# jopohl/urh

Measured on AMD Instinct MI355X. Metric: Msamples/s IQ->bits (1 GiB complex64 2-FSK per GPU, qad materialised, compact outputs copied to the host), higher is better.
Workload: dtype f32

## Files before the change

### include/urhgpu.h

```cpp
#ifndef URHGPU_H
#define URHGPU_H

#include <stdint.h>

#ifdef __cplusplus
extern "C" {
#endif

#define URHGPU_VERSION 100

#define URHGPU_OK 0
#define URHGPU_ERR_HIP (-1)
#define URHGPU_ERR_DTYPE (-2)
#define URHGPU_ERR_ARG (-3)
#define URHGPU_ERR_CAPACITY (-4)
#define URHGPU_ERR_UNSUPPORTED (-5)
#define URHGPU_ERR_NO_DEVICE (-6)

#define URHGPU_DT_I8 0
#define URHGPU_DT_U8 1
#define URHGPU_DT_I16 2
#define URHGPU_DT_U16 3
#define URHGPU_DT_F32 4

// ... 53 lines not shown
                                float *d_out, int64_t chunk, int64_t n_chunks, double *d_sum, double *d_max);

int urhgpu_bandpass(urhgpu_ctx *ctx, const float *x, int64_t n, const double *taps, int64_t m, int64_t shift,
                    int64_t n_out, double *out);

int urhgpu_bandpass_dev(urhgpu_ctx *ctx, const float *d_x, int64_t n, const double *d_taps, int64_t m, int64_t shift,
                        int64_t n_out, const float *d_left, int64_t n_left, const float *d_right, int64_t n_right,
                        void *d_out, int out_c64);

int urhgpu_iir_filter(urhgpu_ctx *ctx, const double *a, int64_t na, const double *b, int64_t nb,
                      const float *x, int64_t n, float *out);


typedef struct urhgpu_params {
    int dtype;
    int mod;
    int bits_per_symbol;
    float noise_threshold;
    float center;
    float center_spacing;
    int tolerance;
    uint32_t samples_per_symbol;
    float costas_loop_bandwidth;
    int64_t pause_threshold;
    int write_bit_sample_pos;
    float noise_other;
    int mod_order;
} urhgpu_params;

typedef struct urhgpu_outputs {
    float *qad;
    int64_t *rows;
    int64_t cap_rows;
    uint8_t *bits;
    int64_t cap_bits;
    int64_t *msg_off;
    int64_t *pauses;
    int64_t cap_msg;
    int64_t *pos;
    int64_t cap_pos;
    int64_t *pos_off;
    int64_t *counts;
    void *blob;
    int64_t cap_blob;
    int64_t *h_counts;
} urhgpu_outputs;

#define URHGPU_BLOB_MAGIC INT64_C(0x55524842424C4F42)
#define URHGPU_BLOB_HEADER_BYTES 128
#define URHGPU_BLOB_LEN16 2
#define URHGPU_BLOB_ROW16 4
int64_t urhgpu_blob_capacity(int64_t cap_rows, int64_t cap_bits, int64_t cap_msg, int64_t cap_pos, int has_pos);

int urhgpu_outputs_to_host(urhgpu_ctx *ctx, const urhgpu_outputs *out, int write_pos, void *host_dst, int64_t cap_dst, int64_t *total_bytes);

int urhgpu_afp_demod_dev(urhgpu_ctx *ctx, const void *d_iq, int64_t n, const urhgpu_params *p, float *d_qad);

int urhgpu_grab_pulse_lens_dev(urhgpu_ctx *ctx, const float *d_qad, int64_t n, const urhgpu_params *p,
                               int64_t *d_rows, int64_t cap_rows, int64_t *d_n_rows);

int urhgpu_ppseq_to_bits_dev(urhgpu_ctx *ctx, const int64_t *d_rows, const int64_t *d_n_rows, int64_t cap_rows_hint,
                             const urhgpu_params *p, const urhgpu_outputs *out);

int urhgpu_iq_to_bits_dev(urhgpu_ctx *ctx, const void *d_iq, int64_t n, const urhgpu_params *p,
                          const urhgpu_outputs *out);

typedef struct urhgpu_center_result {
    double center;
    int64_t flag;
    int64_t n_bins;
    double e0, delta;
    int64_t kept, trimmed;
    int64_t n_counts;
} urhgpu_center_result;
int urhgpu_detect_center_dev(urhgpu_ctx *ctx, const float *d_qad, int64_t n, int64_t max_size, void *d_result, int64_t hist_cap);
int urhgpu_iq_to_bits_auto_center_dev(urhgpu_ctx *ctx, const void *d_iq, int64_t n, const urhgpu_params *p, int64_t max_size,
                                      const urhgpu_outputs *out, void *d_result, void *h_result, int64_t hist_cap);
int64_t urhgpu_center_hist_cap(urhgpu_ctx *ctx);

typedef struct urhgpu_stream urhgpu_stream;
typedef struct urhgpu_host_result {
    int64_t seq;
    int64_t n_samples;
    int64_t n_rows, n_msg, n_bits, n_pos, rows_needed;
    int64_t blob_bytes;
    int truncated;
    const int32_t *row_len;
    const uint16_t *row_len16;
    const void *esc;
    int64_t n_esc;
    const int8_t *row_state;
    const uint8_t *bits_packed;
    const int64_t *msg_off, *pauses, *pos_off;
    const uint32_t *pos32;
    const void *blob;
    const float *d_qad;
    const uint16_t *row16;
} urhgpu_host_result;
int urhgpu_stream_capacities(int64_t n_max, const urhgpu_params *p, int64_t *cap_rows, int64_t *cap_bits, int64_t *cap_msg, int64_t *cap_pos);
int urhgpu_stream_create(urhgpu_ctx *ctx, int64_t n_max, const urhgpu_params *p, int want_qad, int want_pos, int64_t cap_rows, urhgpu_stream **out);
int urhgpu_stream_destroy(urhgpu_stream *st);
int urhgpu_stream_push(urhgpu_stream *st, const void *d_iq, int64_t n, urhgpu_host_result *ready);
int urhgpu_stream_push_upload(urhgpu_stream *st, const void *h_iq, void *d_iq, int64_t n, urhgpu_host_result *ready);
int urhgpu_stream_flush(urhgpu_stream *st, urhgpu_host_result *out3, int *n_out);
int urhgpu_stream_set_auto_center(urhgpu_stream *st, int enable, int64_t max_size);
int urhgpu_stream_center(urhgpu_stream *st, int64_t seq, double *center, int64_t *flag, const uint32_t **hist, int64_t *n_bins, double *e0,
                         double *delta);
int urhgpu_stream_stats(urhgpu_stream *st, int64_t *out4);
int urhgpu_stream_costas_stats(urhgpu_stream *st, int64_t *out5);
int urhgpu_stream_wide_passes(urhgpu_stream *st, int64_t *n_passes);

#define URHGPU_ROW_ABSORBED (-(INT64_C(1) << 62))
#define URHGPU_SHARD_SUMMARY_BYTES 72
int urhgpu_shard_runs_dev(urhgpu_ctx *ctx, const void *d_iq, int64_t n_local, int64_t pos_base, int64_t n_total,
                          int rank, int world, const void *d_left_halo, const urhgpu_params *p,
                          const urhgpu_outputs *out, void *d_summary);
int urhgpu_shard_prelaunch_dev(urhgpu_ctx *ctx, const void *d_iq, int64_t n_local, int64_t pos_base, int64_t n_total,
                               int rank, int world, const urhgpu_params *p, const urhgpu_outputs *out);
int urhgpu_shard_launch_dev(urhgpu_ctx *ctx, const void *d_iq, int64_t n_local, int64_t pos_base, int64_t n_total,
                            int rank, int world, const void *d_left_halo, const urhgpu_params *p, const urhgpu_outputs *out);
int urhgpu_shard_rows_dev(urhgpu_ctx *ctx, const void *d_summaries, int64_t *d_merge);
int urhgpu_shard_bits_prepare_dev(urhgpu_ctx *ctx, const int64_t *d_merge_all, int64_t *d_flags);
int urhgpu_shard_bits_finish_dev(urhgpu_ctx *ctx, const int64_t *d_flags_all);

#define URHGPU_COSTAS_SUMMARY_BYTES 160
int64_t urhgpu_costas_halo_samples(const urhgpu_params *p);
int urhgpu_shard_costas_spec_dev(urhgpu_ctx *ctx, const void *d_iq, int64_t n_local, int64_t pos_base, int64_t n_total, int rank, int world,
                                 const void *d_halo, int64_t n_halo, const urhgpu_params *p, const urhgpu_outputs *out, void *d_summary);
int urhgpu_shard_costas_resolve_dev(urhgpu_ctx *ctx, const uint32_t *start_state, uint32_t *d_end_state);

int urhgpu_shard_demod_dev(urhgpu_ctx *ctx, const void *d_iq, int64_t n_local, int64_t pos_base, int64_t n_total, int rank, int world,
                           const void *d_left_halo, const urhgpu_params *p, const urhgpu_outputs *out);
int urhgpu_shard_seam_value(urhgpu_ctx *ctx, float *seam);

int urhgpu_magnitude_chunk_stats_dev(urhgpu_ctx *ctx, const void *d_iq, int dtype, int64_t n, int64_t chunk,
                                     int64_t n_chunks, double *d_sum, double *d_max);


int urhgpu_segment_runs_dev(urhgpu_ctx *ctx, const void *d_iq, int dtype, int64_t n, float noise_threshold,
                            int64_t *d_rows, int64_t cap_rows, int64_t *d_n_rows);
int urhgpu_message_ranges_dev(urhgpu_ctx *ctx, const void *d_iq, int dtype, int64_t n, float noise_threshold, int64_t *seg_out, int64_t cap_seg_out,
                              int64_t *n_seg_out, int64_t *merged_out, int64_t cap_merged_out, int64_t *n_merged_out, int *merge_ambiguous);
int urhgpu_message_ranges_demod_dev(urhgpu_ctx *ctx, const void *d_iq, int dtype, int64_t n, float noise_threshold, int64_t *seg_out,
                                    int64_t cap_seg_out, int64_t *n_seg_out, int64_t *merged_out, int64_t cap_merged_out,
                                    int64_t *n_merged_out, int *merge_ambiguous, float *d_qad_ask);
int urhgpu_compact_gt_dev(urhgpu_ctx *ctx, const float *d_x, int64_t n, float thr, float *d_out, int64_t *d_count);
int urhgpu_edges_le_dev(urhgpu_ctx *ctx, const float *d_x, int64_t n, float center, int64_t *d_idx, int64_t cap, int64_t *d_count);
int urhgpu_minmax_f32_dev(urhgpu_ctx *ctx, const float *d_x, int64_t n, float *d_out2);
int urhgpu_pairwise_sum_f32_dev(urhgpu_ctx *ctx, const float *d_x, int64_t n, int mode, float mean, float *sum_out);
int urhgpu_histogram_f32_dev(urhgpu_ctx *ctx, const float *d_x, int64_t n, const double *d_edges, int64_t n_edges, int64_t *d_counts);

int urhgpu_msg_center_stats(urhgpu_ctx *ctx, const float *d_x, int64_t n, const int64_t *ranges, int n_msgs, int64_t max_bins,
                            double *out_stats, int64_t *out_hist, double *out_center, int32_t *out_flag);
int urhgpu_msg_plateaus(urhgpu_ctx *ctx, const float *d_x, int64_t n, const int64_t *ranges, const double *centers, int n_msgs,
                        int percentage, int64_t extra_window, int64_t *out_off, uint64_t *out_len, int64_t cap_total);

int urhgpu_merge_plateaus(const uint64_t *plateaus, int64_t n, uint64_t tolerance, uint64_t max_count, uint64_t *out, int64_t *n_out);

int urhgpu_detect_modulation_dev(urhgpu_ctx *ctx, const float *d_iq, int64_t n, const int64_t *ranges, int n_msgs, int wavelet_scale,
                                 int median_filter_order, int *labels_out, double *vars_out);

int urhgpu_msg_bit_lengths(const uint64_t *lens, const int64_t *off, int n_msgs, int64_t *tol_out, int64_t *bitlen_out);
int urhgpu_msg_plateau_decisions(urhgpu_ctx *ctx, const float *d_x, int64_t n, const int64_t *ranges, const double *centers, int n_msgs,
                                 int percentage, int64_t extra_window, int64_t *tol_out, int64_t *bitlen_out);
int urhgpu_msg_estimate(urhgpu_ctx *ctx, const float *d_x, int64_t n, const int64_t *ranges, int n_msgs, int64_t max_bins, int percentage,
                        int64_t extra_window, double *out_stats, double *out_center, int32_t *out_flag, int64_t *tol_out, int64_t *bitlen_out);
int urhgpu_test_bit_length_from_counts(const uint64_t *lens, int64_t n, int64_t *tol_out, int64_t *bitlen_out);
int urhgpu_msg_divisor_histogram(const uint64_t *lens, int64_t n, uint64_t *hist_out, int64_t cap, int64_t *hist_len, int64_t *tol_out);
int urhgpu_bit_length_from_order(const uint64_t *hist, const int64_t *order_desc, int64_t len, int64_t *bitlen_out);

int urhgpu_minmax(urhgpu_ctx *ctx, const void *arr, int dtype, int64_t n, void *out2);
int urhgpu_segment_messages(urhgpu_ctx *ctx, const void *magnitudes, int is_f64, int64_t n, float noise_threshold, int64_t *seg_out,
                            int64_t cap_seg, int64_t *n_seg);
int urhgpu_get_plateau_lengths(urhgpu_ctx *ctx, const float *rect_data, int64_t n, float center, int percentage, uint64_t *out, int64_t cap,
                               int64_t *n_out);
int urhgpu_threshold_divisor_histogram(const uint64_t *lens, int64_t n, float threshold, uint64_t *hist_out, int64_t cap, int64_t *hist_len);
int urhgpu_median_filter(urhgpu_ctx *ctx, const double *data, int64_t n, unsigned int k, float *out);

int urhgpu_test_fast_division_dev(urhgpu_ctx *ctx, uint64_t seed, int reps, uint64_t *n_mismatch);
int urhgpu_test_sincosf_fast_dev(urhgpu_ctx *ctx, uint64_t *n_mismatch);
int urhgpu_test_force_merge_ambiguous(int on);

int urhgpu_modulate_dev(urhgpu_ctx *ctx, const uint8_t *bits, const int64_t *bit_off, const uint32_t *pause, const uint32_t *start,
                        int n_msgs, uint32_t samples_per_symbol, int mod, const float *parameters, int bits_per_symbol,
                        float carrier_amplitude, float carrier_frequency, float carrier_phase, float sample_rate, int dtype,
                        void *d_out, int64_t cap_samples, int64_t *total_samples);
int urhgpu_modulate(urhgpu_ctx *ctx, const uint8_t *bits, int64_t num_bits, uint32_t samples_per_symbol, int mod,
                    const float *parameters, int bits_per_symbol, float carrier_amplitude, float carrier_frequency,
                    float carrier_phase, float sample_rate, uint32_t pause, uint32_t start, int dtype, void *out);

int urhgpu_modulate_gfsk_dev(urhgpu_ctx *ctx, const uint8_t *bits, const int64_t *bit_off, const uint32_t *pause, const uint32_t *start,
                             int n_msgs, uint32_t samples_per_symbol, const float *parameters, int bits_per_symbol,
                             float carrier_amplitude, float carrier_phase, float sample_rate, int dtype, const float *gauss_fir,
                             int n_taps, const float *frequencies, void *d_out, int64_t cap_samples, int64_t *total_samples);
int urhgpu_modulate_gfsk(urhgpu_ctx *ctx, const uint8_t *bits, int64_t num_bits, uint32_t samples_per_symbol, const float *parameters,
                         int bits_per_symbol, float carrier_amplitude, float carrier_phase, float sample_rate, uint32_t pause,
                         uint32_t start, int dtype, const float *gauss_fir, int n_taps, const float *frequencies, void *out);

int urhgpu_convert_dev(urhgpu_ctx *ctx, const void *d_src, int src_dtype, void *d_dst, int dst_dtype, int64_t n);
int urhgpu_pcm_to_iq_dev(urhgpu_ctx *ctx, const void *d_raw, int64_t n_frames, int channels, int sample_width, float *d_out);
int urhgpu_fft_peak_dev(urhgpu_ctx *ctx, const float *d_x, int64_t n, int64_t *peak_index);
int urhgpu_sub_encode_runs(const uint8_t *values, int64_t n, int64_t stride, int64_t *runs_out, int64_t cap, int64_t *n_runs);
int urhgpu_astype_dev(urhgpu_ctx *ctx, const void *d_src, int src_dtype, void *d_dst, int dst_dtype, int64_t n);

int urhgpu_path_minmax_dev(urhgpu_ctx *ctx, const void *d_samples, int dtype, int64_t start, int64_t end,
                           int64_t samples_per_pixel, void *d_values);
int urhgpu_path_minmax(urhgpu_ctx *ctx, const void *samples, int dtype, int64_t n, int64_t start, int64_t end,
                       int64_t samples_per_pixel, void *values);

int urhgpu_spectrogram_dev(urhgpu_ctx *ctx, const float *d_x, int64_t n, int window_size, int64_t hop, int64_t frames,
                           const double *d_window, const double *d_twiddles, double *d_stft, float *d_db);
int urhgpu_bgra_lookup_dev(urhgpu_ctx *ctx, const float *d_db, int64_t frames, int window_size, const uint32_t *d_colormap,
                           int n_colors, float data_min, float data_max, uint32_t *d_image);

int urhgpu_bench_copy_ceiling_dev(urhgpu_ctx *ctx, const float *d_in, float *d_out, int64_t n_samples, int shape, int reps, float *ms_per_copy);
int urhgpu_test_hot_probe(urhgpu_ctx *ctx, const void *d_iq, int64_t n, const urhgpu_params *p, float *d_qad, int stream_kind, int event_mode,
                          int graded, int launches, int keep, void *d_chunks_out, int64_t *n_chunks_out, float *dur_ms, float *gap_ms, int bubble_us,
                          int load_kind);
int urhgpu_test_hot_stamps(int on);
int urhgpu_test_tail_skip(int mask);
int urhgpu_test_fetch_chunk_tables(urhgpu_ctx *ctx, void *host_dst, int64_t n_chunks);
int urhgpu_memcpy_to_host(urhgpu_ctx *ctx, const void *d_src, void *host_dst, int64_t bytes);
int urhgpu_memcpy_dtod(urhgpu_ctx *ctx, void *d_dst, const void *d_src, int64_t bytes);

int urhgpu_test_force_state_bytes(int on);

int urhgpu_test_force_generic_tail(int on);

int urhgpu_test_force_tiles_per_chunk(int tiles);

int64_t urhgpu_test_wide_int_launches(void);

int64_t urhgpu_test_costas_host_syncs(void);
int64_t urhgpu_test_center_host_syncs(void);
int urhgpu_test_costas_scratch(int64_t n, int loop_order, int64_t *out3);

int urhgpu_test_atan2f_dev(urhgpu_ctx *ctx, const float *d_y, const float *d_x, int64_t n, float *d_out);

int urhgpu_chunk_power_stats_dev(urhgpu_ctx *ctx, const void *d_src, int dtype, int64_t n_rows, void *d_dst, int64_t n_store, double *sum_out,
                                 double *max_out);
int urhgpu_chunk_stats_launches(urhgpu_ctx *ctx, int64_t *n_launches);

int urhgpu_magnitude_chunk_partials_dev(urhgpu_ctx *ctx, const void *d_iq, int dtype, int64_t n_local, int64_t pos_base, int64_t n_total,
                                        int64_t chunk, int64_t n_chunks, double *d_sum, double *d_max);
#define URHGPU_PW_REC_HEAD 8
#define URHGPU_PW_REC_FIRST 136
#define URHGPU_PW_REC_LAST 264
#define URHGPU_PW_REC_TAIL 392
#define URHGPU_PW_REC_PIECES 520
int urhgpu_pairwise_partial_f32_dev(urhgpu_ctx *ctx, const float *d_x, int64_t m_local, int64_t g_off, int64_t m_total, int mode, float mean,
                                    float *d_out, int64_t cap, int64_t *n_out);

typedef struct urhgpu_noise_result {
    double noise;
    float noise_f32;
    float noise_sqrd;
    int64_t flag;
    int64_t chunk, n_chunks;
    int64_t n_candidates;
    double min_mean, max_mean;
} urhgpu_noise_result;
double urhgpu_noise_max_magnitude(int dtype);
int urhgpu_detect_noise_level_dev(urhgpu_ctx *ctx, const void *d_iq, int dtype, int64_t n, void *d_result);
int urhgpu_iq_to_bits_auto_dev(urhgpu_ctx *ctx, const void *d_iq, int64_t n, const urhgpu_params *p, int auto_noise, int auto_center,
                               int64_t center_max_size, const urhgpu_outputs *out, void *d_noise_result, void *h_noise_result,
                               void *d_center_result, void *h_center_result, int64_t hist_cap);
int urhgpu_stream_set_auto_noise(urhgpu_stream *st, int enable);
int urhgpu_stream_noise(urhgpu_stream *st, int64_t seq, double *noise, int64_t *flag);
int64_t urhgpu_test_noise_host_syncs(void);

typedef struct urhgpu_msg_record {
    double rssi;
    int64_t first_pos;
    int64_t mid_pos;
    int32_t n_pad;
    int32_t flag;
} urhgpu_msg_record;
int urhgpu_msg_records_dev(urhgpu_ctx *ctx, const void *d_iq, int64_t n, const urhgpu_params *p, const urhgpu_outputs *out,
                           int64_t message_length_divisor, void *d_rec, int64_t cap_msg, void *h_rec);
int urhgpu_stream_set_msg_records(urhgpu_stream *st, int enable, int64_t message_length_divisor);
int urhgpu_stream_msg_records(urhgpu_stream *st, int64_t seq, const urhgpu_msg_record **rec, int64_t *n_msg);
int64_t urhgpu_test_records_host_syncs(void);

int urhgpu_dc_correct_dev(urhgpu_ctx *ctx, const void *d_in, int64_t n, int dtype, void *d_out, void *d_mean);
int urhgpu_dc_correct(urhgpu_ctx *ctx, const void *h_in, int64_t n, int dtype, void *h_out, void *h_mean);
int64_t urhgpu_test_dc_host_syncs(void);
int urhgpu_test_dc_stats(urhgpu_ctx *ctx, int64_t *stats);

int urhgpu_shard_dc_sums_dev(urhgpu_ctx *ctx, const void *d_in, int64_t n, int dtype, void *d_words);
#define URHGPU_DC_RECORD_BYTES 64
int urhgpu_shard_dc_spec_dev(urhgpu_ctx *ctx, const void *d_in, int64_t n, const double *base, void *d_records);
int urhgpu_shard_dc_resolve_dev(urhgpu_ctx *ctx, const void *d_in, int64_t n, const uint32_t *entry, void *d_exit);
int urhgpu_shard_dc_apply_dev(urhgpu_ctx *ctx, const void *d_in, int64_t n, int dtype, const void *mean, void *d_out);
int urhgpu_shard_dc_stats(urhgpu_ctx *ctx, int64_t *stats);

#define URHGPU_SHARD_REC_SUMMARY_WORDS 10
#define URHGPU_SHARD_REC_FIRST_WORDS 8
int urhgpu_shard_records_summary_dev(urhgpu_ctx *ctx, int64_t n_local, int64_t pos_base, const urhgpu_outputs *out, void *d_words);
int urhgpu_shard_records_lookup_dev(urhgpu_ctx *ctx, const urhgpu_outputs *out, const void *d_index, int64_t n, void *d_values);
int urhgpu_shard_msg_records_dev(urhgpu_ctx *ctx, const void *d_iq, int64_t n_local, int64_t pos_base, int64_t n_total, const urhgpu_params *p,
                                 const urhgpu_outputs *out, int64_t message_length_divisor, const int64_t *first, const void *d_window,
                                 int64_t window_len, void *d_rec, int64_t cap_msg, void *h_rec);

#ifdef __cplusplus
}
#endif
#endif
```

### urh_amd/_lib.py

```python
import ctypes as C
import os
import threading

HERE = os.path.dirname(os.path.abspath(__file__))
LIB_PATH = os.path.join(HERE, "liburhgpu.so")

OK = 0
ERR_HIP, ERR_DTYPE, ERR_ARG, ERR_CAPACITY, ERR_UNSUPPORTED, ERR_NO_DEVICE = -1, -2, -3, -4, -5, -6
BLOB_LEN16 = 2
BLOB_ROW16 = 4

DT_I8, DT_U8, DT_I16, DT_U16, DT_F32 = 0, 1, 2, 3, 4
MOD_ASK, MOD_FSK, MOD_PSK, MOD_OTHER = 0, 1, 2, 3
ROW_ABSORBED = -(1 << 62)
BLOB_MAGIC = 0x55524842424C4F42
BLOB_HEADER_BYTES = 128


class UrhGpuError(RuntimeError):
    def __init__(self, status, msg):
        super().__init__(msg)
        self.status = status


class Params(C.Structure):
    _fields_ = [
        ("dtype", C.c_int), ("mod", C.c_int), ("bits_per_symbol", C.c_int),
        ("noise_threshold", C.c_float), ("center", C.c_float), ("center_spacing", C.c_float),
        ("tolerance", C.c_int), ("samples_per_symbol", C.c_uint32), ("costas_loop_bandwidth", C.c_float),
        ("pause_threshold", C.c_int64), ("write_bit_sample_pos", C.c_int), ("noise_other", C.c_float),
        ("mod_order", C.c_int),
    ]


class Outputs(C.Structure):
    _fields_ = [
        ("qad", C.c_void_p), ("rows", C.c_void_p), ("cap_rows", C.c_int64),
        ("bits", C.c_void_p), ("cap_bits", C.c_int64),
        ("msg_off", C.c_void_p), ("pauses", C.c_void_p), ("cap_msg", C.c_int64),
        ("pos", C.c_void_p), ("cap_pos", C.c_int64), ("pos_off", C.c_void_p),
        ("counts", C.c_void_p),
        ("blob", C.c_void_p), ("cap_blob", C.c_int64), ("h_counts", C.c_void_p),
    ]


class CenterResult(C.Structure):
    _fields_ = [("center", C.c_double), ("flag", C.c_int64), ("n_bins", C.c_int64), ("e0", C.c_double), ("delta", C.c_double),
                ("kept", C.c_int64), ("trimmed", C.c_int64), ("n_counts", C.c_int64)]


class NoiseResult(C.Structure):
    _fields_ = [("noise", C.c_double), ("noise_f32", C.c_float), ("noise_sqrd", C.c_float), ("flag", C.c_int64), ("chunk", C.c_int64),
                ("n_chunks", C.c_int64), ("n_candidates", C.c_int64), ("min_mean", C.c_double), ("max_mean", C.c_double)]


class MsgRecord(C.Structure):
    _fields_ = [("rssi", C.c_double), ("first_pos", C.c_int64), ("mid_pos", C.c_int64), ("n_pad", C.c_int32), ("flag", C.c_int32)]


class HostResult(C.Structure):
    _fields_ = [
        ("seq", C.c_int64), ("n_samples", C.c_int64),
        ("n_rows", C.c_int64), ("n_msg", C.c_int64), ("n_bits", C.c_int64), ("n_pos", C.c_int64), ("rows_needed", C.c_int64),
        ("blob_bytes", C.c_int64), ("truncated", C.c_int),
        ("row_len", C.c_void_p), ("row_len16", C.c_void_p), ("esc", C.c_void_p), ("n_esc", C.c_int64),
        ("row_state", C.c_void_p), ("bits_packed", C.c_void_p),
        ("msg_off", C.c_void_p), ("pauses", C.c_void_p), ("pos_off", C.c_void_p), ("pos32", C.c_void_p),
        ("blob", C.c_void_p), ("d_qad", C.c_void_p), ("row16", C.c_void_p),
    ]


_vp, _i64, _i, _f = C.c_void_p, C.c_int64, C.c_int, C.c_float
PROTOTYPES = {
    "urhgpu_version": (_i, []),
    "urhgpu_strerror": (C.c_char_p, [_i]),
    "urhgpu_last_hip_error": (C.c_char_p, []),
    "urhgpu_device_count": (_i, [C.POINTER(_i)]),
    "urhgpu_ctx_create": (_i, [_i, C.POINTER(_vp)]),
    "urhgpu_ctx_destroy": (_i, [_vp]),
    "urhgpu_ctx_set_stream": (_i, [_vp, _vp]),
    "urhgpu_ctx_use_private_stream": (_i, [_vp]),
    "urhgpu_ctx_sync": (_i, [_vp]),
    "urhgpu_ctx_set_pipelined": (_i, [_vp, _i, _vp]),
    "urhgpu_ctx_set_tuning": (_i, [_vp, C.c_char_p, _i]),
    "urhgpu_ctx_join": (_i, [_vp]),
    "urhgpu_ctx_reserve": (_i, [_vp, _i64, _i]),
    "urhgpu_ctx_info": (_i, [_vp, C.POINTER(_i), C.POINTER(_i), C.POINTER(_i64), C.c_char_p, _i]),
    "urhgpu_ctx_costas_stats": (_i, [_vp, C.POINTER(C.c_int32)]),
    "urhgpu_ctx_costas_stats5": (_i, [_vp, C.POINTER(C.c_int32)]),
    "urhgpu_ctx_profile_begin": (_i, [_vp, _i]),
    "urhgpu_ctx_profile_end": (_i, [_vp, C.POINTER(C.c_float), _i, C.POINTER(_i)]),
    "urhgpu_get_magnitudes": (_i, [_vp, _vp, _i, _i64, _vp]),
    "urhgpu_afp_demod": (_i, [_vp, _vp, _i, _i64, _f, _i, _i, _f, _f, _vp]),
    "urhgpu_get_center_thresholds": (_i, [_f, _f, _i, _vp]),
    "urhgpu_grab_pulse_lens": (_i, [_vp, _vp, _i64, _f, C.c_uint16, _i, C.c_uint32, C.c_uint8, _f, _f, _vp, _i64,
                                    C.POINTER(_i64)]),
    "urhgpu_ppseq_to_bits": (_i, [_vp, _vp, _i64, _i64, _i, _i, _i64, _vp, _i64, _vp, _vp, _i64, _vp, _i64, _vp, _vp]),
    "urhgpu_fir_filter": (_i, [_vp, _vp, _i64, _vp, _i64, _vp]),
    "urhgpu_fir_filter_dev": (_i, [_vp, _vp, _i64, _vp, _i64, _vp, _vp]),
    "urhgpu_fir_filter_stats_dev": (_i, [_vp, _vp, _i64, _vp, _i64, _vp, _vp, _i64, _i64, _vp, _vp]),
    "urhgpu_bandpass": (_i, [_vp, _vp, _i64, _vp, _i64, _i64, _i64, _vp]),
    "urhgpu_bandpass_dev": (_i, [_vp, _vp, _i64, _vp, _i64, _i64, _i64, _vp, _i64, _vp, _i64, _vp, _i]),
    "urhgpu_iir_filter": (_i, [_vp, _vp, _i64, _vp, _i64, _vp, _i64, _vp]),
    "urhgpu_afp_demod_dev": (_i, [_vp, _vp, _i64, C.POINTER(Params), _vp]),
    "urhgpu_grab_pulse_lens_dev": (_i, [_vp, _vp, _i64, C.POINTER(Params), _vp, _i64, _vp]),
    "urhgpu_ppseq_to_bits_dev": (_i, [_vp, _vp, _vp, _i64, C.POINTER(Params), C.POINTER(Outputs)]),
    "urhgpu_iq_to_bits_dev": (_i, [_vp, _vp, _i64, C.POINTER(Params), C.POINTER(Outputs)]),
    "urhgpu_detect_center_dev": (_i, [_vp, _vp, _i64, _i64, _vp, _i64]),
    "urhgpu_iq_to_bits_auto_center_dev": (_i, [_vp, _vp, _i64, C.POINTER(Params), _i64, C.POINTER(Outputs), _vp, _vp, _i64]),
    "urhgpu_center_hist_cap": (_i64, [_vp]),
    "urhgpu_stream_set_auto_center": (_i, [_vp, _i, _i64]),
    "urhgpu_stream_center": (_i, [_vp, _i64, C.POINTER(C.c_double), C.POINTER(_i64), C.POINTER(_vp), C.POINTER(_i64), C.POINTER(C.c_double),
                                  C.POINTER(C.c_double)]),
    "urhgpu_test_center_host_syncs": (_i64, []),
    "urhgpu_noise_max_magnitude": (C.c_double, [_i]),
    "urhgpu_detect_noise_level_dev": (_i, [_vp, _vp, _i, _i64, _vp]),
    "urhgpu_iq_to_bits_auto_dev": (_i, [_vp, _vp, _i64, C.POINTER(Params), _i, _i, _i64, C.POINTER(Outputs), _vp, _vp, _vp, _vp, _i64]),
    "urhgpu_stream_set_auto_noise": (_i, [_vp, _i]),
    "urhgpu_stream_noise": (_i, [_vp, _i64, C.POINTER(C.c_double), C.POINTER(_i64)]),
    "urhgpu_test_noise_host_syncs": (_i64, []),
    "urhgpu_msg_records_dev": (_i, [_vp, _vp, _i64, C.POINTER(Params), C.POINTER(Outputs), _i64, _vp, _i64, _vp]),
    "urhgpu_stream_set_msg_records": (_i, [_vp, _i, _i64]),
    "urhgpu_stream_msg_records": (_i, [_vp, _i64, C.POINTER(_vp), C.POINTER(_i64)]),
    "urhgpu_test_records_host_syncs": (_i64, []),
    "urhgpu_shard_records_summary_dev": (_i, [_vp, _i64, _i64, C.POINTER(Outputs), _vp]),
    "urhgpu_shard_records_lookup_dev": (_i, [_vp, C.POINTER(Outputs), _vp, _i64, _vp]),
    "urhgpu_shard_msg_records_dev": (_i, [_vp, _vp, _i64, _i64, _i64, C.POINTER(Params), C.POINTER(Outputs), _i64, C.POINTER(_i64), _vp, _i64, _vp, _i64,
                                          _vp]),
    "urhgpu_blob_capacity": (_i64, [_i64, _i64, _i64, _i64, _i]),
    "urhgpu_outputs_to_host": (_i, [_vp, C.POINTER(Outputs), _i, _vp, _i64, C.POINTER(_i64)]),
    "urhgpu_host_libm_check": (_i, [C.POINTER(_i64)]),
    "urhgpu_stream_capacities": (_i, [_i64, C.POINTER(Params), C.POINTER(_i64), C.POINTER(_i64), C.POINTER(_i64), C.POINTER(_i64)]),
    "urhgpu_stream_create": (_i, [_vp, _i64, C.POINTER(Params), _i, _i, _i64, C.POINTER(_vp)]),
    "urhgpu_stream_destroy": (_i, [_vp]),
    "urhgpu_stream_push": (_i, [_vp, _vp, _i64, C.POINTER(HostResult)]),
    "urhgpu_stream_push_upload": (_i, [_vp, _vp, _vp, _i64, C.POINTER(HostResult)]),
    "urhgpu_stream_flush": (_i, [_vp, C.POINTER(HostResult), C.POINTER(_i)]),
    "urhgpu_stream_stats": (_i, [_vp, C.POINTER(_i64)]),
    "urhgpu_stream_wide_passes": (_i, [_vp, C.POINTER(_i64)]),
    "urhgpu_stream_costas_stats": (_i, [_vp, C.POINTER(_i64)]),
    "urhgpu_shard_runs_dev": (_i, [_vp, _vp, _i64, _i64, _i64, _i, _i, _vp, C.POINTER(Params), C.POINTER(Outputs), _vp]),
    "urhgpu_shard_prelaunch_dev": (_i, [_vp, _vp, _i64, _i64, _i64, _i, _i, C.POINTER(Params), C.POINTER(Outputs)]),
    "urhgpu_shard_launch_dev": (_i, [_vp, _vp, _i64, _i64, _i64, _i, _i, _vp, C.POINTER(Params), C.POINTER(Outputs)]),
    "urhgpu_shard_rows_dev": (_i, [_vp, _vp, _vp]),
    "urhgpu_shard_bits_prepare_dev": (_i, [_vp, _vp, _vp]),
    "urhgpu_shard_bits_finish_dev": (_i, [_vp, _vp]),
    "urhgpu_costas_halo_samples": (_i64, [C.POINTER(Params)]),
    "urhgpu_shard_costas_spec_dev": (_i, [_vp, _vp, _i64, _i64, _i64, _i, _i, _vp, _i64, C.POINTER(Params), C.POINTER(Outputs), _vp]),
    "urhgpu_shard_costas_resolve_dev": (_i, [_vp, C.POINTER(C.c_uint32), _vp]),
    "urhgpu_shard_demod_dev": (_i, [_vp, _vp, _i64, _i64, _i64, _i, _i, _vp, C.POINTER(Params), C.POINTER(Outputs)]),
    "urhgpu_shard_seam_value": (_i, [_vp, C.POINTER(C.c_float)]),
    "urhgpu_magnitude_chunk_stats_dev": (_i, [_vp, _vp, _i, _i64, _i64, _i64, _vp, _vp]),
    "urhgpu_segment_runs_dev": (_i, [_vp, _vp, _i, _i64, _f, _vp, _i64, _vp]),
    "urhgpu_message_ranges_dev": (_i, [_vp, _vp, _i, _i64, _f, _vp, _i64, C.POINTER(_i64), _vp, _i64, C.POINTER(_i64), C.POINTER(_i)]),
    "urhgpu_message_ranges_demod_dev": (_i, [_vp, _vp, _i, _i64, _f, _vp, _i64, C.POINTER(_i64), _vp, _i64, C.POINTER(_i64), C.POINTER(_i), _vp]),
    "urhgpu_compact_gt_dev": (_i, [_vp, _vp, _i64, _f, _vp, _vp]),
    "urhgpu_edges_le_dev": (_i, [_vp, _vp, _i64, _f, _vp, _i64, _vp]),
    "urhgpu_minmax_f32_dev": (_i, [_vp, _vp, _i64, _vp]),
    "urhgpu_pairwise_sum_f32_dev": (_i, [_vp, _vp, _i64, _i, _f, C.POINTER(_f)]),
    "urhgpu_histogram_f32_dev": (_i, [_vp, _vp, _i64, _vp, _i64, _vp]),
    "urhgpu_msg_center_stats": (_i, [_vp, _vp, _i64, _vp, _i, _i64, _vp, _vp, _vp, _vp]),
    "urhgpu_msg_plateaus": (_i, [_vp, _vp, _i64, _vp, _vp, _i, _i, _i64, _vp, _vp, _i64]),
    "urhgpu_detect_modulation_dev": (_i, [_vp, _vp, _i64, _vp, _i, _i, _i, _vp, _vp]),
    "urhgpu_msg_bit_lengths": (_i, [_vp, _vp, _i, _vp, _vp]),
    "urhgpu_msg_plateau_decisions": (_i, [_vp, _vp, _i64, _vp, _vp, _i, _i, _i64, _vp, _vp]),
    "urhgpu_msg_estimate": (_i, [_vp, _vp, _i64, _vp, _i, _i64, _i, _i64, _vp, _vp, _vp, _vp, _vp]),
    "urhgpu_test_bit_length_from_counts": (_i, [_vp, _i64, C.POINTER(_i64), C.POINTER(_i64)]),
    "urhgpu_msg_divisor_histogram": (_i, [_vp, _i64, _vp, _i64, C.POINTER(_i64), C.POINTER(_i64)]),
    "urhgpu_bit_length_from_order": (_i, [_vp, _vp, _i64, C.POINTER(_i64)]),
    "urhgpu_merge_plateaus": (_i, [_vp, _i64, C.c_uint64, C.c_uint64, _vp, C.POINTER(_i64)]),
    "urhgpu_minmax": (_i, [_vp, _vp, _i, _i64, _vp]),
    "urhgpu_segment_messages": (_i, [_vp, _vp, _i, _i64, _f, _vp, _i64, C.POINTER(_i64)]),
    "urhgpu_get_plateau_lengths": (_i, [_vp, _vp, _i64, _f, _i, _vp, _i64, C.POINTER(_i64)]),
    "urhgpu_threshold_divisor_histogram": (_i, [_vp, _i64, _f, _vp, _i64, C.POINTER(_i64)]),
    "urhgpu_median_filter": (_i, [_vp, _vp, _i64, C.c_uint, _vp]),
    "urhgpu_test_hot_probe": (_i, [_vp, _vp, _i64, C.POINTER(Params), _vp, _i, _i, _i, _i, _i, _vp, C.POINTER(_i64), _vp, _vp, _i, _i]),
    "urhgpu_test_hot_stamps": (_i, [_i]),
    "urhgpu_test_tail_skip": (_i, [_i]),
    "urhgpu_test_fetch_chunk_tables": (_i, [_vp, _vp, _i64]),
    "urhgpu_test_fast_division_dev": (_i, [_vp, C.c_uint64, _i, C.POINTER(C.c_uint64)]),
    "urhgpu_test_sincosf_fast_dev": (_i, [_vp, C.POINTER(C.c_uint64)]),
    "urhgpu_test_force_merge_ambiguous": (_i, [_i]),
    "urhgpu_modulate_dev": (_i, [_vp, _vp, _vp, _vp, _vp, _i, C.c_uint32, _i, _vp, _i, _f, _f, _f, _f, _i, _vp, _i64, C.POINTER(_i64)]),
    "urhgpu_modulate": (_i, [_vp, _vp, _i64, C.c_uint32, _i, _vp, _i, _f, _f, _f, _f, C.c_uint32, C.c_uint32, _i, _vp]),
    "urhgpu_modulate_gfsk_dev": (_i, [_vp, _vp, _vp, _vp, _vp, _i, C.c_uint32, _vp, _i, _f, _f, _f, _i, _vp, _i, _vp, _vp, _i64, C.POINTER(_i64)]),
    "urhgpu_modulate_gfsk": (_i, [_vp, _vp, _i64, C.c_uint32, _vp, _i, _f, _f, _f, C.c_uint32, C.c_uint32, _i, _vp, _i, _vp, _vp]),
    "urhgpu_spectrogram_dev": (_i, [_vp, _vp, _i64, _i, _i64, _i64, _vp, _vp, _vp, _vp]),
    "urhgpu_bgra_lookup_dev": (_i, [_vp, _vp, _i64, _i, _vp, _i, _f, _f, _vp]),
    "urhgpu_convert_dev": (_i, [_vp, _vp, _i, _vp, _i, _i64]),
    "urhgpu_pcm_to_iq_dev": (_i, [_vp, _vp, _i64, _i, _i, _vp]),
    "urhgpu_sub_encode_runs": (_i, [_vp, _i64, _i64, _vp, _i64, _vp]),
    "urhgpu_fft_peak_dev": (_i, [_vp, _vp, _i64, _vp]),
    "urhgpu_astype_dev": (_i, [_vp, _vp, _i, _vp, _i, _i64]),
    "urhgpu_path_minmax_dev": (_i, [_vp, _vp, _i, _i64, _i64, _i64, _vp]),
    "urhgpu_path_minmax": (_i, [_vp, _vp, _i, _i64, _i64, _i64, _i64, _vp]),
    "urhgpu_bench_copy_ceiling_dev": (_i, [_vp, _vp, _vp, _i64, _i, _i, C.POINTER(_f)]),
    "urhgpu_memcpy_to_host": (_i, [_vp, _vp, _vp, _i64]),
    "urhgpu_memcpy_dtod": (_i, [_vp, _vp, _vp, _i64]),
    "urhgpu_test_force_state_bytes": (_i, [_i]),
    "urhgpu_test_force_tiles_per_chunk": (_i, [_i]),
    "urhgpu_test_wide_int_launches": (_i64, []),
    "urhgpu_test_costas_host_syncs": (_i64, []),
    "urhgpu_test_costas_scratch": (_i, [_i64, _i, C.POINTER(_i64)]),
    "urhgpu_test_force_generic_tail": (_i, [_i]),
    "urhgpu_test_atan2f_dev": (_i, [_vp, _vp, _vp, _i64, _vp]),
    "urhgpu_chunk_power_stats_dev": (_i, [_vp, _vp, _i, _i64, _vp, _i64, C.POINTER(C.c_double), C.POINTER(C.c_double)]),
    "urhgpu_chunk_stats_launches": (_i, [_vp, C.POINTER(_i64)]),
    "urhgpu_magnitude_chunk_partials_dev": (_i, [_vp, _vp, _i, _i64, _i64, _i64, _i64, _i64, _vp, _vp]),
    "urhgpu_pairwise_partial_f32_dev": (_i, [_vp, _vp, _i64, _i64, _i64, _i, _f, _vp, _i64, C.POINTER(_i64)]),
    "urhgpu_dc_correct_dev": (_i, [_vp, _vp, _i64, _i, _vp, _vp]),
    "urhgpu_dc_correct": (_i, [_vp, _vp, _i64, _i, _vp, _vp]),
    "urhgpu_test_dc_host_syncs": (_i64, []),
    "urhgpu_test_dc_stats": (_i, [_vp, C.POINTER(_i64)]),
    "urhgpu_shard_dc_sums_dev": (_i, [_vp, _vp, _i64, _i, _vp]),
    "urhgpu_shard_dc_spec_dev": (_i, [_vp, _vp, _i64, C.POINTER(C.c_double), _vp]),
    "urhgpu_shard_dc_resolve_dev": (_i, [_vp, _vp, _i64, C.POINTER(C.c_uint32), _vp]),
    "urhgpu_shard_dc_apply_dev": (_i, [_vp, _vp, _i64, _i, _vp, _vp]),
    "urhgpu_shard_dc_stats": (_i, [_vp, C.POINTER(_i64)]),
}

_lib = None
_lock = threading.Lock()


def _share_torch_hip_runtime():
    import importlib.util
    try:
        spec = importlib.util.find_spec("torch")
    except (ImportError, ValueError):
        spec = None
    if spec is None or not spec.origin:
        return
    cand = os.path.join(os.path.dirname(spec.origin), "lib", "libamdhip64.so")
    if os.path.exists(cand):
        try:
            C.CDLL(cand, mode=C.RTLD_GLOBAL)
        except OSError:
            pass


def load():
    global _lib
    with _lock:
        if _lib is None:
            path = os.environ.get("URHGPU_LIB", LIB_PATH)
            if not os.path.exists(path):
                raise UrhGpuError(ERR_NO_DEVICE, f"{path} is missing: build it with `python -m urh_amd.build` "
                                                 "(there is no CPU fallback)")
            _share_torch_hip_runtime()
            lib = C.CDLL(path)
            for name, (res, args) in PROTOTYPES.items():
                fn = getattr(lib, name)
                fn.restype = res
                fn.argtypes = args
            _lib = lib
    return _lib


def host_libm_check():
    out = (C.c_int64 * 4)()
    check(load().urhgpu_host_libm_check(out))
    return {"sincosf_compared": int(out[0]), "sincosf_mismatches": int(out[1]), "atan2f_compared": int(out[2]), "atan2f_mismatches": int(out[3])}


_libm_verdict = None


def host_libm_verdict(warn: bool = True):
    global _libm_verdict
    if _libm_verdict is None:
        _libm_verdict = host_libm_check()
        if warn and (_libm_verdict["sincosf_mismatches"] or _libm_verdict["atan2f_mismatches"]):
            import warnings
            warnings.warn("liburhgpu: this host's libm differs from the one the device code restates "
                          f"(sinf/cosf: {_libm_verdict['sincosf_mismatches']} of {_libm_verdict['sincosf_compared']}, atan2f: "
                          f"{_libm_verdict['atan2f_mismatches']} of {_libm_verdict['atan2f_compared']} probes): PSK / FSK results may differ from the "
                          "reference run on THIS host in isolated samples", RuntimeWarning, stacklevel=3)
    return _libm_verdict


def check(status: int):
    if status == OK:
        return
    lib = load()
    msg = lib.urhgpu_strerror(status).decode()
    if status == ERR_HIP:
        msg += ": " + lib.urhgpu_last_hip_error().decode()
    if status == ERR_DTYPE:
        raise ValueError("Unsupported dtype")
    raise UrhGpuError(status, msg)


class Context:

    def __init__(self, device: int = 0):
        lib = load()
        h = C.c_void_p()
        check(lib.urhgpu_ctx_create(int(device), C.byref(h)))
        self._h = h
        self.device = int(device)

    @property
    def handle(self):
        return self._h

    def set_stream(self, stream_ptr):
        check(load().urhgpu_ctx_set_stream(self._h, C.c_void_p(stream_ptr or 0)))

    def use_private_stream(self):
        check(load().urhgpu_ctx_use_private_stream(self._h))

    def sync(self):
        check(load().urhgpu_ctx_sync(self._h))

    def set_pipelined(self, enable: bool, tail_stream_ptr=None):
        check(load().urhgpu_ctx_set_pipelined(self._h, 1 if enable else 0, C.c_void_p(tail_stream_ptr or 0)))

    def set_tuning(self, key: str, value: int):
        check(load().urhgpu_ctx_set_tuning(self._h, key.encode(), int(value)))

    def join(self):
        check(load().urhgpu_ctx_join(self._h))

    def reserve(self, n_samples: int, tolerance: int):
        check(load().urhgpu_ctx_reserve(self._h, int(n_samples), int(tolerance)))

    def info(self):
        cu, wf, mem = C.c_int(), C.c_int(), C.c_int64()
        name = C.create_string_buffer(256)
        check(load().urhgpu_ctx_info(self._h, C.byref(cu), C.byref(wf), C.byref(mem), name, 256))
        return {"compute_units": cu.value, "wavefront": wf.value, "hbm_bytes": mem.value, "name": name.value.decode()}

    def profile_begin(self, max_records: int):
        check(load().urhgpu_ctx_profile_begin(self._h, int(max_records)))

    def profile_end(self, cap: int = 4096):
        ms = (C.c_float * cap)()
        n = C.c_int(0)
        check(load().urhgpu_ctx_profile_end(self._h, ms, cap, C.byref(n)))
        return [float(ms[i]) for i in range(min(n.value, cap))]

    def costas_stats(self):
        out = (C.c_int32 * 4)()
        check(load().urhgpu_ctx_costas_stats(self._h, out))
        return tuple(int(v) for v in out)

    def costas_stats5(self):
        out = (C.c_int32 * 5)()
        check(load().urhgpu_ctx_costas_stats5(self._h, out))
        return tuple(int(v) for v in out)

    def close(self):
        if self._h:
            load().urhgpu_ctx_destroy(self._h)
            self._h = None

    def __del__(self):
        try:
            self.close()
        except Exception:
            pass


_tls = threading.local()


def default_context() -> Context:
    ctx = getattr(_tls, "ctx", None)
    if ctx is None or ctx._h is None:
        ctx = Context(int(os.environ.get("URHGPU_DEVICE", "0")))
        _tls.ctx = ctx
    return ctx
```

### urh_amd/csrc/common.hpp

```cpp
#pragma once
#include <hip/hip_runtime.h>
#include <stdint.h>
#include <stdio.h>
#include <string.h>

#include <atomic>
#include <vector>

#include "../../include/urhgpu.h"

#ifndef URH_TAIL_PRIO_LEVEL
#define URH_TAIL_PRIO_LEVEL 3
#endif
#ifndef URH_TAIL_PAD
#define URH_TAIL_PAD 0
#endif
#if URH_TAIL_PAD
#define URH_TAIL_PRIO() do { __builtin_amdgcn_s_setprio(URH_TAIL_PRIO_LEVEL); __asm__ volatile("v_mov_b32 v95, 0" ::: "v95"); } while (0)
#else
#define URH_TAIL_PRIO() __builtin_amdgcn_s_setprio(URH_TAIL_PRIO_LEVEL)
#endif

namespace urh {

extern thread_local char g_hip_err[256];

inline int hip_fail(hipError_t e, const char *what, const char *file, int line) {
    snprintf(g_hip_err, sizeof(g_hip_err), "%s: %s (%s:%d)", what, hipGetErrorString(e), file, line);
    return URHGPU_ERR_HIP;
}

#define URH_HIP(call)                                                        \
    do {                                                                     \
        hipError_t _e = (call);                                              \
        if (_e != hipSuccess) return urh::hip_fail(_e, #call, __FILE__, __LINE__); \
    } while (0)

#define URH_TRY(call)                 \
    do {                              \
        int _s = (call);              \
        if (_s != URHGPU_OK) return _s; \
    } while (0)

struct Arena {
    void *base = nullptr;
    size_t cap = 0;
    size_t used = 0;
    int reserve(size_t bytes);
    void reset() { used = 0; }
    void *take(size_t bytes) {
        size_t off = (used + 255) & ~size_t(255);
        if (off + bytes > cap) return nullptr;
        used = off + bytes;
        return (char *)base + off;
    }
    void release();
};
inline size_t align256(size_t x) { return (x + 255) & ~size_t(255); }

extern std::atomic<long long> g_center_host_syncs;
extern thread_local int g_center_scope;
extern std::atomic<long long> g_noise_host_syncs;
extern thread_local int g_noise_scope;
extern std::atomic<long long> g_records_host_syncs;
extern thread_local int g_records_scope;
inline void center_note_wait() {
    if (g_center_scope > 0) ++g_center_host_syncs;
    if (g_noise_scope > 0) ++g_noise_host_syncs;
    if (g_records_scope > 0) ++g_records_host_syncs;
}
struct CenterScope { CenterScope() { ++g_center_scope; } ~CenterScope() { --g_center_scope; } };
struct NoiseScope { bool on; explicit NoiseScope(bool enable = true) : on(enable) { if (on) ++g_noise_scope; } ~NoiseScope() { if (on) --g_noise_scope; } };
struct RecordsScope { bool on; explicit RecordsScope(bool enable = true) : on(enable) { if (on) ++g_records_scope; } ~RecordsScope() { if (on) --g_records_scope; } };

}

constexpr size_t kSmallPinned = size_t(1) << 20;
constexpr int kNoiseMaxChunks = 199;
constexpr size_t kNoiseWorkBytes = 128 * 1024;
struct urhgpu_ctx {
    int device = 0;
    hipStream_t own_stream = nullptr;
    hipStream_t stream = nullptr;
    hipDeviceProp_t prop;
    urh::Arena arena;
    urh::Arena staging;
    urh::Arena aux;
    urh::Arena fir_work;
    hipEvent_t ev_fir = nullptr;
    hipStream_t fir_stream = nullptr;
    int64_t *d_counts = nullptr;
    int64_t *h_counts = nullptr;
    bool tune_spin_wait = true;
    bool tune_wide_int = false;
    bool tune_shard_summary_generic = false;
    int tune_costas_dev_rounds = -1;
    int32_t *costas_stats_next = nullptr;
    hipStream_t last_tail = nullptr;
    int wide_int_next = 0;
    char *h_small = nullptr;
    int32_t *d_tickets = nullptr;
    void *d_desc = nullptr;
    size_t desc_cap = 0;
    void *d_rdesc = nullptr;
    size_t rdesc_cap = 0;
    unsigned long long scan_epoch = 0x0ACE0FBA5E000000ull;
    std::vector<hipEvent_t> prof_events;
    std::vector<bool> prof_dispatch;
    int prof_used = 0;
    bool prof_on = false;
    bool prof_bracket = false;
    void *shard = nullptr;
    bool pipelined = false;
    int hot_lds_pad_sharded = 33 * 1024;
    int tune_hot_cus_removed = 4;
    hipStream_t hot_masked = nullptr;
    hipEvent_t ev_in = nullptr;
    int hot_lds_pad = 0;
    hipStream_t tail_stream = nullptr;
    bool own_tail_stream = false;
    urh::Arena arena_alt, arena_alt2;
    hipEvent_t ev_hot = nullptr;
    hipEvent_t ev_tail[3] = {nullptr, nullptr, nullptr};
    int flip = 0;
    bool tail_pending = false;
    int tile_parity = 0;
    void *d_seg = nullptr;
    bool seg_dirty[3] = {false, false, false};
    int tune_stream_segments = 7;
    int tune_stream_policy = 5;
    long long passes_begun = 0;
    bool tune_stream_latency = false;
    bool tune_stream_pos_direct = true;
    int tune_upload_pieces = 4;
    hipEvent_t ev_piece[16] = {};
    hipEvent_t ev_hot_done[3] = {nullptr, nullptr, nullptr};
    hipStream_t bits_stream = nullptr;
    hipEvent_t ev_rows[3][16] = {};
    hipEvent_t ev_bits[3] = {nullptr, nullptr, nullptr};
    urh::Arena chunk_work;
    double *h_chunk = nullptr;
    long long chunk_launches = 0;
    urh::Arena center_work;
    int tune_center_max_bins = 4096;
    hipEvent_t ev_center = nullptr;
    void *d_noise_work = nullptr;
    int wide_int_auto = 0;
    urh::Arena dc_work;
    hipEvent_t ev_dc = nullptr;
    hipStream_t dc_stream = nullptr;
    const void *dc_shard_in = nullptr;
    int64_t dc_shard_n = -1;
};
constexpr size_t kSegBlockBytes = 4096;

namespace urh {
int iq_to_bits_streamed(urhgpu_ctx *ctx, const void *d_iq, int64_t n, const urhgpu_params *p, const urhgpu_outputs *out, void *host_blob,
                        int64_t cap_host, hipEvent_t ev_ready, bool *streamed, const void *h_iq, void *stage_blob = nullptr, bool *staged = nullptr,
                        hipEvent_t ev_rows = nullptr, int len16 = 0);
hipError_t wait_stream(const urhgpu_ctx *ctx, hipStream_t s);
int reserve_psk_pass(urhgpu_ctx *ctx, int64_t n_max, int tolerance, bool want_qad);
int join_tail(urhgpu_ctx *ctx);
inline int stage_in(urhgpu_ctx *ctx, const void *host, size_t bytes, void **dev) {
    void *d = ctx->staging.take(bytes ? bytes : 16);
    if (!d) return URHGPU_ERR_ARG;
    if (bytes) URH_HIP(hipMemcpyAsync(d, host, bytes, hipMemcpyHostToDevice, ctx->stream));
    *dev = d;
    return URHGPU_OK;
}
inline int fetch_out(urhgpu_ctx *ctx, void *host, const void *dev, size_t bytes) {
    URH_HIP(hipMemcpyAsync(host, dev, bytes, hipMemcpyDeviceToHost, ctx->stream));
    URH_HIP(hipStreamSynchronize(ctx->stream));
    return URHGPU_OK;
}
}
```

### urh_amd/csrc/compact.hip

```cpp
#include <hip/hip_runtime.h>

#include "common.hpp"
#include "compact.hpp"
#include "launchers.hpp"

namespace urh {

struct PackArgs {
    const int64_t *rows; const uint8_t *bits; const int64_t *msg_off, *pauses, *pos_off, *pos; const int64_t *counts;
    int64_t cap_rows, cap_bits, cap_msg, cap_pos;
    int has_pos;
    char *blob; int64_t cap_blob;
};

__global__ __launch_bounds__(256) void k_pack_blob(const PackArgs a) {
    URH_TAIL_PRIO();
    const BlobLayout L = blob_layout(a.counts, a.cap_rows, a.cap_bits, a.cap_msg, a.cap_pos, a.has_pos);
    const int64_t gtid = blockIdx.x * 256ll + threadIdx.x, stride = (int64_t)gridDim.x * 256;
    int64_t *hdr = (int64_t *)a.blob;
    const bool fits = L.total <= a.cap_blob;
    if (gtid == 0) {
        hdr[0] = URHGPU_BLOB_MAGIC; hdr[1] = L.n_rows; hdr[2] = L.n_msg; hdr[3] = L.n_bits; hdr[4] = L.n_pos; hdr[5] = a.counts[4];
        hdr[6] = fits ? L.total : -L.total; hdr[7] = a.has_pos;
        hdr[8] = L.off_pauses; hdr[9] = L.off_msg_off; hdr[10] = L.off_pos_off; hdr[11] = L.off_row_state; hdr[12] = L.off_bits;
        hdr[13] = L.off_row_len; hdr[14] = L.off_pos32;
        if (a.counts[1] > a.cap_msg || a.counts[2] > a.cap_bits || (a.has_pos && a.counts[3] > a.cap_pos) || a.counts[4] > a.cap_rows)
            atomicOr((unsigned long long *)&hdr[15], 1ull);
    }
    bool narrow_fail = false;
    if (!fits) return;
    {
        const int64_t nb = (L.n_bits + 7) / 8;
        uint8_t *out = (uint8_t *)(a.blob + L.off_bits);
        const unsigned long long *in = (const unsigned long long *)a.bits;
        for (int64_t j = gtid; j < nb; j += stride) {
            unsigned long long w;
            if (8 * j + 8 <= L.n_bits) w = in[j];
            else { w = 0; for (int k = 0; k < 8 && 8 * j + k < L.n_bits; ++k) w |= (unsigned long long)a.bits[8 * j + k] << (8 * k); }
            out[j] = (uint8_t)(((w & 0x0101010101010101ull) * 0x8040201008040201ull) >> 56);
        }
    }
    {
        int32_t *len = (int32_t *)(a.blob + L.off_row_len);
        int8_t *st = (int8_t *)(a.blob + L.off_row_state);
        for (int64_t i = gtid; i < L.n_rows; i += stride) {
            const longlong2 r = *(const longlong2 *)(a.rows + 2 * i);
            const bool absorbed = (r.x == kRowAbsorbed);
            st[i] = absorbed ? (int8_t)-128 : (int8_t)r.x; len[i] = (int32_t)r.y;
            narrow_fail |= ((!absorbed && (r.x < -127 || r.x > 127)) || r.y < -0x80000000ll || r.y > 0x7fffffffll);
        }
    }
    if (a.has_pos) {
        uint32_t *p32 = (uint32_t *)(a.blob + L.off_pos32);
        for (int64_t i = gtid; i < L.n_pos; i += stride) {
            const int64_t v = a.pos[i];
            p32[i] = (uint32_t)v;
            narrow_fail |= (v < 0 || v > 0xffffffffll);
        }
    }
    if (narrow_fail) atomicOr((unsigned long long *)&hdr[15], 4ull);
    {
        int64_t *pa = (int64_t *)(a.blob + L.off_pauses), *mo = (int64_t *)(a.blob + L.off_msg_off), *po = (int64_t *)(a.blob + L.off_pos_off);
        for (int64_t i = gtid; i <= L.n_msg; i += stride) {
            if (i < L.n_msg) pa[i] = a.pauses[i];
            mo[i] = a.msg_off[i]; po[i] = a.pos_off[i];
        }
    }
}

int launch_pack_blob(const urhgpu_outputs *o, int write_pos, hipStream_t s) {
    if (!o->blob) return URHGPU_OK;
    if (!o->rows || !o->bits || !o->msg_off || !o->pauses || !o->pos_off || !o->counts) return URHGPU_ERR_ARG;
    if (((uintptr_t)o->bits & 7) || ((uintptr_t)o->blob & 15) || ((uintptr_t)o->rows & 15)) return URHGPU_ERR_ARG;
    const int has_pos = (write_pos && o->pos) ? 1 : 0;
    if (o->cap_blob < blob_capacity(o->cap_rows, o->cap_bits, o->cap_msg, o->cap_pos, has_pos)) return URHGPU_ERR_CAPACITY;
    PackArgs a{o->rows, o->bits, o->msg_off, o->pauses, o->pos_off, o->pos, o->counts, o->cap_rows, o->cap_bits, o->cap_msg, o->cap_pos, has_pos,
               (char *)o->blob, o->cap_blob};
#ifndef URH_PACK_BLOCKS
#define URH_PACK_BLOCKS 512
#endif
    if (hipMemsetAsync((char *)o->blob + 15 * 8, 0, 8, s) != hipSuccess) return URHGPU_ERR_HIP;
    hipLaunchKernelGGL(k_pack_blob, dim3(URH_PACK_BLOCKS), dim3(256), 0, s, a);
    return URHGPU_OK;
}

typedef float cp_v4 __attribute__((ext_vector_type(4)));
typedef float cp_v2 __attribute__((ext_vector_type(2)));
__global__ __launch_bounds__(256) void k_copy_shape(const float *in, float *out) {
    const int lane = threadIdx.x & 63;
    const int64_t wave = (int64_t)blockIdx.x * 4 + (threadIdx.x >> 6);
    const float *src = in + wave * 16 * 256 + lane * 4;
    float *dst = out + wave * 16 * 128 + lane * 2;
    cp_v4 cur[2], nxt[2];
    cur[0] = __builtin_nontemporal_load((const cp_v4 *)src);
    cur[1] = __builtin_nontemporal_load((const cp_v4 *)(src + 256));
#pragma unroll 1
    for (int r = 0; r < 16; r += 2) {
        if (r + 2 < 16) {
            nxt[0] = __builtin_nontemporal_load((const cp_v4 *)(src + (int64_t)(r + 2) * 256));
            nxt[1] = __builtin_nontemporal_load((const cp_v4 *)(src + (int64_t)(r + 3) * 256));
        }
#pragma unroll
        for (int j = 0; j < 2; ++j) {
            const cp_v2 t = {cur[j].x + cur[j].y, cur[j].z + cur[j].w};
            __builtin_nontemporal_store(t, (cp_v2 *)(dst + (int64_t)(r + j) * 128));
        }
        cur[0] = nxt[0]; cur[1] = nxt[1];
    }
}
__global__ __launch_bounds__(256) void k_copy_plain(const cp_v4 *in, cp_v4 *out, int64_t n4) {
    for (int64_t i = blockIdx.x * 256ll + threadIdx.x; i < n4; i += (int64_t)gridDim.x * 256) out[i] = in[i];
}
void launch_copy_shape(const float *in, float *out, int64_t n_samples, int shape, hipStream_t s) {
    if (shape == 0) hipLaunchKernelGGL(k_copy_shape, dim3((unsigned)(n_samples / 8192)), dim3(256), 0, s, in, out);
    else hipLaunchKernelGGL(k_copy_plain, dim3(256 * 20), dim3(256), 0, s, (const cp_v4 *)in, (cp_v4 *)out, n_samples / 4);
}

}
```

### urh_amd/csrc/compact.hpp

```cpp
#pragma once
#include <stdint.h>

#include "../../include/urhgpu.h"

namespace urh {

struct BlobLayout {
    int64_t n_rows, n_msg, n_bits, n_pos;
    int64_t off_pauses, off_msg_off, off_pos_off, off_row_state, off_bits, off_row_len, off_pos32, total;
};

__host__ __device__ inline BlobLayout blob_layout(const int64_t *counts5, int64_t cap_rows, int64_t cap_bits, int64_t cap_msg, int64_t cap_pos,
                                                  int has_pos) {
    BlobLayout L;
    L.n_rows = counts5[0] < cap_rows ? counts5[0] : cap_rows;
    L.n_msg = counts5[1] < cap_msg ? counts5[1] : cap_msg;
    L.n_bits = counts5[2] < cap_bits ? counts5[2] : cap_bits;
    L.n_pos = has_pos ? (counts5[3] < cap_pos ? counts5[3] : cap_pos) : 0;
    if (L.n_rows < 0) L.n_rows = 0;
    if (L.n_msg < 0) L.n_msg = 0;
    if (L.n_bits < 0) L.n_bits = 0;
    if (L.n_pos < 0) L.n_pos = 0;
    auto up = [](int64_t x) { return (x + 15) & ~int64_t(15); };
    int64_t o = URHGPU_BLOB_HEADER_BYTES;
    L.off_pauses = o; o = up(o + L.n_msg * 8);
    L.off_msg_off = o; o = up(o + (L.n_msg + 1) * 8);
    L.off_pos_off = o; o = up(o + (L.n_msg + 1) * 8);
    L.off_row_state = o; o = up(o + L.n_rows);
    L.off_bits = o; o = up(o + (L.n_bits + 7) / 8);
    L.off_row_len = o; o = up(o + L.n_rows * 4);
    L.off_pos32 = o; o = up(o + L.n_pos * 4);
    L.total = o;
    return L;
}

struct StagedLayout { int64_t head_cap, off_row_state, off_row_len, off_pos32, total; };
__host__ __device__ inline StagedLayout staged_layout(int64_t cap_rows, int64_t cap_bits, int64_t cap_msg, int64_t cap_pos, int has_pos) {
    const int64_t c[5] = {0, cap_msg, cap_bits, 0, 0};
    auto up = [](int64_t x) { return (x + 15) & ~int64_t(15); };
    StagedLayout S;
    S.head_cap = blob_layout(c, cap_rows, cap_bits, cap_msg, cap_pos, 0).total;
    S.off_row_state = S.head_cap;
    S.off_row_len = up(S.off_row_state + cap_rows);
    S.off_pos32 = up(S.off_row_len + 4 * cap_rows);
    S.total = up(S.off_pos32 + (has_pos ? 4 * cap_pos : 0));
    return S;
}

inline int64_t blob_capacity(int64_t cap_rows, int64_t cap_bits, int64_t cap_msg, int64_t cap_pos, int has_pos) {
    const int64_t c[5] = {cap_rows, cap_msg, cap_bits, cap_pos, cap_rows};
    return blob_layout(c, cap_rows, cap_bits, cap_msg, cap_pos, has_pos).total;
}

}
```

### urh_amd/csrc/launchers.hpp

```cpp
#pragma once
#include <atomic>
#include <hip/hip_runtime.h>
#include <stdint.h>

#include "common.hpp"
#include "runs.hpp"

namespace urh {

struct RunArgs {
    const void *in;
    float *qad;
    const void *left_halo;
    int64_t n;
    int64_t range_begin;
    int64_t range_end;
    int64_t chunk_base;
    int64_t pos_base;
    int64_t chunk_len;
    uint64_t *slab;
    int64_t slab_stride;
    ChunkInfo *chunks;
    float noise_sqrd;
    float noise_val;
    float max_magnitude;
    int order;
    int tol;
    int launch_part;
    int seg_mode;
    float dm_noise_sqrd, dm_max_magnitude, dm_noise_val;
    int lds_pad;
    uint32_t *progress;
    int32_t n_seg;
    int32_t seg_end[kMaxSegments];
    int64_t launch_lo, launch_hi;
    int64_t graded_from, graded_len;
    int wide_int;
    int stamp_probe;
    float thr[kMaxOrder - 1];
    const float *d_thr;
    const float *d_noise;
};
extern bool g_force_state_bytes;
extern std::atomic<long long> g_wide_int_launches;
extern bool g_stamp_probe;
extern int g_tail_skip;
struct HotEvents { hipEvent_t start = nullptr, stop = nullptr; bool used = false; };
int launch_wide_probe(const void *d_iq, int dtype, int64_t n, float noise_sqrd, int32_t *h_out, hipStream_t s, const float *d_noise = nullptr);
int launch_demod_runs_iq(const RunArgs &a, int dtype, int mod, bool write_qad, hipStream_t s, HotEvents *ev = nullptr);
int launch_runs_qad(const RunArgs &a, hipStream_t s, HotEvents *ev = nullptr);
bool runs_streamable(const RunArgs &a);
int launch_afp_demod(const RunArgs &a, int dtype, int mod, int grid, hipStream_t s);
int launch_afp_seam(const RunArgs &a, int dtype, int mod, float *d_out, hipStream_t s);
void launch_test_div(uint64_t seed, int reps, unsigned long long *d_mismatches, hipStream_t s);
void launch_test_sincosf_fast(unsigned long long *d_mismatches, hipStream_t s);
void launch_test_atan2f(const float *y, const float *x, int64_t n, float *out, hipStream_t s);

struct ModMsg {
    int64_t bit_off;
    int64_t n_sym;
    int64_t sym_off;
    int64_t out_off;
    uint32_t pause;
    uint32_t start;
};
constexpr int kModGfsk = 5;
struct ModArgs {
    const uint8_t *bits;
    const ModMsg *msgs;
    const float *params;
    float *phase;
    void *out;
    int n_msgs, mod, dtype, bps;
    int oqpsk;
    const float *taps;
    int n_taps;
    int freq_given;
    float *gf_freq, *gf_phase;
    uint32_t sps;
    float carrier_amplitude, carrier_frequency, carrier_phase, sample_rate;
};
int launch_modulate(const ModArgs &a, int64_t max_samples, hipStream_t s);

int launch_stft(const float2 *x, int64_t n, int ws, int64_t hop, int64_t frames, const double *window, const double2 *tw,
                double2 *out_c128, float *out_db, hipStream_t s);
int launch_bgra_lookup(const float *data, int64_t frames, int ws, const uint32_t *colormap, int n_colors, float dmin, float dmax,
                       uint32_t *image, hipStream_t s);

int launch_convert(const void *src, int src_dtype, void *dst, int dst_dtype, int64_t n, hipStream_t s);
int launch_astype(const void *src, int src_dtype, void *dst, int dst_dtype, int64_t n, hipStream_t s);
int launch_pcm_to_iq(const void *raw, int64_t n_frames, int channels, int width, float *out, hipStream_t s);
size_t fft_peak_scratch_bytes(int64_t n);
int launch_fft_peak(const float2 *x, int log2n, void *scratch, int64_t *d_peak, hipStream_t s);

int launch_path_minmax(const void *samples, int dtype, int64_t start, int64_t end, int64_t spp, void *values, hipStream_t s);

int launch_bandpass(const float2 *x, int64_t n, const float2 *left, int64_t n_left, const float2 *right, int64_t n_right,
                    const double2 *taps, int m, int64_t shift, int64_t n_out, double2 *out128, float2 *out64, hipStream_t s,
                    void *work = nullptr);
size_t bandpass_fft_work_bytes();

struct ResolveScratch {
    int32_t *has_stable;
    int32_t *prev_stable;
    int32_t *has_acc;
    int32_t *prev_acc;
    int64_t *out_cnt;
    int64_t *out_off;
    int32_t *blk_stable;
    int32_t *blk_acc;
    int64_t *blk_cnt;
};
size_t resolve_scratch_bytes(int64_t n_chunks);
ResolveScratch resolve_scratch_carve(void *mem, int64_t n_chunks);

struct ResolveAux {
    int32_t first_nonlead;
    int32_t open_chunk;
    int32_t first_stable;
    int32_t last_stable;
};
constexpr int32_t kAuxNone = 0x7F7F7F7F;

struct ResolveArgs {
    ChunkInfo *chunks;
    int64_t n_chunks;
    int64_t n_total;
    int tol;
    int local_pass;
    ResolveAux *aux;
    ChunkInfo *summary_out;
    int64_t chunk_first;
    int64_t n_local;
    int64_t *d_ts_carry;
    int64_t *rows;
    int64_t cap_rows;
    int64_t *d_n_acc;
    int64_t *d_n_rows;
    int64_t *d_n_rows_needed;
    int write_last_row;
    ResolveScratch sc;
};
struct EmitArgs {
    const ChunkInfo *chunks;
    int64_t chunk_first;
    const uint64_t *slab;
    int64_t slab_stride;
    int64_t *rows;
    int64_t cap_rows;
    int64_t *d_ts_carry;
    int is_ask;
    int64_t sps;
    ResolveScratch sc;
};
struct BitsParams {
    int64_t sps;
    int64_t bps;
    int64_t pause_threshold;
    int64_t samples_per_bit;
    int write_pos;
    const int64_t *d_row_base;
    const int64_t *d_ts_carry;
    const int64_t *d_absorbed;
    const int32_t *d_extra;
    int is_last_rank;
    const int64_t *d_rows_needed;
};
constexpr int64_t kRowAbsorbed = -(int64_t(1) << 62);
struct BitsOut {
    uint8_t *bits; int64_t cap_bits;
    int64_t *msg_off; int64_t *pauses; int64_t cap_msg;
    int64_t *pos; int64_t cap_pos; int64_t *pos_off;
    int64_t *counts;
    int64_t *h_counts = nullptr;
};
int launch_resolve(const ResolveArgs &a, int32_t *tickets, hipStream_t s);
int launch_shard_summary(const ResolveArgs &a, int32_t *ticket, hipStream_t s);
int launch_resolve_emit_single(const ResolveArgs &r, const EmitArgs &e, hipStream_t s);
int launch_emit_rows(const EmitArgs &a, int64_t n_local_chunks, hipStream_t s);
size_t merge_scratch_bytes(int64_t cap);
int launch_merge_rows_ask(const int64_t *rows_in, const int64_t *d_n_in, int64_t cap, int64_t *rows_out,
                          int64_t cap_out, int64_t *d_n_out, void *scratch, int32_t *tickets, hipStream_t s);
size_t bits_scratch_bytes(int64_t cap_rows);
struct ScanState {
    int32_t *tickets;
    void *desc;
    size_t desc_bytes;
    unsigned long long *epoch;
};
size_t bits_desc_bytes(int64_t cap_rows);
int launch_ppseq_to_bits(const int64_t *rows, const int64_t *d_n_rows, int64_t cap_rows, const BitsParams &bp,
                         const BitsOut &o, void *scratch, const ScanState &ss, hipStream_t s);
int launch_bits_prepare(const int64_t *rows, const int64_t *d_n_rows, int64_t cap_rows, const BitsParams &bp,
                        void *scratch, int64_t *d_flags, const ScanState &ss, hipStream_t s);
int launch_bits_finish(const int64_t *rows, const int64_t *d_n_rows, int64_t cap_rows, const BitsParams &bp,
                       const BitsOut &o, void *scratch, const ScanState &ss, hipStream_t s);
struct SegState {
    int64_t rows_at[kMaxSegments];
    int64_t rows_needed;
    int64_t n_acc;
    int64_t n_groups;
    int64_t n_groups_local;
    int64_t end_bits, end_pos, end_msgs;
    int64_t err;
    struct In {
        int64_t g0;
        int64_t carry[3];
        int64_t ship_bits, ship_pos, ship_msgs, pad;
    } in[2];
};
static_assert(sizeof(SegState) == 128 + 64 + 128, "SegState");
constexpr int64_t kSegAlign = 256;
struct SegGate {
    const uint32_t *progress;
    int k;
    uint32_t target;
    int init;
    SegState *seg;
    long long max_ticks;
    int fused;
};
struct RowsSegment {
    int index;
    int final;
    int64_t c0, c1;
    SegGate gate;
    int8_t *h_state;
    int32_t *h_len;
    int fuse_gate;
    int len16;
    int64_t *esc;
    int64_t esc_cap;
};
struct BitsSegment {
    int index;
    int final;
    int64_t c0, c1;
    int rows_index;
    SegState *state;
};
struct SegPackDst {
    void *host;
    int64_t cap_host;
    uint32_t *progress_reset;
    int blocks;
    int pos_direct;
    int split;
    void *host_head;
    const int64_t *esc;
    int64_t esc_cap;
    int64_t row16_esc_off;
};

struct TileTailMem {
    void *mem;
    int64_t n_chunks;
    int32_t *huge_count;
    int parity;
    void *rdesc;
    unsigned long long epoch;
    int64_t *d_row_base = nullptr;
};
size_t tile_rdesc_bytes(int64_t n_chunks);
size_t tile_tail_bytes(int64_t n_chunks);
int64_t tile_desc_cap(int64_t cap_rows, int64_t n_chunks);
int launch_tile_rows(const ResolveArgs &r, const EmitArgs &e, const TileTailMem &m, const BitsParams *bp, hipStream_t s);
int launch_tile_bits(const TileTailMem &m, const int64_t *rows, const int64_t *d_n_rows, int64_t cap_rows, const BitsParams &bp,
                     const BitsOut &o, void *scratch, const ScanState &ss, hipStream_t s);
int launch_tile_bits_prepare(const TileTailMem &m, const int64_t *rows, const int64_t *d_n_rows, int64_t cap_rows, const BitsParams &bp,
                             void *scratch, int64_t *d_flags, const ScanState &ss, hipStream_t s);
int launch_tile_bits_finish(const TileTailMem &m, const int64_t *rows, const int64_t *d_n_rows, int64_t cap_rows, const BitsParams &bp,
                            const BitsOut &o, void *scratch, const ScanState &ss, hipStream_t s);
int launch_rows_segment(const ResolveArgs &r, const EmitArgs &e, const TileTailMem &m, const BitsParams &bp, SegState *state, const RowsSegment &sg,
                        hipStream_t s);
int launch_bits_segment(const TileTailMem &m, const BitsParams &bp, const BitsOut &o, void *scratch, const ScanState &ss, int64_t *rows,
                        int64_t cap_rows, const BitsSegment &sg, const SegPackDst *dst, hipStream_t s);
void launch_merge_summary(const int64_t *rows, const int64_t *d_n_rows, int64_t *d_out5, hipStream_t s);
void launch_merge_fix(int64_t *rows, const int64_t *d_n_rows, const int64_t *d_all, int rank, int world,
                      int64_t *d_absorbed, hipStream_t s);
void launch_bits_extra(const int64_t *d_all, int rank, int world, int32_t *d_extra, hipStream_t s);

size_t fir_stats_scratch_bytes(int64_t n);
size_t fir_work_bytes(int64_t n, int m);
int launch_fir(const float2 *x, int64_t n, const float2 *taps, int m, const float2 *halo, float2 *out, hipStream_t s, void *work = nullptr,
               int64_t chunk = 0, int64_t n_chunks = 0, double *d_sum = nullptr, double *d_max = nullptr, void *tile_scratch = nullptr);
int launch_iir(const double *a, int64_t M, const double *b, int64_t N, const float2 *x, int64_t n, float2 *y, hipStream_t s);
int launch_magnitudes(const void *iq, int dtype, int64_t n, double *out, hipStream_t s);
size_t mag_chunk_scratch_bytes(int64_t n_chunks);
int launch_mag_chunk_stats(const void *iq, int dtype, int64_t n, int64_t chunk, int64_t n_chunks, double *d_sum, double *d_max,
                           void *scratch, hipStream_t s);
int launch_noise_chain(const void *iq, int dtype, int64_t n, double max_mag, float cfg_noise, int use_cfg, void *work, void *d_result, void *h_result,
                       hipStream_t s);
size_t compact_scratch_bytes(int64_t n);
int launch_compact_gt(const float *x, int64_t n, const int64_t *d_n, float thr, float *out, int64_t *d_count, void *scratch,
                      int32_t *tickets, hipStream_t s);
int launch_compact_edges(const float *x, int64_t n, const int64_t *d_n, float center, int64_t *out, int64_t cap, int64_t *d_count,
                         void *scratch, int32_t *tickets, hipStream_t s);
size_t minmax_scratch_bytes();
int launch_minmax(const float *x, int64_t n, float *d_out2, void *scratch, hipStream_t s);
int launch_minmax_any(const void *x, int dtype, int64_t n, void *d_out2, void *scratch, hipStream_t s);
int launch_above_flags(const void *mag, int is_f64, int64_t n, float thr, float *flags, hipStream_t s);
int launch_median_filter(const double *data, int64_t n, int k, float *out, hipStream_t s);
constexpr int kDtAboveFlags = 100;
int pairwise_sum_f32(urhgpu_ctx *ctx, const float *d_x, int64_t n, int mode, float mean, float *out);
int launch_hist_edges(const float *x, int64_t n, const double *d_edges, int n_edges, int64_t *d_counts, hipStream_t s);
size_t sp_mag_scratch_bytes(int64_t n_chunks);
int launch_mag_chunk_partials(const void *iq, int dtype, int64_t n_local, int64_t pos_base, int64_t n_total, int64_t chunk, int64_t n_chunks,
                              double *d_sum, double *d_max, void *scratch, hipStream_t s);
int64_t pairwise_partial_words(int64_t m_local, int64_t g_off, int64_t m_total);
size_t pairwise_partial_scratch_bytes(int64_t m_local);
int launch_pairwise_partial(const float *x, int64_t m_local, int64_t g_off, int64_t m_total, int mode, float mean, float *rec, void *scratch,
                            hipStream_t s);
size_t chunk_stats_scratch_bytes(int dtype, int64_t n_rows);
int launch_chunk_stats(const void *d_src, int dtype, int64_t n_rows, void *d_dst, int64_t store_rows, void *scratch, double *h_out, hipStream_t s);
struct SegCtl;
extern bool g_force_merge_ambiguous;
int launch_message_ranges(const int64_t *d_rows, const int64_t *d_n_rows, int64_t cap_rows, const void *d_iq, int dtype, int64_t n, float thr,
                          int ook_merge, int64_t *d_seg, int64_t *d_msgs, int64_t cap, SegCtl *d_ctl, void *scratch, hipStream_t s);
size_t seg_scratch_bytes(int64_t cap_rows, int64_t cap);
size_t seg_ctl_bytes();
void seg_ctl_read(const void *host_copy, int64_t *n_seg, int64_t *n_msgs, int *ambiguous);
int launch_pack_blob(const urhgpu_outputs *o, int write_pos, hipStream_t s);
void launch_copy_shape(const float *in, float *out, int64_t n_samples, int shape, hipStream_t s);
int launch_msg_records(const void *d_iq, int64_t n, const urhgpu_params *p, const urhgpu_outputs *out, int64_t divisor, void *d_rec, int64_t cap_rec,
                       void *h_rec, hipStream_t s);
size_t costas_scratch_bytes(int64_t n);
int launch_costas(urhgpu_ctx *ctx, const void *d_iq, int64_t n, const urhgpu_params *p, float *d_qad, void *scratch, const float *d_noise = nullptr);
extern std::atomic<long long> g_costas_host_syncs;
void costas_scratch_layout(int64_t n, int K, int64_t out3[3]);
constexpr int kCostasSummaryBytes = 160;
struct CostasShard {
    const void *iq;
    const void *halo_end;
    float *out;
    int64_t n, origin, lo, start1;
    urhgpu_params p;
    void *scratch;
};
int64_t costas_halo_samples(const urhgpu_params *p);
int launch_costas_shard_spec(urhgpu_ctx *ctx, const CostasShard &cs, void *d_summary);
int launch_costas_shard_resolve(urhgpu_ctx *ctx, const CostasShard &cs, uint32_t freq_bits, uint32_t phase_bits, void *d_end);

}
```

### urh_amd/csrc/pulse_table.hip

```cpp
#include <hip/hip_runtime.h>

#include <algorithm>

#include "common.hpp"
#include "compact.hpp"
#include "launchers.hpp"
#include "runs.hpp"
#include "scan.hpp"

namespace urh {

#ifndef URH_RESOLVE_BLOCK
#define URH_RESOLVE_BLOCK 256
#endif
#ifndef URH_RESOLVE_ITEMS
#define URH_RESOLVE_ITEMS 4
#endif
constexpr int kResolveBlock = URH_RESOLVE_BLOCK;

__host__ __device__ static inline int64_t resolve_blocks(int64_t n_chunks) { return (n_chunks + kResolveBlock - 1) / kResolveBlock; }

size_t resolve_scratch_bytes(int64_t n_chunks) {
    return (size_t)n_chunks * (4 * 4 + 2 * 8) + (size_t)(resolve_blocks(n_chunks) + 1) * (4 + 4 + 8) + 10 * 256;
}
// ... 1307 lines not shown
            int64_t type = 0;
#if URH_EXPAND_PREFETCH
            longlong2 row_pf = longlong2{0, 0};
            if (i + 64 < end) row_pf = *(const longlong2 *)(a.rows + 2 * (i + 64));
            if (i < end) {
                type = row_cur.x;
                v = row_value(type, row_cur.y, i == 0 && row0g, a.bp);
            }
            row_cur = row_pf;
#else
            if (i < end) {
                const longlong2 row = (i0 == off) ? row0 : *(const longlong2 *)(a.rows + 2 * i);
                type = row.x;
                v = row_value(type, row.y, i == 0 && row0g, a.bp);
            }
#endif
            int64_t in_bits = v.v[0], in_ts = v.v[2];
            int in_l = (int)v.v[1];
#if URH_DPP_SCAN
            in_bits = wave_incl_sum_dpp(in_bits); in_ts = wave_incl_sum_dpp(in_ts); in_l = wave_incl_sum_dpp(in_l);
#else
#pragma unroll
            for (int o = 1; o < 64; o <<= 1) {
                const int64_t ub = __shfl_up(in_bits, o), ut = __shfl_up(in_ts, o);
                const int ul = __shfl_up(in_l, o);
                if (lane >= o) { in_bits += ub; in_ts += ut; in_l += ul; }
            }
#endif
            int64_t kb = 0, ob = 0, op = 0, ts = 0;
            if (i < end && v.v[0] > 0 && v.v[0] <= own_limit) {
                const int64_t grp = run.v[1] + in_l - v.v[1];
                if (grp < n_groups) {
                    GroupOut go = go0;
                    if (grp != g0) go = a.gout[grp];
                    if (go.is_msg) {
                        const int64_t bit_prefix = run.v[0] + in_bits - v.v[0];
                        kb = v.v[0];
                        ob = go.out_bits + (bit_prefix - go.bits_start);
                        op = go.out_pos + (bit_prefix - go.bits_start);
                        ts = run.v[2] + in_ts - v.v[2];
                    }
                }
            }
            constexpr int kShort = 16;
#if URH_EXPAND_EARLY_EXIT
            {
                const int kbs = (kb > 0 && kb <= kShort) ? (int)kb : 0;
                const int nb = (ob + kbs <= a.cap_bits) ? kbs : (int)((a.cap_bits > ob) ? a.cap_bits - ob : 0);
                const int np = !a.bp.write_pos ? 0 : ((op + kbs <= a.cap_pos) ? kbs : (int)((a.cap_pos > op) ? a.cap_pos - op : 0));
                uint8_t *bp8 = a.bits + ob;
                int64_t *pp = a.pos + op;
                uint32_t *hp = a.h_pos ? a.h_pos + op : nullptr;
                int64_t tsk = ts;
                int sh = bps - 1;
#pragma unroll 1
                for (int k = 0; k < kShort; ++k) {
                    if (__ballot(k < kbs) == 0ull) break;
                    const uint8_t b = (type < 0) ? 0 : (uint8_t)((type >> sh) & 1);
                    sh = (sh == 0) ? bps - 1 : sh - 1;
                    if (k < nb) bp8[k] = b;
                    if (k < np) { pp[k] = tsk; if (hp) hp[k] = (uint32_t)tsk; }
                    tsk += a.bp.samples_per_bit;
                }
            }
#else
            if (kb > 0 && kb <= kShort) {
                const int nb = (ob + kb <= a.cap_bits) ? (int)kb : (int)((a.cap_bits > ob) ? a.cap_bits - ob : 0);
                const int np = !a.bp.write_pos ? 0 : ((op + kb <= a.cap_pos) ? (int)kb : (int)((a.cap_pos > op) ? a.cap_pos - op : 0));
                uint8_t *bp8 = a.bits + ob;
                int64_t *pp = a.pos + op;
                uint32_t *hp = a.h_pos ? a.h_pos + op : nullptr;
                int64_t tsk = ts;
                int sh = bps - 1;
                for (int k = 0; k < (int)kb; ++k) {
                    const uint8_t b = (type < 0) ? 0 : (uint8_t)((type >> sh) & 1);
                    sh = (sh == 0) ? bps - 1 : sh - 1;
                    if (k < nb) bp8[k] = b;
                    if (k < np) { pp[k] = tsk; if (hp) hp[k] = (uint32_t)tsk; }
                    tsk += a.bp.samples_per_bit;
                }
            }
#endif
            unsigned long long big = __ballot(kb > kShort);
            while (big) {
                const int src = __builtin_ctzll(big);
                big &= big - 1;
                const int64_t kb_s = __shfl(kb, src), ob_s = __shfl(ob, src), op_s = __shfl(op, src), ts_s = __shfl(ts, src),
                              ty_s = __shfl(type, src);
                for (int64_t k = lane; k < kb_s; k += 64) {
                    const uint8_t b = symbol_bit(ty_s, k, bps);
                    if (ob_s + k < a.cap_bits) a.bits[ob_s + k] = b;
                    if (a.bp.write_pos && op_s + k < a.cap_pos) {
                        a.pos[op_s + k] = ts_s + k * a.bp.samples_per_bit;
                        if (a.h_pos) a.h_pos[op_s + k] = (uint32_t)(ts_s + k * a.bp.samples_per_bit);
                    }
                }
            }
            run.v[0] += lane_bcast(in_bits, 63); run.v[1] += lane_bcast(in_l, 63); run.v[2] += lane_bcast(in_ts, 63);
        }
        row0 = row_next;
    }
}

int launch_resolve(const ResolveArgs &a, int32_t *tickets, hipStream_t s) {
    if (a.n_chunks <= 0) return URHGPU_ERR_ARG;
    const unsigned g = (unsigned)((a.n_chunks + kResolveBlock - 1) / kResolveBlock);
    (void)tickets;
    hipLaunchKernelGGL(k_resolve_a, dim3(g), dim3(kResolveBlock), 0, s, a);
    hipLaunchKernelGGL(k_resolve_b, dim3(g), dim3(kResolveBlock), 0, s, a);
    hipLaunchKernelGGL(k_resolve_c, dim3(g), dim3(kResolveBlock), 0, s, a);
    return URHGPU_OK;
}

int launch_shard_summary(const ResolveArgs &a, int32_t *ticket, hipStream_t s) {
    if (a.n_chunks <= 0 || !a.local_pass || !a.summary_out || a.n_chunks >= kAuxNone) return URHGPU_ERR_ARG;
    static_assert(sizeof(ShardPart) <= 256 && sizeof(ShardPart) <= (size_t)kResolveBlock * 8, "one partial per kResolveBlock chunks fits the out_cnt section (8 bytes per chunk, 256-byte granules)");
    const unsigned g = (unsigned)resolve_blocks(a.n_chunks);
    hipLaunchKernelGGL(k_shard_summary, dim3(g), dim3(kResolveBlock), 0, s, a, (ShardPart *)a.sc.out_cnt, ticket);
    return URHGPU_OK;
}

int launch_resolve_emit_single(const ResolveArgs &r, const EmitArgs &e, hipStream_t s) {
    if (r.n_chunks <= 0 || r.local_pass || r.chunk_first != 0 || r.n_local != r.n_chunks || e.chunk_first != 0) return URHGPU_ERR_ARG;
    const unsigned g = (unsigned)((r.n_chunks + kResolveBlock - 1) / kResolveBlock);
    hipLaunchKernelGGL(k_resolve_a, dim3(g), dim3(kResolveBlock), 0, s, r);
    hipLaunchKernelGGL(k_resolve_b, dim3(g), dim3(kResolveBlock), 0, s, r);
    hipLaunchKernelGGL(k_emit_rows_fused, dim3((unsigned)r.n_chunks), dim3(64), 0, s, e, r);
    return URHGPU_OK;
}

int launch_emit_rows(const EmitArgs &a, int64_t n_local_chunks, hipStream_t s) {
    if (n_local_chunks > 0) hipLaunchKernelGGL(k_emit_rows, dim3((unsigned)n_local_chunks), dim3(64), 0, s, a);
    return URHGPU_OK;
}

static inline int64_t scan_blocks(int64_t cap) { return (cap + kScanTile - 1) / kScanTile; }
constexpr int kGroupItems = 1;
static inline int64_t group_scan_blocks(int64_t cap) { return (cap + kScanBlock * kGroupItems - 1) / (kScanBlock * kGroupItems); }

size_t merge_scratch_bytes(int64_t cap) {
    return (size_t)(scan_blocks(cap) + 1) * sizeof(VecK<2>) + 256 + (size_t)cap * 16 + 512;
}

int launch_merge_rows_ask(const int64_t *rows_in, const int64_t *d_n_in, int64_t cap, int64_t *rows_out,
                          int64_t cap_out, int64_t *d_n_out, void *scratch, int32_t *tickets, hipStream_t s) {
    if (cap <= 0) return URHGPU_OK;
    const int64_t nb = scan_blocks(cap);
    char *p = (char *)scratch;
    VecK<2> *partials = (VecK<2> *)p; p += ((size_t)(nb + 1) * sizeof(VecK<2>) + 255) & ~size_t(255);
    int64_t *grp_state = (int64_t *)p; p += (size_t)cap * 8;
    int64_t *grp_end = (int64_t *)p;
    MergeLoad ld{rows_in};
    MergeStore st{rows_in, d_n_in, grp_state, grp_end};
    (void)tickets;
    hipLaunchKernelGGL((k_scan_reduce<2, MergeLoad>), dim3(scan_grid(nb)), dim3(kScanBlock), 0, s, d_n_in, ld, partials, nb);
    hipLaunchKernelGGL((k_scan_apply<2, MergeLoad, MergeStore>), dim3(scan_grid(nb)), dim3(kScanBlock), 0, s, d_n_in, ld, partials, nb, st,
                       kScanAlwaysDirect);
    hipLaunchKernelGGL((k_scan_finish<2, NoFinal>), dim3(1), dim3(kScanBlock), 0, s, d_n_in, partials, nb, NoFinal(), kScanAlwaysDirect);
    int64_t fin_blocks = (cap + 255) / 256; if (fin_blocks > 4096) fin_blocks = 4096;
    hipLaunchKernelGGL(k_merge_finish, dim3((unsigned)fin_blocks), dim3(256), 0, s, partials + nb, grp_state, grp_end,
                       rows_out, cap_out, d_n_out);
    return URHGPU_OK;
}

size_t bits_scratch_bytes(int64_t cap_rows) {
    const int64_t nb = scan_blocks(cap_rows);
    const int64_t cap_groups = cap_rows + 1;
    const int64_t nbg = group_scan_blocks(cap_groups);
    return (size_t)(nb + 1) * sizeof(VecK<4>) + (size_t)(nbg + 1) * sizeof(VecK<3>) + (size_t)cap_rows * sizeof(RowInfo) +
           (size_t)cap_groups * (sizeof(GroupInfo) + sizeof(GroupOut)) + 64 + 8 * 256 + 64 + 256 +
           (size_t)kHugeCap * sizeof(HugeRow) + 256;
}

namespace {
struct BitsScratch {
    VecK<4> *part4; VecK<3> *part3; RowInfo *info; GroupInfo *groups; GroupOut *gout; int64_t *d_n_groups;
    HugeRow *huge; int32_t *huge_count;
    int64_t nb, nbg;
};
BitsScratch carve_bits(void *scratch, int64_t cap_rows) {
    BitsScratch b;
    b.nb = scan_blocks(cap_rows);
    const int64_t cap_groups = cap_rows + 1;
    b.nbg = group_scan_blocks(cap_groups);
    char *p = (char *)scratch;
    auto take = [&](size_t bytes) { char *r = p; p += (bytes + 255) & ~size_t(255); return r; };
    b.part4 = (VecK<4> *)take((size_t)(b.nb + 1) * sizeof(VecK<4>));
    b.part3 = (VecK<3> *)take((size_t)(b.nbg + 1) * sizeof(VecK<3>));
    b.info = (RowInfo *)take((size_t)cap_rows * sizeof(RowInfo));
    b.groups = (GroupInfo *)take((size_t)cap_groups * sizeof(GroupInfo));
    b.gout = (GroupOut *)take((size_t)cap_groups * sizeof(GroupOut));
    b.d_n_groups = (int64_t *)take(64);
    b.huge_count = (int32_t *)take(64);
    b.huge = (HugeRow *)take((size_t)kHugeCap * sizeof(HugeRow));
    return b;
}
}

struct GroupCountFinal {
    const int64_t *d_n_rows;
    const GroupInfo *groups;
    int64_t *d_n_groups;
    int64_t *d_flags;
    __device__ void operator()(const VecK<4> &grand) const {
        const int64_t n = *d_n_rows;
        const int64_t n_l = (n > 0) ? grand.v[1] : 0;
        *d_n_groups = (n > 0) ? n_l + 1 : 0;
        if (d_flags) {
            d_flags[0] = n_l > 0;
            d_flags[1] = (n > 0) && groups[0].data_end > 0;
            d_flags[2] = (n > 0) && (groups[n_l].data_end - (n_l ? groups[n_l - 1].data_end : 0) > 0);
        }
    }
};

size_t bits_desc_bytes(int64_t cap_rows) {
    if (cap_rows <= 0) cap_rows = 1;
    return (((size_t)(scan_blocks(cap_rows) + 1) * sizeof(ScanDesc<4>) + 255) & ~size_t(255)) + (size_t)(group_scan_blocks(cap_rows + 1) + 1) * sizeof(ScanDesc<3>) + 512;
}

int launch_bits_prepare(const int64_t *rows, const int64_t *d_n_rows, int64_t cap_rows, const BitsParams &bp,
                        void *scratch, int64_t *d_flags, const ScanState &ss, hipStream_t s) {
    if (cap_rows <= 0) cap_rows = 1;
    if (ss.desc_bytes < bits_desc_bytes(cap_rows)) return URHGPU_ERR_ARG;
    const BitsScratch b = carve_bits(scratch, cap_rows);
    const bool single = (d_flags == nullptr);
    BitsLoad ld{rows, d_n_rows, bp, single ? b.d_n_groups : nullptr};
    BitsStore st{rows, d_n_rows, b.info, b.groups, bp.d_ts_carry, bp.d_absorbed, single ? b.d_n_groups : nullptr};
    GroupCountFinal fin{d_n_rows, b.groups, b.d_n_groups, d_flags};
    hipLaunchKernelGGL((k_scan_reduce<4, BitsLoad>), dim3(scan_grid(b.nb)), dim3(kScanBlock), 0, s, d_n_rows, ld, b.part4, b.nb);
    hipLaunchKernelGGL((k_scan_apply<4, BitsLoad, BitsStore>), dim3(scan_grid(b.nb)), dim3(kScanBlock), 0, s, d_n_rows, ld, b.part4, b.nb, st,
                       kScanAlwaysDirect);
    if (!single)
        hipLaunchKernelGGL((k_scan_finish<4, GroupCountFinal>), dim3(1), dim3(kScanBlock), 0, s, d_n_rows, b.part4, b.nb, fin, kScanAlwaysDirect);
    return URHGPU_OK;
}

int launch_bits_finish(const int64_t *rows, const int64_t *d_n_rows, int64_t cap_rows, const BitsParams &bp,
                       const BitsOut &o, void *scratch, const ScanState &ss, hipStream_t s) {
    if (cap_rows <= 0) cap_rows = 1;
    if (ss.desc_bytes < bits_desc_bytes(cap_rows)) return URHGPU_ERR_ARG;
    const BitsScratch b = carve_bits(scratch, cap_rows);
    ScanDesc<3> *desc3 = (ScanDesc<3> *)((char *)ss.desc + (((size_t)(b.nb + 1) * sizeof(ScanDesc<4>) + 255) & ~size_t(255)));
    GroupLoad gl{b.groups, b.d_n_groups, bp.d_extra, bp.is_last_rank, bp.write_pos};
    GroupStore gs{gl, b.gout, o.msg_off, o.pauses, o.pos_off, o.pos, o.cap_msg, o.cap_pos};
    BitsCountsFinal fin{d_n_rows, o.msg_off, o.pos_off, o.counts, b.huge_count, bp.d_rows_needed, o.h_counts};
    if (!(g_tail_skip & 8))
        hipLaunchKernelGGL((k_scan_lookback<3, GroupLoad, GroupStore, BitsCountsFinal, kGroupItems>), dim3(scan_grid(b.nbg)), dim3(kScanBlock), 0, s,
                           b.d_n_groups, gl, desc3, b.nbg, gs, fin, ++*ss.epoch, ss.tickets + 2, 0);
    ExpandArgs ea{rows, d_n_rows, b.info, b.gout, o.bits, o.cap_bits, o.pos, o.cap_pos, bp, b.huge, b.huge_count, kHugeCap};
    const int64_t eb = std::min<int64_t>((cap_rows + 255) / 256, kExpandMaxBlocks);
    hipLaunchKernelGGL(k_expand_bits, dim3((unsigned)eb), dim3(256), 0, s, ea);
    hipLaunchKernelGGL(k_expand_huge, dim3(kHugeGridX, kHugeGridY), dim3(256), 0, s, ea);
    return URHGPU_OK;
}

int launch_ppseq_to_bits(const int64_t *rows, const int64_t *d_n_rows, int64_t cap_rows, const BitsParams &bp,
                         const BitsOut &o, void *scratch, const ScanState &ss, hipStream_t s) {
    URH_TRY(launch_bits_prepare(rows, d_n_rows, cap_rows, bp, scratch, nullptr, ss, s));
    return launch_bits_finish(rows, d_n_rows, cap_rows, bp, o, scratch, ss, s);
}


int g_tail_skip = 0;
namespace {
constexpr int kTileHugeCap = 8192;
struct TileCarve { TileTail ft; HugeRef *huge; };
TileCarve carve_tile(const TileTailMem &m) {
    TileCarve tc;
    char *p = (char *)m.mem;
    auto take = [&](size_t bytes) { char *r = p; p += (bytes + 255) & ~size_t(255); return r; };
    const int64_t nt = m.n_chunks + 1;
    tc.ft.ploc = (ResElem *)take((size_t)m.n_chunks * sizeof(ResElem));
    tc.ft.btot = (ResElem *)take((size_t)(resolve_blocks(m.n_chunks) + 1) * sizeof(ResElem));
    tc.ft.agg = (VecK<4> *)take((size_t)nt * sizeof(VecK<4>));
    tc.ft.excl = (VecK<4> *)take((size_t)nt * sizeof(VecK<4>));
    tc.ft.tile_off = (int64_t *)take((size_t)nt * 8);
    tc.ft.tile_cnt = (int32_t *)take((size_t)nt * 4);
    tc.ft.d_n_tiles = (int64_t *)take(64);
    tc.huge = (HugeRef *)take((size_t)kTileHugeCap * sizeof(HugeRef));
    tc.ft.huge_count = m.huge_count;
    tc.ft.parity = m.parity;
    tc.ft.want_bits = 0;
    tc.ft.rdesc = (GranDesc *)m.rdesc;
    tc.ft.epoch = m.epoch;
    tc.ft.d_row_base = m.d_row_base;
    tc.ft.esc = nullptr;
    return tc;
}
}

int64_t tile_desc_cap(int64_t cap_rows, int64_t n_chunks) { return std::max<int64_t>(cap_rows, 8 * (n_chunks + 2) + kScanTile); }

size_t tile_rdesc_bytes(int64_t n_chunks) {
    return (size_t)(resolve_blocks(n_chunks) + 2 + (n_chunks + 1 + kScanBlock - 1) / kScanBlock + 2) * sizeof(GranDesc);
}

size_t tile_tail_bytes(int64_t n_chunks) {
    const int64_t nt = n_chunks + 1;
    return (size_t)n_chunks * sizeof(ResElem) + (size_t)(resolve_blocks(n_chunks) + 1) * sizeof(ResElem) + (size_t)nt * (2 * sizeof(VecK<4>) + 12) +
           64 + (size_t)kTileHugeCap * sizeof(HugeRef) + 10 * 256;
}

int launch_tile_rows(const ResolveArgs &r, const EmitArgs &e, const TileTailMem &m, const BitsParams *bp, hipStream_t s) {
    if (r.n_chunks <= 0 || r.local_pass || r.chunk_first != e.chunk_first || r.chunk_first < 0 || r.chunk_first + r.n_local > r.n_chunks ||
        m.n_chunks != r.n_chunks || e.is_ask)
        return URHGPU_ERR_ARG;
    if ((r.n_local != r.n_chunks) != (m.d_row_base != nullptr)) return URHGPU_ERR_ARG;
    TileCarve tc = carve_tile(m);
    EmitTileArgs g;
    g.e = e; g.r = r; g.ft = tc.ft; g.huge = tc.huge; g.huge_cap = kTileHugeCap;
    memset(&g.bp, 0, sizeof(g.bp));
    if (bp) { g.bp = *bp; g.ft.want_bits = 1; }
    const unsigned gb = (unsigned)resolve_blocks(r.n_chunks);
    g.w0 = 0; g.w_end = tail_waves(r.n_chunks); g.final_seg = 1; g.seg = nullptr; g.seg_k = 0; g.h_state = nullptr; g.h_len = nullptr; g.len16 = 0; g.esc = nullptr; g.esc_cap = 0; g.ft.esc = nullptr;
    SegGate no_gate;
    memset(&no_gate, 0, sizeof(no_gate));
    if (!(g_tail_skip & 1)) hipLaunchKernelGGL(k_resolve_one, dim3(gb), dim3(kResolveBlock), 0, s, r, g.ft, (int64_t)0, no_gate);
    if (!(g_tail_skip & 2)) hipLaunchKernelGGL(k_emit_rows_tiles, dim3((unsigned)((tail_waves(r.n_chunks) + 1 + kEmitWaves - 1) / kEmitWaves)), dim3(64 * kEmitWaves), 0, s, g);
    return URHGPU_OK;
}

namespace {
__global__ void k_tile_flags(const int64_t *d_n_rows, const GroupInfo *groups, const int64_t *d_n_groups, int64_t *d_flags) {
    const int64_t n = *d_n_rows, ng = *d_n_groups;
    const int64_t n_l = (n > 0 && ng > 0) ? ng - 1 : 0;
    d_flags[0] = n_l > 0;
    d_flags[1] = (n > 0) && groups[0].data_end > 0;
    d_flags[2] = (n > 0) && (groups[n_l].data_end - (n_l ? groups[n_l - 1].data_end : 0) > 0);
}
}

int launch_tile_bits_prepare(const TileTailMem &m, const int64_t *rows, const int64_t *d_n_rows, int64_t cap_rows, const BitsParams &bp,
                             void *scratch, int64_t *d_flags, const ScanState &ss, hipStream_t s) {
    if (cap_rows <= 0) cap_rows = 1;
    const int64_t nt = m.n_chunks + 1;
    const int64_t cap_desc = tile_desc_cap(cap_rows, m.n_chunks);
    if (ss.desc_bytes < bits_desc_bytes(cap_desc)) return URHGPU_ERR_ARG;
    const TileCarve tc = carve_tile(m);
    const BitsScratch b = carve_bits(scratch, cap_rows);
    const int64_t cap_groups = cap_rows + 1;
    GranDesc *tdesc = (GranDesc *)m.rdesc + resolve_blocks(m.n_chunks) + 2;
    TileScanArgs ta{rows, d_n_rows, tc.ft.agg, tc.ft.tile_off, tc.ft.tile_cnt, tc.ft.excl, b.groups, cap_groups, b.d_n_groups, nt, bp, tdesc,
                    m.epoch, 0, nullptr, 0};
    const unsigned nb_ts = (unsigned)((nt + kScanBlock - 1) / kScanBlock);
    if (!(g_tail_skip & 4)) hipLaunchKernelGGL(k_tile_scan, dim3(nb_ts), dim3(kScanBlock), 0, s, ta);
    if (d_flags) hipLaunchKernelGGL(k_tile_flags, dim3(1), dim3(1), 0, s, d_n_rows, b.groups, b.d_n_groups, d_flags);
    return URHGPU_OK;
}

int launch_tile_bits_finish(const TileTailMem &m, const int64_t *rows, const int64_t *d_n_rows, int64_t cap_rows, const BitsParams &bp,
                            const BitsOut &o, void *scratch, const ScanState &ss, hipStream_t s) {
    if (cap_rows <= 0) cap_rows = 1;
    const int64_t nt = m.n_chunks + 1;
    const int64_t cap_desc = tile_desc_cap(cap_rows, m.n_chunks);
    if (ss.desc_bytes < bits_desc_bytes(cap_desc)) return URHGPU_ERR_ARG;
    const TileCarve tc = carve_tile(m);
    const BitsScratch b = carve_bits(scratch, cap_rows);
    ScanDesc<3> *desc3 = (ScanDesc<3> *)((char *)ss.desc + (((size_t)(scan_blocks(cap_desc) + 1) * sizeof(ScanDesc<4>) + 255) & ~size_t(255)));
    GroupLoad gl{b.groups, b.d_n_groups, bp.d_extra, bp.is_last_rank, bp.write_pos};
    GroupStore gs{gl, b.gout, o.msg_off, o.pauses, o.pos_off, o.pos, o.cap_msg, o.cap_pos};
    BitsCountsFinal fin{d_n_rows, o.msg_off, o.pos_off, o.counts, b.huge_count, bp.d_rows_needed, o.h_counts};
    if (!(g_tail_skip & 8))
        hipLaunchKernelGGL((k_scan_lookback<3, GroupLoad, GroupStore, BitsCountsFinal, kGroupItems>), dim3(scan_grid(b.nbg)), dim3(kScanBlock), 0, s,
                           b.d_n_groups, gl, desc3, b.nbg, gs, fin, ++*ss.epoch, ss.tickets + 2, 0);
    ExpandTileArgs ea{rows, d_n_rows, tc.ft.excl, tc.ft.tile_off, tc.ft.tile_cnt, b.gout, b.d_n_groups, o.bits, o.cap_bits, o.pos, o.cap_pos,
                      bp, tc.huge, m.huge_count, kTileHugeCap, m.parity, nt, 0, nullptr};
    const unsigned tile_blocks = (unsigned)expand_tile_blocks(nt);
    if (!(g_tail_skip & 16)) hipLaunchKernelGGL(k_expand_tiles, dim3(tile_blocks + kHugeBlocksX * kHugeBlocksY), dim3(64 * kEmitWaves), 0, s, ea);
    return URHGPU_OK;
}

int launch_tile_bits(const TileTailMem &m, const int64_t *rows, const int64_t *d_n_rows, int64_t cap_rows, const BitsParams &bp,
                     const BitsOut &o, void *scratch, const ScanState &ss, hipStream_t s) {
    URH_TRY(launch_tile_bits_prepare(m, rows, d_n_rows, cap_rows, bp, scratch, nullptr, ss, s));
    return launch_tile_bits_finish(m, rows, d_n_rows, cap_rows, bp, o, scratch, ss, s);
}

__global__ void k_seg_gate(const SegGate gate) {
    if (threadIdx.x != 0) return;
    if (gate.init) gate.seg->err = 0;
    if (!gate.progress) return;
    const uint32_t *ctr = gate.progress + gate.k * kProgressStride;
    const long long t0 = (long long)wall_clock64();
    while (__hip_atomic_load(ctr, __ATOMIC_RELAXED, __HIP_MEMORY_SCOPE_AGENT) < gate.target) {
        __builtin_amdgcn_s_sleep(16);
        if ((long long)wall_clock64() - t0 > gate.max_ticks) { gate.seg->err = 1 + gate.k; break; }
    }
}

struct SegGroupLoad {
    GroupLoad ld;
    const SegState *seg;
    int parity;
    __device__ VecK<3> operator()(int64_t i) const { return ld(seg->in[parity].g0 + i); }
};
struct SegGroupStore {
    GroupStore st;
    const SegState *seg;
    int parity;
    __device__ void operator()(int64_t i, const VecK<3> &val, const VecK<3> &ex) const {
        const int64_t g0 = seg->in[parity].g0;
        VecK<3> e = ex;
#pragma unroll
        for (int k = 0; k < 3; ++k) e.v[k] += seg->in[parity].carry[k];
        st(g0 + i, val, e);
    }
};
struct SegFinal {
    SegGroupLoad ld;
    SegState *seg;
    const int64_t *d_n_rows;
    int parity;
    int final;
    BitsCountsFinal counts;
    __device__ void operator()(const VecK<3> &grand) const {
        const SegState::In in = seg->in[parity];
        const int64_t nl = seg->n_groups_local;
        VecK<3> tot;
#pragma unroll
        for (int k = 0; k < 3; ++k) tot.v[k] = in.carry[k] + grand.v[k];
        if (final) {
            counts(tot);
            const bool any = *d_n_rows > 0;
            seg->end_msgs = any ? tot.v[0] : 0; seg->end_bits = any ? tot.v[1] : 0; seg->end_pos = any ? tot.v[2] : 0;
            return;
        }
        SegState::In nx = in;
        if (nl <= 0) {
            seg->end_msgs = 0; seg->end_bits = 0; seg->end_pos = 0;
        } else {
            const int64_t g_open = in.g0 + nl - 1;
            const VecK<3> vo = ld(nl - 1);
            VecK<3> exo;
#pragma unroll
            for (int k = 0; k < 3; ++k) exo.v[k] = tot.v[k] - vo.v[k];
            const int64_t d0 = g_open ? ld.ld.groups[g_open - 1].data_end : 0;
            const bool has_data = ld.ld.groups[g_open].data_end - d0 > 0;
            nx.g0 = g_open;
#pragma unroll
            for (int k = 0; k < 3; ++k) nx.carry[k] = exo.v[k];
            seg->end_msgs = exo.v[0]; seg->end_bits = exo.v[1] + vo.v[1]; seg->end_pos = exo.v[2] + vo.v[2];
            nx.ship_msgs = exo.v[0];
            nx.ship_bits = has_data ? exo.v[1] + vo.v[1] : exo.v[1];
            nx.ship_pos = has_data ? exo.v[2] + vo.v[2] : exo.v[2];
        }
        seg->in[parity ^ 1] = nx;
    }
};

struct SegPack {
    const uint8_t *bits; const int64_t *msg_off, *pauses, *pos_off, *pos; const int64_t *counts;
    int64_t cap_rows, cap_bits, cap_msg, cap_pos;
    int has_pos;
    char *host;
    BlobLayout L;
    const SegState *seg;
    const int64_t *d_n_rows;
    int parity, final;
    uint32_t *progress;
    int pos_shipped;
    int split;
    char *head;
    const int64_t *esc;
    int64_t esc_cap;
    int64_t row16_esc_off;
};
__global__ __launch_bounds__(256) void k_pack_seg(const SegPack a) {
    URH_TAIL_PRIO();
    const int64_t gtid = blockIdx.x * 256ll + threadIdx.x, stride = (int64_t)gridDim.x * 256;
    const SegState::In in = a.seg->in[a.parity];
    auto lim = [](int64_t x, int64_t cap) { return x < cap ? (x < 0 ? 0 : x) : cap; };
    const int64_t nbits = lim(a.seg->end_bits, a.cap_bits);
    const int64_t j0 = lim(in.ship_bits, a.cap_bits) / 8, j1 = a.final ? (nbits + 7) / 8 : nbits / 8;
    const int64_t p0 = a.has_pos ? lim(in.ship_pos, a.cap_pos) : 0, p1 = a.has_pos ? lim(a.seg->end_pos, a.cap_pos) : 0;
    const int64_t m0 = lim(in.ship_msgs, a.cap_msg), m1 = lim(a.seg->end_msgs, a.cap_msg);
    BlobLayout L = a.L;
    if (a.split) {
        const int64_t c5[5] = {0, m1, nbits, 0, 0};
        const BlobLayout T = blob_layout(c5, a.cap_rows, a.cap_bits, a.cap_msg, a.cap_pos, 0);
        L.off_pauses = T.off_pauses; L.off_msg_off = T.off_msg_off; L.off_pos_off = T.off_pos_off; L.off_bits = T.off_bits;
    }
    {
        uint8_t *out = (uint8_t *)(a.head + L.off_bits);
        const unsigned long long *in8 = (const unsigned long long *)a.bits;
        auto pack8 = [&](int64_t j) -> unsigned long long {
            unsigned long long w;
            if (8 * j + 8 <= nbits) w = in8[j];
            else { w = 0; for (int k = 0; k < 8 && 8 * j + k < nbits; ++k) w |= (unsigned long long)a.bits[8 * j + k] << (8 * k); }
            return ((w & 0x0101010101010101ull) * 0x8040201008040201ull) >> 56;
        };
#if URH_PACK_WORDS
        int64_t ja = j0 + (int64_t)((8 - ((uintptr_t)(out + j0) & 7)) & 7);
        if (ja > j1) ja = j1;
        int64_t nw = (j1 - ja) / 8;
        const int64_t full = nbits / 8;
        if (ja + 8 * nw > full) nw = full > ja ? (full - ja) / 8 : 0;
        for (int64_t k = gtid; k < nw; k += stride) {
            const int64_t j = ja + 8 * k;
            unsigned long long r = 0;
#pragma unroll
            for (int b = 0; b < 8; ++b) r |= (((in8[j + b] & 0x0101010101010101ull) * 0x8040201008040201ull) >> 56) << (8 * b);
            *(unsigned long long *)(out + j) = r;
        }
        for (int64_t j = j0 + gtid; j < ja; j += stride) out[j] = (uint8_t)pack8(j);
        for (int64_t j = ja + 8 * nw + gtid; j < j1; j += stride) out[j] = (uint8_t)pack8(j);
#else
        for (int64_t j = j0 + gtid; j < j1; j += stride) out[j] = (uint8_t)pack8(j);
#endif
    }
    if (a.has_pos && !a.pos_shipped) {
        uint32_t *p32 = (uint32_t *)(a.host + L.off_pos32);
        for (int64_t i = p0 + gtid; i < p1; i += stride) p32[i] = (uint32_t)a.pos[i];
    }
    {
        int64_t *pa = (int64_t *)(a.head + L.off_pauses), *mo = (int64_t *)(a.head + L.off_msg_off), *po = (int64_t *)(a.head + L.off_pos_off);
        if (gtid == 0 && m0 == 0) { mo[0] = 0; po[0] = 0; }
        for (int64_t i = m0 + gtid; i < m1; i += stride) { pa[i] = a.pauses[i]; mo[i + 1] = a.msg_off[i + 1]; po[i + 1] = a.pos_off[i + 1]; }
    }
    int64_t n_esc = 0;
    if (a.esc && a.final) {
        n_esc = a.esc[0];
        const bool over = n_esc > a.esc_cap;
        if (over) n_esc = a.esc_cap;
        int64_t *dst = (int64_t *)(a.head + (a.row16_esc_off > 0 ? a.row16_esc_off : ((L.off_bits + (nbits + 7) / 8 + 15) & ~int64_t(15))));
        if (gtid == 0) dst[0] = over ? -n_esc : n_esc;
        for (int64_t i = gtid; i < n_esc; i += stride) dst[1 + i] = a.esc[1 + i];
    }
    if (a.final && gtid == 0) {
        int64_t *hdr = (int64_t *)a.head;
        const int64_t *c = a.counts;
        const int64_t n_rows = lim(*a.d_n_rows, a.cap_rows);
        hdr[1] = n_rows; hdr[2] = m1; hdr[3] = nbits; hdr[4] = p1; hdr[5] = c[4];
        const bool row16 = a.esc && a.row16_esc_off > 0;
        hdr[6] = URHGPU_BLOB_HEADER_BYTES + n_rows * (row16 ? 2 : (a.esc ? 3 : 5)) + (a.esc ? 8 + n_esc * 8 : 0) + (nbits + 7) / 8 + p1 * 4 + m1 * 24 + 16;
        hdr[7] = a.has_pos | (row16 ? URHGPU_BLOB_ROW16 : (a.esc ? URHGPU_BLOB_LEN16 : 0));
        hdr[8] = L.off_pauses; hdr[9] = L.off_msg_off; hdr[10] = L.off_pos_off; hdr[11] = row16 ? a.row16_esc_off : L.off_row_state; hdr[12] = L.off_bits;
        hdr[13] = L.off_row_len; hdr[14] = L.off_pos32;
        hdr[15] = ((c[1] > a.cap_msg || c[2] > a.cap_bits || (a.has_pos && c[3] > a.cap_pos) || c[4] > a.cap_rows) ? 1 : 0) | (a.seg->err ? 2 : 0);
        hdr[0] = URHGPU_BLOB_MAGIC;
    }
    if (a.final && a.progress && gtid < kMaxSegments) a.progress[gtid * kProgressStride] = 0;
}

int launch_rows_segment(const ResolveArgs &r, const EmitArgs &e, const TileTailMem &m, const BitsParams &bp, SegState *state, const RowsSegment &sg,
                        hipStream_t s) {
    if (r.n_chunks <= 0 || r.local_pass || r.chunk_first != 0 || e.chunk_first != 0 || r.n_local != r.n_chunks || m.n_chunks != r.n_chunks ||
        e.is_ask || m.d_row_base != nullptr || !state || sg.index < 0 || sg.index >= kMaxSegments)
        return URHGPU_ERR_ARG;
    if (sg.c0 < 0 || sg.c0 % kSegAlign || sg.c1 <= sg.c0 || sg.c1 > r.n_chunks || (sg.final ? sg.c1 != r.n_chunks : (sg.c1 % kSegAlign != 0 || sg.c1 >= r.n_chunks)))
        return URHGPU_ERR_ARG;
    static_assert(kSegAlign % kResolveBlock == 0 && kSegAlign % kScanBlock == 0 && kSegAlign % (kTailCPW * kEmitWaves) == 0, "segment alignment");
    if (sg.final && (r.d_n_rows != &state->rows_at[sg.index] || r.d_n_rows_needed != &state->rows_needed)) return URHGPU_ERR_ARG;
    if ((sg.h_state == nullptr) != (sg.h_len == nullptr) || sg.gate.seg != state) return URHGPU_ERR_ARG;
    const TileCarve tc = carve_tile(m);
    EmitTileArgs g;
    g.e = e; g.r = r; g.ft = tc.ft; g.huge = tc.huge; g.huge_cap = kTileHugeCap;
    g.bp = bp; g.ft.want_bits = 1;
    g.w0 = sg.c0 / kTailCPW; g.w_end = sg.final ? tail_waves(r.n_chunks) : sg.c1 / kTailCPW; g.final_seg = sg.final; g.seg = state; g.seg_k = sg.index;
    g.h_state = sg.h_state; g.h_len = sg.h_len;
    g.len16 = (sg.len16 && sg.esc && sg.h_len) ? sg.len16 : 0; g.esc = g.len16 ? sg.esc : nullptr; g.esc_cap = sg.esc_cap;
    g.ft.esc = (g.len16 && sg.index == 0) ? sg.esc : nullptr;
    if (g_tail_skip & 64) { g.h_state = nullptr; g.h_len = nullptr; }
    if (g_tail_skip & 128) g.e.rows = nullptr;
    TileTail ft_resolve = g.ft;
    if (sg.index != 0) ft_resolve.want_bits = 0;
    SegGate gate = sg.gate;
    gate.fused = (sg.fuse_gate && gate.progress && !gate.init && resolve_blocks(sg.c1 - sg.c0) == 1) ? 1 : 0;
    if (!gate.fused && gate.progress) hipLaunchKernelGGL(k_seg_gate, dim3(1), dim3(64), 0, s, gate);
    if (!(g_tail_skip & 1)) hipLaunchKernelGGL(k_resolve_one, dim3((unsigned)resolve_blocks(sg.c1 - sg.c0)), dim3(kResolveBlock), 0, s, r, ft_resolve, sg.c0 / kResolveBlock, gate);
    if (!(g_tail_skip & 2)) hipLaunchKernelGGL(k_emit_rows_tiles, dim3((unsigned)((g.w_end - g.w0 + 1 + kEmitWaves - 1) / kEmitWaves)), dim3(64 * kEmitWaves), 0, s, g);
    return URHGPU_OK;
}

int launch_bits_segment(const TileTailMem &m, const BitsParams &bp, const BitsOut &o, void *scratch, const ScanState &ss, int64_t *rows,
                        int64_t cap_rows, const BitsSegment &sg, const SegPackDst *dst, hipStream_t s) {
    if (m.n_chunks <= 0 || m.d_row_base != nullptr || !sg.state || sg.rows_index < 0 || sg.rows_index >= kMaxSegments) return URHGPU_ERR_ARG;
    if (sg.c0 < 0 || sg.c0 % kSegAlign || sg.c1 <= sg.c0 || sg.c1 > m.n_chunks || (sg.final ? sg.c1 != m.n_chunks : (sg.c1 % kSegAlign != 0 || sg.c1 >= m.n_chunks)))
        return URHGPU_ERR_ARG;
    if (cap_rows <= 0) cap_rows = 1;
    const int64_t cap_desc = tile_desc_cap(cap_rows, m.n_chunks);
    if (ss.desc_bytes < bits_desc_bytes(cap_desc)) return URHGPU_ERR_ARG;
    const TileCarve tc = carve_tile(m);
    const BitsScratch b = carve_bits(scratch, cap_rows);
    SegState *st = sg.state;
    const int64_t *d_n_rows = &st->rows_at[sg.rows_index];
    const int parity = sg.index & 1;
    const int64_t t1 = sg.final ? m.n_chunks + 1 : sg.c1;
    const int64_t cap_groups = cap_rows + 1;
    GranDesc *tdesc = (GranDesc *)m.rdesc + resolve_blocks(m.n_chunks) + 2;
    TileScanArgs ta{rows, d_n_rows, tc.ft.agg, tc.ft.tile_off, tc.ft.tile_cnt, tc.ft.excl, b.groups, cap_groups, &st->n_groups, t1, bp, tdesc,
                    m.epoch, sg.c0 / kScanBlock, st, parity};
    if (!(g_tail_skip & 4)) hipLaunchKernelGGL(k_tile_scan, dim3((unsigned)((t1 - sg.c0 + kScanBlock - 1) / kScanBlock)), dim3(kScanBlock), 0, s, ta);
    ScanDesc<3> *desc3 = (ScanDesc<3> *)((char *)ss.desc + (((size_t)(scan_blocks(cap_desc) + 1) * sizeof(ScanDesc<4>) + 255) & ~size_t(255)));
    GroupLoad gl{b.groups, &st->n_groups, nullptr, sg.final ? 1 : 0, bp.write_pos, sg.final ? 0 : 1};
    const int has_pos = (bp.write_pos && o.pos) ? 1 : 0;
    const int64_t caps[5] = {cap_rows, o.cap_msg, o.cap_bits, o.cap_pos, cap_rows};
    BlobLayout L = blob_layout(caps, cap_rows, o.cap_bits, o.cap_msg, o.cap_pos, has_pos);
    const bool split = dst && dst->host && dst->split;
    if (split) {
        if (!sg.final || sg.c0 != 0) return URHGPU_ERR_ARG;
        const StagedLayout SL = staged_layout(cap_rows, o.cap_bits, o.cap_msg, o.cap_pos, has_pos);
        L.off_row_state = SL.off_row_state; L.off_row_len = SL.off_row_len; L.off_pos32 = SL.off_pos32;
    }
    const bool pos_direct = dst && dst->host && has_pos && sg.final && sg.c0 == 0 && dst->pos_direct;
    uint32_t *h_pos = pos_direct ? (uint32_t *)((char *)dst->host + L.off_pos32) : nullptr;
    GroupStore gs{gl, b.gout, o.msg_off, o.pauses, o.pos_off, o.pos, o.cap_msg, o.cap_pos, h_pos};
    SegGroupLoad sl{gl, st, parity};
    SegGroupStore sst{gs, st, parity};
    SegFinal fin{sl, st, d_n_rows, parity, sg.final ? 1 : 0, BitsCountsFinal{d_n_rows, o.msg_off, o.pos_off, o.counts, b.huge_count, &st->rows_needed, o.h_counts}};
    if (!(g_tail_skip & 8))
        hipLaunchKernelGGL((k_scan_lookback<3, SegGroupLoad, SegGroupStore, SegFinal, kGroupItems>), dim3((unsigned)std::min<int64_t>(scan_grid(b.nbg), 32)),
                           dim3(kScanBlock), 0, s, &st->n_groups_local, sl, desc3, b.nbg, sst, fin, ++*ss.epoch, ss.tickets + 2, 0);
    ExpandTileArgs ea{rows, d_n_rows, tc.ft.excl, tc.ft.tile_off, tc.ft.tile_cnt, b.gout, &st->n_groups, o.bits, o.cap_bits, o.pos, o.cap_pos,
                      bp, tc.huge, m.huge_count, kTileHugeCap, m.parity, t1, sg.c0, h_pos};
    const unsigned tile_blocks = (unsigned)expand_tile_blocks(t1 - sg.c0);
    if (g_tail_skip & 2048) ea.cap_bits = 0;
    if (!(g_tail_skip & 16)) hipLaunchKernelGGL(k_expand_tiles, dim3(tile_blocks + kHugeBlocksX * kHugeBlocksY), dim3(64 * kEmitWaves), 0, s, ea);
// ... 73 lines not shown
```

### urh_amd/csrc/shard.hip

```cpp
#include "pass.hpp"

using namespace urh;

namespace {

struct ShardSession {
    int phase = 0;
    bool piped = false;
    RunArgs run;
    int rank = 0, world = 1;
    int64_t n_local = 0, pos_base = 0, n_total = 0;
    urhgpu_params p;
    urhgpu_outputs out;
    Plan pl;
    ChunkInfo *table = nullptr;
    uint64_t *slab = nullptr;
    ResolveAux *aux = nullptr;
    void *rs_mem = nullptr;
    int64_t *rows_stage = nullptr; void *merge_scratch = nullptr; int64_t *d_n_stage = nullptr;
    void *bits_scratch = nullptr;
    int64_t *d_small = nullptr;
    const int64_t *d_row_base = nullptr;
    bool use_tile = false;
    TileTailMem tile;
    CostasShard costas;
    int costas_phase = 0;
    bool demod_done = false;
    const void *demod_iq = nullptr; float *demod_qad = nullptr; int64_t demod_n = 0;
    int demod_mod = 0, demod_dtype = 0; float demod_noise = 0.f;
    float *d_seam = nullptr;
};

ShardSession *session(urhgpu_ctx *ctx) {
    if (!ctx->shard) ctx->shard = new (std::nothrow) ShardSession();
    return (ShardSession *)ctx->shard;
}

}

void urh::free_shard_session(urhgpu_ctx *ctx) {
    ShardSession *ss = (ShardSession *)ctx->shard;
    if (ss && ss->d_seam) (void)hipFree(ss->d_seam);
    delete ss;
    ctx->shard = nullptr;
}

extern "C" {

static int shard_launch(urhgpu_ctx *ctx, const void *d_iq, int64_t n_local, int64_t pos_base, int64_t n_total, int rank, int world,
                        const void *d_left_halo, const urhgpu_params *p, const urhgpu_outputs *out, int part) {
    if (!ctx || !p || !out || !d_iq || !out->rows || !out->counts) return URHGPU_ERR_ARG;
    if (world < 1 || world > kMaxWorld || rank < 0 || rank >= world || n_local < 2 || pos_base < 0 || pos_base + n_local > n_total)
        return URHGPU_ERR_ARG;
    if (rank == 0 && pos_base != 0) return URHGPU_ERR_ARG;
    if (dtype_bytes(p->dtype) == 0) return URHGPU_ERR_DTYPE;
    URH_TRY(check_params(p, true));
    if (((uintptr_t)d_iq & 15) || (out->qad && ((uintptr_t)out->qad & 7))) return URHGPU_ERR_ARG;
    URH_HIP(hipSetDevice(ctx->device));
    ShardSession *ss = session(ctx);
    if (!ss) return URHGPU_ERR_ARG;
    const bool psk = (p->mod == URHGPU_MOD_PSK);
    if (psk && (ctx->pipelined || part != 0)) return URHGPU_ERR_UNSUPPORTED;
    if (psk && (ss->costas_phase != 2 || out->qad != ss->costas.out || n_local != ss->costas.n || d_iq != ss->costas.iq)) return URHGPU_ERR_ARG;
    const bool dem = !psk && part == 0 && !ctx->pipelined && ss->demod_done && out->qad && out->qad == ss->demod_qad && n_local == ss->demod_n &&
                     d_iq == ss->demod_iq && p->mod == ss->demod_mod && p->dtype == ss->demod_dtype && p->noise_threshold == ss->demod_noise;
    ss->demod_done = false;
    const bool from_qad = psk || dem;
    if (dem) d_left_halo = (rank > 0) ? (const void *)ss->d_seam : nullptr;
    ss->piped = ctx->pipelined;
    if (ss->piped) URH_TRY(begin_pipelined_pass(ctx)); else URH_TRY(join_tail(ctx));
    const bool ask = (p->mod == URHGPU_MOD_ASK);
    ss->use_tile = !ask && g_tile_tail;
    hipStream_t s = ctx->stream;
    if (ss->piped && ss->use_tile) URH_TRY(hot_stream_begin(ctx, &s));
    ss->phase = 0; ss->rank = rank; ss->world = world; ss->n_local = n_local; ss->pos_base = pos_base; ss->n_total = n_total;
    ss->p = *p; ss->out = *out;
    const Plan pl = make_plan(ctx, n_local, p->tolerance);
    ss->pl = pl;
    URH_TRY(ctx->arena.reserve(digitize_scratch_bytes(pl, out->cap_rows, ask, true)));
    ctx->arena.reset();
    const int64_t n_table = pl.n_chunks + world - 1;
    ss->table = (ChunkInfo *)ctx->arena.take((size_t)n_table * sizeof(ChunkInfo));
    ss->slab = (uint64_t *)ctx->arena.take((size_t)pl.n_chunks * pl.slab_stride * 8);
    ss->rs_mem = ctx->arena.take(resolve_scratch_bytes(n_table));
    ss->aux = (ResolveAux *)(ctx->d_tickets + 4);
    ss->d_small = (int64_t *)ctx->arena.take(8 * 8);
    ss->bits_scratch = ctx->arena.take(bits_scratch_bytes(std::max<int64_t>(out->cap_rows, 1)));
    ss->rows_stage = out->rows; ss->merge_scratch = nullptr; ss->d_n_stage = ss->d_small + 3;
    if (ask) {
        ss->rows_stage = (int64_t *)ctx->arena.take((size_t)out->cap_rows * 16);
        ss->merge_scratch = ctx->arena.take(merge_scratch_bytes(out->cap_rows));
        ss->d_n_stage = (int64_t *)ctx->arena.take(64);
    }
    if (!ss->table || !ss->slab || !ss->rs_mem || !ss->d_small || !ss->bits_scratch || !ss->rows_stage ||
        !ss->d_n_stage || (ask && !ss->merge_scratch))
        return URHGPU_ERR_ARG;
    if (ss->use_tile) {
        URH_TRY(tile_tail_mem(ctx, n_table, true, &ss->tile));
        if (world > 1) ss->tile.d_row_base = ss->d_small + 4;
    }
    RunArgs &a = ss->run;
    URH_TRY(hot_run_args(ctx, p, pl, n_local, pos_base, !from_qad, &a));
    a.in = from_qad ? (const void *)out->qad : d_iq; a.qad = from_qad ? nullptr : out->qad; a.left_halo = d_left_halo;
    a.lds_pad = !ctx->pipelined ? 0 : (ss->use_tile ? ctx->hot_lds_pad : ctx->hot_lds_pad_sharded);
    a.chunks = ss->table + rank;
    a.slab = ss->slab;
    a.launch_part = part;
    if (part == 1 && rank > 0 && !a.left_halo) a.left_halo = d_iq;
    URH_TRY(hot_launch(ctx, a, p, !from_qad, s, ss->piped && n_local % kTile == 0, ss->piped ? ctx->ev_hot : nullptr,
                       ss->piped ? ctx->tail_stream : nullptr, nullptr));
    ss->costas_phase = 0;
    URH_HIP(hipGetLastError());
    return URHGPU_OK;
}

int urhgpu_shard_prelaunch_dev(urhgpu_ctx *ctx, const void *d_iq, int64_t n_local, int64_t pos_base, int64_t n_total,
                               int rank, int world, const urhgpu_params *p, const urhgpu_outputs *out) {
    if (p && p->mod == URHGPU_MOD_PSK) return URHGPU_ERR_UNSUPPORTED;
    if (ctx && ctx->shard) ((ShardSession *)ctx->shard)->demod_done = false;
    URH_TRY(shard_launch(ctx, d_iq, n_local, pos_base, n_total, rank, world, nullptr, p, out, rank > 0 ? 1 : 0));
    ((ShardSession *)ctx->shard)->phase = -1;
    return URHGPU_OK;
}

int urhgpu_shard_launch_dev(urhgpu_ctx *ctx, const void *d_iq, int64_t n_local, int64_t pos_base, int64_t n_total,
                            int rank, int world, const void *d_left_halo, const urhgpu_params *p, const urhgpu_outputs *out) {
    if ((rank == 0) != (d_left_halo == nullptr)) return URHGPU_ERR_ARG;
    if (p && p->mod == URHGPU_MOD_PSK) return URHGPU_ERR_UNSUPPORTED;
    if (ctx && ctx->shard) ((ShardSession *)ctx->shard)->demod_done = false;
    URH_TRY(shard_launch(ctx, d_iq, n_local, pos_base, n_total, rank, world, d_left_halo, p, out, 0));
    ((ShardSession *)ctx->shard)->phase = -2;
    return URHGPU_OK;
}

int urhgpu_shard_runs_dev(urhgpu_ctx *ctx, const void *d_iq, int64_t n_local, int64_t pos_base, int64_t n_total,
                          int rank, int world, const void *d_left_halo, const urhgpu_params *p,
                          const urhgpu_outputs *out, void *d_summary) {
    if (!ctx || !d_summary) return URHGPU_ERR_ARG;
    if ((rank == 0) != (d_left_halo == nullptr)) return URHGPU_ERR_ARG;
    ShardSession *ss = (ShardSession *)ctx->shard;
    hipStream_t s;
    if (ss && (ss->phase == -1 || ss->phase == -2)) {
        if (ss->rank != rank || ss->world != world || ss->n_local != n_local || ss->run.in != d_iq) return URHGPU_ERR_ARG;
        URH_HIP(hipSetDevice(ctx->device));
        s = ss->piped ? ctx->tail_stream : ctx->stream;
        if (rank > 0 && ss->phase == -1) {
            RunArgs a = ss->run;
            a.left_halo = d_left_halo; a.launch_part = 2;
            URH_TRY(launch_demod_runs_iq(a, p->dtype, p->mod, out->qad != nullptr, s));
        }
    } else {
        URH_TRY(shard_launch(ctx, d_iq, n_local, pos_base, n_total, rank, world, d_left_halo, p, out, 0));
        ss = (ShardSession *)ctx->shard;
        s = ss->piped ? ctx->tail_stream : ctx->stream;
    }
    const Plan &pl = ss->pl;
    const int64_t n_table = pl.n_chunks + world - 1;
    ResolveArgs r;
    memset(&r, 0, sizeof(r));
    r.sc = resolve_scratch_carve(ss->rs_mem, n_table);
    r.chunks = ss->table + rank; r.n_chunks = pl.n_chunks; r.n_total = n_local; r.tol = ss->p.tolerance;
    r.rows = nullptr; r.cap_rows = 0; r.d_n_acc = ctx->d_counts + 9; r.d_n_rows = ctx->d_counts + 10;
    r.d_n_rows_needed = ctx->d_counts + 8; r.write_last_row = 0;
    r.local_pass = 1; r.aux = ss->aux; r.summary_out = (ChunkInfo *)d_summary; r.chunk_first = 0; r.n_local = pl.n_chunks;
    if (ctx->tune_shard_summary_generic) URH_TRY(launch_resolve(r, ctx->d_tickets, s));
    else URH_TRY(launch_shard_summary(r, ctx->d_tickets + 1, s));
    URH_HIP(hipGetLastError());
    ss->phase = 1;
    return URHGPU_OK;
}

int urhgpu_shard_demod_dev(urhgpu_ctx *ctx, const void *d_iq, int64_t n_local, int64_t pos_base, int64_t n_total, int rank, int world,
                           const void *d_left_halo, const urhgpu_params *p, const urhgpu_outputs *out) {
    if (!ctx || !p || !out || !d_iq || !out->qad || !out->rows || !out->counts) return URHGPU_ERR_ARG;
    if (world < 1 || world > kMaxWorld || rank < 0 || rank >= world || n_local < 2 || pos_base < 0 || pos_base + n_local > n_total || n_total <= 2)
        return URHGPU_ERR_ARG;
    if (rank == 0 ? pos_base != 0 : pos_base < 1) return URHGPU_ERR_ARG;
    if ((rank == 0) != (d_left_halo == nullptr)) return URHGPU_ERR_ARG;
    if (dtype_bytes(p->dtype) == 0) return URHGPU_ERR_DTYPE;
    if (p->mod != URHGPU_MOD_ASK && p->mod != URHGPU_MOD_FSK) return URHGPU_ERR_UNSUPPORTED;
    URH_TRY(check_params(p, true));
    if (((uintptr_t)d_iq & 15) || ((uintptr_t)out->qad & 7)) return URHGPU_ERR_ARG;
    if (ctx->pipelined) return URHGPU_ERR_UNSUPPORTED;
    URH_HIP(hipSetDevice(ctx->device));
    URH_TRY(join_tail(ctx));
    ShardSession *ss = session(ctx);
    if (!ss) return URHGPU_ERR_ARG;
    ss->demod_done = false;
    ss->costas_phase = 0;
    ss->phase = 0;
    if (!ss->d_seam) URH_HIP(hipMalloc((void **)&ss->d_seam, 64));
    RunArgs a;
    URH_TRY(hot_run_args(ctx, p, make_plan(ctx, n_local, p->tolerance), n_local, pos_base, true, &a));
    a.in = d_iq; a.qad = out->qad; a.left_halo = d_left_halo;
    const int64_t rows = (n_local + 511) / 512;
    const int grid = (int)std::min<int64_t>(rows, (int64_t)ctx->prop.multiProcessorCount * 16);
    URH_TRY(launch_afp_demod(a, p->dtype, p->mod, grid, ctx->stream));
    if (rank > 0) URH_TRY(launch_afp_seam(a, p->dtype, p->mod, ss->d_seam, ctx->stream));
    URH_HIP(hipGetLastError());
    ss->demod_iq = d_iq; ss->demod_qad = out->qad; ss->demod_n = n_local;
    ss->demod_mod = p->mod; ss->demod_dtype = p->dtype; ss->demod_noise = p->noise_threshold;
    ss->demod_done = true;
    return URHGPU_OK;
}

int urhgpu_shard_seam_value(urhgpu_ctx *ctx, float *seam) {
    if (!ctx || !seam) return URHGPU_ERR_ARG;
    ShardSession *ss = (ShardSession *)ctx->shard;
    if (!ss || !ss->d_seam) return URHGPU_ERR_ARG;
    URH_HIP(hipSetDevice(ctx->device));
    URH_HIP(hipMemcpyAsync(seam, ss->d_seam, sizeof(float), hipMemcpyDeviceToHost, ctx->stream));
    URH_HIP(hipStreamSynchronize(ctx->stream));
    return URHGPU_OK;
}

int urhgpu_shard_rows_dev(urhgpu_ctx *ctx, const void *d_summaries, int64_t *d_merge) {
    if (!ctx || !d_summaries) return URHGPU_ERR_ARG;
    ShardSession *ss = (ShardSession *)ctx->shard;
    if (!ss || ss->phase != 1) return URHGPU_ERR_ARG;
    URH_HIP(hipSetDevice(ctx->device));
    hipStream_t s = ss->piped ? ctx->tail_stream : ctx->stream;
    const int rank = ss->rank, world = ss->world;
    const Plan &pl = ss->pl;
    const bool ask = (ss->p.mod == URHGPU_MOD_ASK);
    if (ask && !d_merge) return URHGPU_ERR_ARG;
    const int64_t n_table = pl.n_chunks + world - 1;
    const ChunkInfo *S = (const ChunkInfo *)d_summaries;
    if (rank > 0) URH_HIP(hipMemcpyAsync(ss->table, S, (size_t)rank * sizeof(ChunkInfo), hipMemcpyDeviceToDevice, s));
    if (rank + 1 < world)
        URH_HIP(hipMemcpyAsync(ss->table + rank + pl.n_chunks, S + rank + 1, (size_t)(world - 1 - rank) * sizeof(ChunkInfo),
                               hipMemcpyDeviceToDevice, s));
    ResolveArgs r;
    memset(&r, 0, sizeof(r));
    r.sc = resolve_scratch_carve(ss->rs_mem, n_table);
    r.chunks = ss->table; r.n_chunks = n_table; r.n_total = ss->n_total; r.tol = ss->p.tolerance;
    r.rows = ss->rows_stage; r.cap_rows = ss->out.cap_rows; r.d_n_acc = ctx->d_counts + 9; r.d_n_rows = ss->d_n_stage;
    r.d_n_rows_needed = ctx->d_counts + 8; r.write_last_row = (rank == world - 1) ? 1 : 0;
    r.local_pass = 0; r.aux = ss->aux; r.summary_out = nullptr; r.chunk_first = rank; r.n_local = pl.n_chunks;
    r.d_ts_carry = ss->d_small;
    URH_HIP(hipMemsetAsync(ss->d_small, 0, 8 * 8, s));
    EmitArgs e;
    e.sc = r.sc;
    e.chunks = ss->table; e.chunk_first = rank; e.slab = ss->slab; e.slab_stride = pl.slab_stride;
    e.rows = ss->rows_stage; e.cap_rows = ss->out.cap_rows; e.d_ts_carry = ss->d_small; e.is_ask = ask ? 1 : 0;
    e.sps = ss->p.samples_per_symbol;
    if (ss->use_tile) {
        BitsParams bp = bits_params(&ss->p);
        bp.d_row_base = ss->tile.d_row_base;
        URH_TRY(launch_tile_rows(r, e, ss->tile, &bp, s));
        ss->d_row_base = ss->tile.d_row_base;
    } else {
        URH_TRY(launch_resolve(r, ctx->d_tickets, s));
        URH_TRY(launch_emit_rows(e, pl.n_chunks, s));
        ss->d_row_base = r.sc.out_off + rank;
    }
    if (ask) {
        URH_TRY(launch_merge_rows_ask(ss->rows_stage, ss->d_n_stage, ss->out.cap_rows, ss->out.rows, ss->out.cap_rows,
                                      ss->d_small + 3, ss->merge_scratch, ctx->d_tickets, s));
        launch_merge_summary(ss->out.rows, ss->d_small + 3, d_merge, s);
    }
    URH_HIP(hipGetLastError());
    ss->phase = 2;
    return URHGPU_OK;
}

int urhgpu_shard_bits_prepare_dev(urhgpu_ctx *ctx, const int64_t *d_merge_all, int64_t *d_flags) {
    if (!ctx || !d_flags) return URHGPU_ERR_ARG;
    ShardSession *ss = (ShardSession *)ctx->shard;
    if (!ss || ss->phase != 2) return URHGPU_ERR_ARG;
    const bool ask = (ss->p.mod == URHGPU_MOD_ASK);
    if (ask && !d_merge_all) return URHGPU_ERR_ARG;
    if (!ss->out.bits || !ss->out.msg_off || !ss->out.pauses || !ss->out.pos_off) return URHGPU_ERR_ARG;
    URH_HIP(hipSetDevice(ctx->device));
    hipStream_t s = ss->piped ? ctx->tail_stream : ctx->stream;
    int64_t *d_n_rows = ss->d_small + 3;
    if (ask) launch_merge_fix(ss->out.rows, d_n_rows, d_merge_all, ss->rank, ss->world, ss->d_small + 1, s);
    BitsParams bp = bits_params(&ss->p);
    bp.d_row_base = ss->d_row_base; bp.d_ts_carry = ss->d_small; bp.d_absorbed = ask ? ss->d_small + 1 : nullptr;
    bp.d_extra = (const int32_t *)(ss->d_small + 2); bp.is_last_rank = (ss->rank == ss->world - 1) ? 1 : 0;
    ScanState sst;
    const int64_t cap = std::max<int64_t>(ss->out.cap_rows, 1);
    if (ss->use_tile) {
        bp.d_ts_carry = nullptr;
        URH_TRY(scan_state(ctx, tile_desc_cap(cap, ss->tile.n_chunks), &sst));
        URH_TRY(launch_tile_bits_prepare(ss->tile, ss->out.rows, d_n_rows, cap, bp, ss->bits_scratch, d_flags, sst, s));
    } else {
        URH_TRY(scan_state(ctx, cap, &sst));
        URH_TRY(launch_bits_prepare(ss->out.rows, d_n_rows, cap, bp, ss->bits_scratch, d_flags, sst, s));
    }
    URH_HIP(hipGetLastError());
    ss->phase = 3;
    return URHGPU_OK;
}

int urhgpu_shard_bits_finish_dev(urhgpu_ctx *ctx, const int64_t *d_flags_all) {
    if (!ctx || !d_flags_all) return URHGPU_ERR_ARG;
    ShardSession *ss = (ShardSession *)ctx->shard;
    if (!ss || ss->phase != 3) return URHGPU_ERR_ARG;
    URH_HIP(hipSetDevice(ctx->device));
    hipStream_t s = ss->piped ? ctx->tail_stream : ctx->stream;
    const bool ask = (ss->p.mod == URHGPU_MOD_ASK);
    launch_bits_extra(d_flags_all, ss->rank, ss->world, (int32_t *)(ss->d_small + 2), s);
    BitsParams bp = bits_params(&ss->p);
    bp.d_row_base = ss->d_row_base; bp.d_ts_carry = ss->d_small; bp.d_absorbed = ask ? ss->d_small + 1 : nullptr;
    bp.d_extra = (const int32_t *)(ss->d_small + 2); bp.is_last_rank = (ss->rank == ss->world - 1) ? 1 : 0;
    bp.d_rows_needed = ctx->d_counts + 8;
    const urhgpu_outputs &o = ss->out;
    BitsOut bo{o.bits, o.cap_bits, o.msg_off, o.pauses, o.cap_msg, o.pos, o.cap_pos, o.pos_off, o.counts};
    ScanState sst;
    const int64_t cap = std::max<int64_t>(o.cap_rows, 1);
    if (ss->use_tile) {
        bp.d_ts_carry = nullptr;
        URH_TRY(scan_state(ctx, tile_desc_cap(cap, ss->tile.n_chunks), &sst));
        URH_TRY(launch_tile_bits_finish(ss->tile, o.rows, ss->d_small + 3, cap, bp, bo, ss->bits_scratch, sst, s));
    } else {
        URH_TRY(scan_state(ctx, cap, &sst));
        URH_TRY(launch_bits_finish(o.rows, ss->d_small + 3, cap, bp, bo, ss->bits_scratch, sst, s));
    }
    if (o.blob) {
        URH_TRY(launch_pack_blob(&o, ss->p.write_bit_sample_pos, s));
    }
    URH_HIP(hipGetLastError());
    ss->phase = 0;
    if (ss->piped) URH_TRY(end_pipelined_pass(ctx));
    return URHGPU_OK;
}

int64_t urhgpu_costas_halo_samples(const urhgpu_params *p) {
    if (!p) return 0;
    return costas_halo_samples(p);
}

int urhgpu_shard_costas_spec_dev(urhgpu_ctx *ctx, const void *d_iq, int64_t n_local, int64_t pos_base, int64_t n_total, int rank, int world,
                                 const void *d_halo, int64_t n_halo, const urhgpu_params *p, const urhgpu_outputs *out, void *d_summary) {
    if (!ctx || !p || !out || !d_iq || !out->qad || !d_summary) return URHGPU_ERR_ARG;
    if (world < 1 || world > kMaxWorld || rank < 0 || rank >= world || n_local < 2 || pos_base < 0 || pos_base + n_local > n_total ||
        n_total <= 2)
        return URHGPU_ERR_ARG;
    if (rank == 0 ? pos_base != 0 : pos_base < 2) return URHGPU_ERR_ARG;
    if (p->mod != URHGPU_MOD_PSK) return URHGPU_ERR_ARG;
    if (dtype_bytes(p->dtype) == 0) return URHGPU_ERR_DTYPE;
    URH_TRY(check_params(p, true));
    if (((uintptr_t)d_iq & 15) || ((uintptr_t)out->qad & 7)) return URHGPU_ERR_ARG;
    if (ctx->pipelined) return URHGPU_ERR_UNSUPPORTED;
    const int64_t need = (rank == 0) ? 0 : std::min<int64_t>(costas_halo_samples(p), pos_base - 1);
    if (rank == 0 ? (d_halo != nullptr || n_halo != 0) : (d_halo == nullptr || n_halo < need || n_halo > pos_base)) return URHGPU_ERR_ARG;
    URH_HIP(hipSetDevice(ctx->device));
    URH_TRY(join_tail(ctx));
    ShardSession *ss = session(ctx);
    if (!ss) return URHGPU_ERR_ARG;
    ss->costas_phase = 0;
    ss->demod_done = false;
    CostasShard &cs = ss->costas;
    cs.iq = d_iq; cs.n = n_local; cs.out = out->qad; cs.p = *p;
    cs.origin = (rank == 0) ? 1 : 0;
    cs.halo_end = (rank == 0) ? nullptr : (const char *)d_halo + (size_t)n_halo * dtype_bytes(p->dtype);
    cs.lo = (rank == 0) ? 1 : std::max<int64_t>(1 - pos_base, -n_halo);
    cs.start1 = 1 - pos_base;
    URH_TRY(ctx->aux.reserve(costas_scratch_bytes(n_local) + 1024));
    ctx->aux.reset();
    cs.scratch = ctx->aux.take(costas_scratch_bytes(n_local));
    if (!cs.scratch) return URHGPU_ERR_ARG;
    URH_TRY(launch_costas_shard_spec(ctx, cs, d_summary));
    ss->costas_phase = 1;
    return URHGPU_OK;
}

int urhgpu_shard_costas_resolve_dev(urhgpu_ctx *ctx, const uint32_t *start_state, uint32_t *d_end_state) {
    if (!ctx || !start_state) return URHGPU_ERR_ARG;
    ShardSession *ss = (ShardSession *)ctx->shard;
    if (!ss || ss->costas_phase != 1) return URHGPU_ERR_ARG;
    URH_HIP(hipSetDevice(ctx->device));
    URH_TRY(launch_costas_shard_resolve(ctx, ss->costas, start_state[0], start_state[1], d_end_state));
    ss->costas_phase = 2;
    return URHGPU_OK;
}

}
```

### urh_amd/shard_engine.py

```python
import ctypes as C

import numpy as np

from . import _lib
from .pipeline import DevicePipeline, _torch_dtype


class ShardResult:

    def __init__(self, qad, rows, bits, msg_off, pauses, pos, pos_off, counts, params, ctx=None):
        self.qad, self.rows_buf, self.bits_buf = qad, rows, bits
        self.msg_off_buf, self.pauses_buf, self.pos_buf, self.pos_off_buf = msg_off, pauses, pos, pos_off
        self.counts, self.params = counts, params
        self._host_counts = None
        self._ctx = ctx
        self._host = None

    def host_counts(self):
        if self._host_counts is None:
            if self._ctx is not None:
                self._ctx.join()
            c = self.counts.cpu().numpy()
            self._host_counts = tuple(int(x) for x in c[:4])
            self._rows_needed = int(c[4])
        return self._host_counts

    def check_capacity(self):
        n_rows, n_msg, n_bits, n_pos = self.host_counts()
        if self._rows_needed > self.rows_buf.shape[0] or n_msg > self.pauses_buf.shape[0] or n_bits > self.bits_buf.shape[0] \
                or (self.pos_buf is not None and n_pos > self.pos_buf.shape[0]):
            raise _lib.UrhGpuError(_lib.ERR_CAPACITY, f"output capacity too small: rows={self._rows_needed} msgs={n_msg} "
                                                      f"bits={n_bits} pos={n_pos}")

    def piece(self):
        self.check_capacity()
        n_rows, n_msg, n_bits, n_pos = self.host_counts()
        rows = self.rows_buf[:n_rows].cpu().numpy()
        if n_rows and rows[0, 0] == _lib.ROW_ABSORBED:
            rows = rows[1:]
        return dict(rows=rows, bits=self.bits_buf[:n_bits].cpu().numpy(),
                    msg_end=self.msg_off_buf[1:n_msg + 1].cpu().numpy(), pauses=self.pauses_buf[:n_msg].cpu().numpy(),
                    pos=self.pos_buf[:n_pos].cpu().numpy() if self.pos_buf is not None else np.zeros(0, np.int64),
                    pos_end=self.pos_off_buf[1:n_msg + 1].cpu().numpy())

    def host(self):
        from .pipeline import HostBits
        if self._host is None:
            raise ValueError("the engine was not asked for host results (host_results=True)")
        if not isinstance(self._host, HostBits):
            eng, slot, copied, pass_no = self._host
            self._host = eng._finish_host_copy(slot, copied, self.params, self.qad, pass_no)
        return self._host

    def __getitem__(self, k):
        if not hasattr(self, "_piece"):
            self._piece = self.piece()
        return self._piece[k]


class GpuShardEngine(DevicePipeline):

    def __init__(self, device: int = 0, pipelined: bool = False, tuning=None, tail_stream_priority: int = 0, host_results: bool = False,
                 worst_case_rows: bool = False):
        super().__init__(device, pipelined=pipelined, tuning=tuning, tail_stream_priority=tail_stream_priority)
        self.worst_case_rows = bool(worst_case_rows)
        self.host_results = bool(host_results)
        self._pass = 0
        self._hslots = None
        self._copy_stream = None
        self._predicted = 0
        self._hqueued = [False, False, False]
        self._slot_pass = [-1, -1, -1]

    def _host_slot(self, cap_rows, cap_bits, cap_msg, cap_pos, has_pos):
        torch = self.torch
        cap = int(_lib.load().urhgpu_blob_capacity(cap_rows, cap_bits, cap_msg, cap_pos, 1 if has_pos else 0))
        if self._hslots is None or self._hslots[0][0].numel() < cap:
            self._hslots = [(torch.empty(cap, dtype=torch.uint8, device=self.device), torch.empty(cap, dtype=torch.uint8).pin_memory(),
                             torch.cuda.Event()) for _ in range(3)]
            self._hevents = [torch.cuda.Event() for _ in range(3)]
            self._copy_stream = torch.cuda.Stream(self.device)
            self._predicted = 0
            self._hqueued = [False, False, False]
            self._slot_pass = [-1, -1, -1]
        k = self._pass % 3
        self._slot_pass[k] = self._pass
        self._pass += 1
        return k, cap

    def _queue_host_copy(self, k):
        torch = self.torch
        dblob, hblob, done = self._hslots[k]
        if self._predicted <= 0:
            for j in range(3):
                if j != k and self._hqueued[j] and self._hslots[j][2].query():
                    hdr = self._hslots[j][1][:128].numpy().view(np.int64)
                    if int(hdr[0]) == _lib.BLOB_MAGIC:
                        self._predicted = max(self._predicted, abs(int(hdr[6])) + abs(int(hdr[6])) // 8 + 65536)
        n = dblob.numel() if self._predicted <= 0 else min(dblob.numel(), self._predicted)
        self._hqueued[k] = True
        ev = self._hevents[k]
        ev.record(torch.cuda.current_stream(self.device))
        self._copy_stream.wait_event(ev)
        with torch.cuda.stream(self._copy_stream):
            hblob[:n].copy_(dblob[:n], non_blocking=True)
            done.record(self._copy_stream)
        return n

    def _finish_host_copy(self, k, copied, params, qad, pass_no):
        from .pipeline import HostBits
        if self._slot_pass[k] != pass_no:
            raise RuntimeError(f"ShardResult.host(): the blob slot of pass {pass_no} has been reused by pass {self._slot_pass[k]} (three blob slots "
                               f"rotate: look at a result before three later passes have been issued) or the slots were reallocated")
        dblob, hblob, done = self._hslots[k]
        done.synchronize()
        hdr = hblob[:128].numpy().view(np.int64)
        total = abs(int(hdr[6]))
        if total > copied:
            with self.torch.cuda.stream(self._copy_stream):
                hblob[copied:total].copy_(dblob[copied:total], non_blocking=False)
        self._predicted = total + total // 8 + 65536
        h = self._host_bits(HostBits, hblob, params, qad)
        h.sharded_piece = True
        return h

    @staticmethod
    def _host_bits(HostBits, hblob, params, qad):
        return HostBits.from_blob(hblob.data_ptr(), params, n_samples=int(qad.shape[0]) if qad is not None else 0,
                                  d_qad=qad.data_ptr() if qad is not None else 0)

    def tail(self, iq_local, p):
        torch = self.torch
        if iq_local.dtype == torch.complex64:
            iq_local = torch.view_as_real(iq_local)
        return iq_local[-2:].contiguous()

    def halo_view(self, left_halo):
        torch = self.torch
        if left_halo.dtype == torch.complex64:
            left_halo = torch.view_as_real(left_halo)
        if tuple(left_halo.shape) != (2, 2):
            raise ValueError("left_halo: the two samples before the shard, shape (2, 2)")
        return left_halo.contiguous()

    def fir_tail(self, iq_local, k):
        torch = self.torch
        if iq_local.dtype == torch.complex64:
            iq_local = torch.view_as_real(iq_local)
        return iq_local[-k:].contiguous()

    def fir(self, iq_local, taps, left):
        torch = self.torch
        x = torch.view_as_real(iq_local) if iq_local.dtype == torch.complex64 else iq_local
        h = torch.view_as_real(taps) if taps.dtype == torch.complex64 else taps
        if x.dtype != torch.float32 or h.dtype != torch.float32 or not x.is_contiguous():
            raise ValueError("FIR needs contiguous float32 / complex64 samples and taps")
        if h.dim() != 2 or h.shape[1] != 2:
            raise ValueError("taps: complex64 (m,) or float32 (m, 2)")
        h = h.contiguous()
        out = torch.empty_like(x)
        self.ctx.set_stream(torch.cuda.current_stream(self.device).cuda_stream)
        _lib.check(_lib.load().urhgpu_fir_filter_dev(self.ctx.handle, C.c_void_p(x.data_ptr()), x.shape[0], C.c_void_p(h.data_ptr()),
                                                     h.shape[0], C.c_void_p(left.data_ptr()) if left is not None else None,
                                                     C.c_void_p(out.data_ptr())))
        self._fir_keep = (x, h, left)
        return out if iq_local.dtype != torch.complex64 else torch.view_as_complex(out)

    def _setup(self, iq, p, want_qad, n_total=0):
        torch = self.torch
        if iq.dtype == torch.complex64:
            iq = torch.view_as_real(iq)
        if iq.dim() != 2 or iq.shape[1] != 2 or not iq.is_contiguous():
            raise ValueError("IQ must be a contiguous (N, 2) tensor")
        npdt = _torch_dtype(iq)
        n = iq.shape[0]
        cp = p.to_c(npdt)
        cap_rows, cap_bits, cap_msg, cap_pos = self.capacities(n, p, (n // (p.tolerance + 1) + 2) if self.worst_case_rows else None)
        extra = (max(int(n_total) - n, 0) // max(int(p.samples_per_symbol), 1) + 1) * int(p.bits_per_symbol)
        cap_bits += extra
        cap_pos += extra
        qad = self._buf("qad", (n,), torch.float32) if want_qad else None
        rows = self._buf("rows", (cap_rows, 2), torch.int64)
        bits = self._buf("bits", (cap_bits,), torch.uint8)
        msg_off = self._buf("msg_off", (cap_msg + 1,), torch.int64)
        pauses = self._buf("pauses", (cap_msg,), torch.int64)
        pos_off = self._buf("pos_off", (cap_msg + 1,), torch.int64)
        pos = self._buf("pos", (cap_pos,), torch.int64) if p.write_bit_sample_pos else None
        counts = self._buf("counts", (5,), torch.int64)
        o = _lib.Outputs()
        o.qad = qad.data_ptr() if qad is not None else None
        o.rows = rows.data_ptr(); o.cap_rows = cap_rows
        o.bits = bits.data_ptr(); o.cap_bits = cap_bits
        o.msg_off = msg_off.data_ptr(); o.pauses = pauses.data_ptr(); o.cap_msg = cap_msg
        o.pos = pos.data_ptr() if pos is not None else None
        o.cap_pos = cap_pos if pos is not None else 0
        o.pos_off = pos_off.data_ptr()
        o.counts = counts.data_ptr()
        self._hslot = None
        if self.host_results:
            k, cap = self._host_slot(cap_rows, cap_bits, cap_msg, cap_pos if pos is not None else 0, pos is not None)
            dblob, _, done = self._hslots[k]
            (self.tail_stream if self.tail_stream is not None else torch.cuda.current_stream(self.device)).wait_event(done)
            o.blob = dblob.data_ptr(); o.cap_blob = cap
            self._hslot = k
        self._res = ShardResult(qad, rows, bits, msg_off, pauses, pos, pos_off, counts, p, self.ctx)
        self._ask = p.modulation_type == "ASK"
        self._keep = (iq,)
        self.ctx.set_stream(torch.cuda.current_stream(self.device).cuda_stream)
        return iq, n, cp, o

    def runs_begin(self, iq, pos_base, n_total, rank, world, p, want_qad):
        iq, n, cp, o = self._setup(iq, p, want_qad, n_total)
        self._pre = (iq, n, cp, o)
        _lib.check(_lib.load().urhgpu_shard_prelaunch_dev(self.ctx.handle, C.c_void_p(iq.data_ptr()), n, int(pos_base), int(n_total),
                                                          int(rank), int(world), C.byref(cp), C.byref(o)))

    def runs_launch(self, iq, left, pos_base, n_total, rank, world, p, want_qad):
        iq, n, cp, o = self._setup(iq, p, want_qad, n_total)
        self._pre = (iq, n, cp, o)
        self._keep += (left,)
        _lib.check(_lib.load().urhgpu_shard_launch_dev(self.ctx.handle, C.c_void_p(iq.data_ptr()), n, int(pos_base), int(n_total),
                                                       int(rank), int(world), C.c_void_p(left.data_ptr()) if left is not None else None,
                                                       C.byref(cp), C.byref(o)))

    def runs(self, iq, left, pos_base, n_total, rank, world, p, want_qad):
        torch = self.torch
        pre = getattr(self, "_pre", None)
        if pre is not None:
            iq, n, cp, o = pre
            self._pre = None
        else:
            iq, n, cp, o = self._setup(iq, p, want_qad, n_total)
        self._keep += (left,)
        if left is not None and getattr(self, "tail_stream", None) is not None:
            left.record_stream(self.tail_stream)
        summary = self._buf("summary", (9,), torch.int64)
        lh = C.c_void_p(left.data_ptr()) if left is not None else None
        _lib.check(_lib.load().urhgpu_shard_runs_dev(self.ctx.handle, C.c_void_p(iq.data_ptr()), n, int(pos_base), int(n_total),
                                                     int(rank), int(world), lh, C.byref(cp), C.byref(o),
                                                     C.c_void_p(summary.data_ptr())))
        return summary

    def costas_spec(self, iq_local, left_raw, pos_base, n_total, rank, world, p):
        from .sharding import COSTAS_SUMMARY_BYTES
        torch = self.torch
        if self.tail_stream is not None:
            raise ValueError("PSK shards run on an engine that is not pipelined: GpuShardEngine(pipelined=False)")
        iq, n, cp, o = self._setup(iq_local, p, True, n_total)
        self._pre = (iq, n, cp, o)
        halo = None
        if left_raw is not None:
            halo = torch.view_as_real(left_raw) if left_raw.dtype == torch.complex64 else left_raw
            if halo.dtype != iq.dtype or halo.dim() != 2 or halo.shape[1] != 2:
                raise ValueError("left_raw: raw samples in the shard's dtype, (m, 2) or complex64 (m,)")
            halo = halo.contiguous()
            self._keep += (halo,)
        summary = self._buf("costas_summary", (COSTAS_SUMMARY_BYTES,), torch.uint8)
        self._costas_end = self._buf("costas_end", (2,), torch.int32)
        self._costas_end.zero_()
        _lib.check(_lib.load().urhgpu_shard_costas_spec_dev(
            self.ctx.handle, C.c_void_p(iq.data_ptr()), n, int(pos_base), int(n_total), int(rank), int(world),
            C.c_void_p(halo.data_ptr()) if halo is not None else None, int(halo.shape[0]) if halo is not None else 0,
            C.byref(cp), C.byref(o), C.c_void_p(summary.data_ptr())))
        return summary

    def costas_resolve(self, start):
        st = (C.c_uint32 * 2)(int(start[0]), int(start[1]))
        _lib.check(_lib.load().urhgpu_shard_costas_resolve_dev(self.ctx.handle, st, C.c_void_p(self._costas_end.data_ptr())))

    def costas_end(self):
        return self._costas_end

    def costas_last(self):
        return self._res.qad[-1:]

    def costas_stats(self):
        return self.ctx.costas_stats()

    def costas_qad(self):
        return self._res.qad

    def set_center(self, center):
        self._pre[2].center = float(center)

    def demod_own(self, iq_local, left_halo=None):
        torch = self.torch
        if self.tail_stream is not None:
            raise ValueError("a pass that demodulates first runs on an engine that is not pipelined: GpuShardEngine(pipelined=False) "
                             "(gathered values are read on the host between its phases)")
        iq = torch.view_as_real(iq_local) if iq_local.dtype == torch.complex64 else iq_local
        if iq.dim() != 2 or iq.shape[1] != 2:
            raise ValueError("IQ must be an (N, 2) tensor or complex64 (N,)")
        _torch_dtype(iq)
        self._own(iq, "iq_to_bits_auto")
        if left_halo is not None:
            halo = self.halo_view(left_halo)
            if halo.dtype != iq.dtype or halo.device != iq.device:
                raise ValueError("left_halo: the two samples before the shard, in the shard's sample type and on its device")

    def demod(self, iq_local, left, pos_base, n_total, rank, world, p):
        iq, n, cp, o = self._setup(iq_local, p, True, n_total)
        self._pre = (iq, n, cp, o)
        self._keep += (left,)
        _lib.check(_lib.load().urhgpu_shard_demod_dev(self.ctx.handle, C.c_void_p(iq.data_ptr()), n, int(pos_base), int(n_total), int(rank), int(world),
                                                      C.c_void_p(left.data_ptr()) if left is not None else None, C.byref(cp), C.byref(o)))

    def demod_qad(self):
        return self._res.qad

    def demod_seam(self):
        v = (C.c_float * 1)()
        _lib.check(_lib.load().urhgpu_shard_seam_value(self.ctx.handle, v))
        return np.frombuffer(v, dtype=np.float32)[0].copy()

    def _own(self, t, what):
        if not t.is_cuda or t.device != self.device:
            raise ValueError(f"{what}: the shard lies on {t.device}, the engine runs on {self.device}")
        if not t.is_contiguous():
            raise ValueError(f"{what}: the shard must be contiguous")
        self.ctx.set_stream(self.torch.cuda.current_stream(self.device).cuda_stream)

    def noise_partials(self, iq_local, pos_base, n_total, chunk, n_chunks):
        from .signal_functions import dtype_code
        torch = self.torch
        iq = torch.view_as_real(iq_local) if iq_local.dtype == torch.complex64 else iq_local
        if iq.dim() != 2 or iq.shape[1] != 2:
            raise ValueError("IQ must be an (N, 2) tensor or complex64 (N,)")
        code = dtype_code(_torch_dtype(iq))
        self._own(iq, "detect_noise_level")
        out = torch.empty((2, int(n_chunks)), dtype=torch.float64, device=self.device)
        if n_chunks:
            _lib.check(_lib.load().urhgpu_magnitude_chunk_partials_dev(
                self.ctx.handle, C.c_void_p(iq.data_ptr()), code, int(iq.shape[0]), int(pos_base), int(n_total), int(chunk), int(n_chunks),
                C.c_void_p(out[0].data_ptr()), C.c_void_p(out[1].data_ptr())))
        out._urh_keep = iq
        return out

    def compact_gt(self, x, thr):
        torch = self.torch
        if x.dtype != torch.float32 or x.dim() != 1:
            raise ValueError("detect_center: a float32 1-D tensor (the shard's demodulated signal)")
        self._own(x, "detect_center")
        n = int(x.shape[0])
        kept = torch.empty(max(n, 1), dtype=torch.float32, device=self.device)
        cnt = torch.zeros(1, dtype=torch.int64, device=self.device)
        _lib.check(_lib.load().urhgpu_compact_gt_dev(self.ctx.handle, C.c_void_p(x.data_ptr()), n, float(thr), C.c_void_p(kept.data_ptr()),
                                                     C.c_void_p(cnt.data_ptr())))
        kept._urh_keep = x
        return kept, cnt

    def pairwise_partial(self, x, g_off, m_total, mode, mean, words):
        torch = self.torch
        self.ctx.set_stream(torch.cuda.current_stream(self.device).cuda_stream)
        rec = torch.zeros(int(words), dtype=torch.float32, device=self.device)
        n_out = C.c_int64(0)
        _lib.check(_lib.load().urhgpu_pairwise_partial_f32_dev(self.ctx.handle, C.c_void_p(x.data_ptr()) if x.numel() else None, int(x.shape[0]),
                                                               int(g_off), int(m_total), int(mode), float(mean), C.c_void_p(rec.data_ptr()),
                                                               int(words), C.byref(n_out)))
        rec._urh_keep = x
        return rec

    def histogram(self, x, edges):
        torch = self.torch
        self.ctx.set_stream(torch.cuda.current_stream(self.device).cuda_stream)
        d_edges = torch.from_numpy(np.ascontiguousarray(edges, dtype=np.float64)).to(self.device)
        counts = torch.empty(len(edges) - 1, dtype=torch.int64, device=self.device)
        _lib.check(_lib.load().urhgpu_histogram_f32_dev(self.ctx.handle, C.c_void_p(x.data_ptr()) if x.numel() else None, int(x.shape[0]),
                                                        C.c_void_p(d_edges.data_ptr()), len(edges), C.c_void_p(counts.data_ptr())))
        counts._urh_keep = (x, d_edges)
        return counts

    def _dc_rows(self, t, what):
        from .filter import _TORCH_CODES
        torch = self.torch
        x = torch.view_as_real(t) if t.dtype == torch.complex64 else t
        code = _TORCH_CODES.get(str(x.dtype))
        if code is None:
            raise ValueError(f"{what}: Unsupported dtype {x.dtype}")
        if x.dim() != 2 or x.shape[1] != 2:
            raise ValueError(f"{what}: an (n, 2) tensor of a sample type or complex64 (n,)")
        return x, code

    def dc_own(self, iq_local, also, out):
        x, code = self._dc_rows(iq_local, "dc_correct")
        self._own(x, "dc_correct")
        if out is not None and out is not iq_local:
            raise ValueError("dc_correct: out is None or the shard itself")
        for t in also:
            a, a_code = self._dc_rows(t, "dc_correct: also")
            if a_code != code:
                raise ValueError("dc_correct: `also` holds tensors of the shard's sample type")
            self._own(a, "dc_correct: also")
        return code == _lib.DT_F32

    def dc_whole(self, iq_local, out):
        from .filter import dc_correct_dev
        res, mean = dc_correct_dev(self, iq_local, out=out, want_mean=True)
        self._dc_single = self._dc_rows(iq_local, "dc_correct")[1] == _lib.DT_F32
        return res, mean.cpu().numpy()

    def dc_sums(self, iq_local):
        x, code = self._dc_rows(iq_local, "dc_correct")
        self.ctx.set_stream(self.torch.cuda.current_stream(self.device).cuda_stream)
        words = self.torch.empty(3, dtype=self.torch.int64, device=self.device)
        _lib.check(_lib.load().urhgpu_shard_dc_sums_dev(self.ctx.handle, C.c_void_p(x.data_ptr()) if x.shape[0] else None, int(x.shape[0]), code,
                                                        C.c_void_p(words.data_ptr())))
        words._urh_keep = x
        self._dc_single = None
        return words

    def dc_spec(self, iq_local, base):
        x, _ = self._dc_rows(iq_local, "dc_correct")
        self.ctx.set_stream(self.torch.cuda.current_stream(self.device).cuda_stream)
        recs = self.torch.empty((2, 2, 4), dtype=self.torch.int32, device=self.device)
        _lib.check(_lib.load().urhgpu_shard_dc_spec_dev(self.ctx.handle, C.c_void_p(x.data_ptr()) if x.shape[0] else None, int(x.shape[0]),
                                                        (C.c_double * 2)(float(base[0]), float(base[1])), C.c_void_p(recs.data_ptr())))
        recs._urh_keep = x
        return recs

    def dc_resolve(self, iq_local, entry):
        out = self.torch.zeros(2, dtype=self.torch.int32, device=self.device)
        if entry is not None:
            x, _ = self._dc_rows(iq_local, "dc_correct")
            self.ctx.set_stream(self.torch.cuda.current_stream(self.device).cuda_stream)
            _lib.check(_lib.load().urhgpu_shard_dc_resolve_dev(self.ctx.handle, C.c_void_p(x.data_ptr()) if x.shape[0] else None, int(x.shape[0]),
                                                               (C.c_uint32 * 2)(int(entry[0]), int(entry[1])), C.c_void_p(out.data_ptr())))
            out._urh_keep = x
        return out

    def dc_apply(self, t, mean, out=None):
        x, code = self._dc_rows(t, "dc_correct")
        res = self.torch.empty_like(t) if out is None else out
        y = self.torch.view_as_real(res) if res.dtype == self.torch.complex64 else res
        m = np.ascontiguousarray(mean, dtype=np.float32 if code == _lib.DT_F32 else np.float64)
        self.ctx.set_stream(self.torch.cuda.current_stream(self.device).cuda_stream)
        _lib.check(_lib.load().urhgpu_shard_dc_apply_dev(self.ctx.handle, C.c_void_p(x.data_ptr()) if x.shape[0] else None, int(x.shape[0]), code,
                                                         C.c_void_p(m.ctypes.data), C.c_void_p(y.data_ptr()) if x.shape[0] else None))
        res._urh_keep = x
        return res

    def dc_stats(self):
        lib, st = _lib.load(), (C.c_int64 * 8)()
        single = getattr(self, "_dc_single", None)
        if single is not None:
            if single:
                _lib.check(lib.urhgpu_test_dc_stats(self.ctx.handle, st))
            return {"chunks": int(st[0]), "derived": int(st[1]), "reevaluated": int(st[2])}
        _lib.check(lib.urhgpu_shard_dc_stats(self.ctx.handle, st))
        return {"chunks": int(st[0]), "derived": int(st[1] + st[5]), "reevaluated": int(st[2] + st[6])}

    def _records_outputs(self, res):
        if res.pos_buf is None:
            raise ValueError("message_records needs the positions of the pass (write_bit_sample_pos)")
        o = _lib.Outputs()
        o.rows = res.rows_buf.data_ptr(); o.cap_rows = int(res.rows_buf.shape[0])
        o.bits = res.bits_buf.data_ptr(); o.cap_bits = int(res.bits_buf.shape[0])
        o.msg_off = res.msg_off_buf.data_ptr(); o.pauses = res.pauses_buf.data_ptr(); o.cap_msg = int(res.pauses_buf.shape[0])
        o.pos = res.pos_buf.data_ptr(); o.cap_pos = int(res.pos_buf.shape[0])
        o.pos_off = res.pos_off_buf.data_ptr()
        o.counts = res.counts.data_ptr()
        return o

    def _records_shard(self, iq_local):
        torch = self.torch
        iq = torch.view_as_real(iq_local) if iq_local.dtype == torch.complex64 else iq_local
        if iq.dim() != 2 or iq.shape[1] != 2:
            raise ValueError("IQ must be an (N, 2) tensor or complex64 (N,)")
        npdt = _torch_dtype(iq)
        self._own(iq, "message_records")
        return iq, npdt

    def records_summary(self, iq_local, res, pos_base):
        from .sharding import REC_SUMMARY_WORDS
        iq, _ = self._records_shard(iq_local)
        o = self._records_outputs(res)
        self.ctx.set_stream(self.torch.cuda.current_stream(self.device).cuda_stream)
        words = self.torch.empty(REC_SUMMARY_WORDS, dtype=self.torch.int64, device=self.device)
        _lib.check(_lib.load().urhgpu_shard_records_summary_dev(self.ctx.handle, int(iq.shape[0]), int(pos_base), C.byref(o), C.c_void_p(words.data_ptr())))
        return words

    def records_lookup(self, res, index):
        torch = self.torch
        self.ctx.set_stream(torch.cuda.current_stream(self.device).cuda_stream)
        o = self._records_outputs(res)
        d_index = torch.from_numpy(np.ascontiguousarray(index, dtype=np.int64)).to(self.device)
        values = torch.empty(len(index), dtype=torch.int64, device=self.device)
        _lib.check(_lib.load().urhgpu_shard_records_lookup_dev(self.ctx.handle, C.byref(o), C.c_void_p(d_index.data_ptr()), len(index),
                                                               C.c_void_p(values.data_ptr())))
        values._urh_keep = d_index
        return values

    def records_window_part(self, iq_local, pos_base, spans, w_max):
        torch = self.torch
        iq, npdt = self._records_shard(iq_local)
        raw = iq.view(torch.uint8).view(int(iq.shape[0]), 2 * npdt.itemsize)
        part = torch.zeros((len(spans), int(w_max), 2 * npdt.itemsize), dtype=torch.uint8, device=self.device)
        a0, b0 = int(pos_base), int(pos_base) + int(iq.shape[0])
        for j, (lo, w) in enumerate(spans):
            a, b = max(lo, a0), min(lo + w, b0)
            if b > a:
                part[j, a - lo:b - lo] = raw[a - a0:b - a0]
        return part

    def records_finish(self, iq_local, res, pos_base, n_total, p, divisor, first, window):
        from .protocol import RECORD_DTYPE
        torch = self.torch
        iq, npdt = self._records_shard(iq_local)
        o, cp = self._records_outputs(res), p.to_c(npdt)
        self.ctx.set_stream(torch.cuda.current_stream(self.device).cuda_stream)
        cap = max(int(o.cap_msg), 1)
        d_rec = self._buf("shard_records", (cap * RECORD_DTYPE.itemsize,), torch.uint8)
        block = self._pinned.get(("records", "shard"))
        if block is None or block.numel() < cap * RECORD_DTYPE.itemsize:
            block = torch.zeros(cap * RECORD_DTYPE.itemsize, dtype=torch.uint8).pin_memory()
            self._pinned[("records", "shard")] = block
        first = np.ascontiguousarray(first, dtype=np.int64)
        if window is not None:
            window = window.contiguous()
        _lib.check(_lib.load().urhgpu_shard_msg_records_dev(
            self.ctx.handle, C.c_void_p(iq.data_ptr()), int(iq.shape[0]), int(pos_base), int(n_total), C.byref(cp), C.byref(o), int(divisor),
            first.ctypes.data_as(C.POINTER(C.c_int64)), C.c_void_p(window.data_ptr()) if window is not None else None,
            int(window.shape[0]) if window is not None else 0, C.c_void_p(d_rec.data_ptr()), cap, C.c_void_p(block.data_ptr())))
        n_msg = min(int(res.counts[1:2].cpu()[0]), cap)
        return block.numpy().view(RECORD_DTYPE)[:n_msg].copy()

    def rows(self, summaries):
        torch = self.torch
        self._keep += (summaries,)
        merge = self._buf("merge", (5,), torch.int64) if self._ask else None
        _lib.check(_lib.load().urhgpu_shard_rows_dev(self.ctx.handle, C.c_void_p(summaries.data_ptr()),
                                                     C.c_void_p(merge.data_ptr()) if merge is not None else None))
        return merge

    def bits_prepare(self, merged_all):
        torch = self.torch
        self._keep += (merged_all,)
        flags = self._buf("flags", (3,), torch.int64)
        _lib.check(_lib.load().urhgpu_shard_bits_prepare_dev(
            self.ctx.handle, C.c_void_p(merged_all.data_ptr()) if merged_all is not None else None, C.c_void_p(flags.data_ptr())))
        return flags

    def bits_finish(self, flags_all):
        self._keep += (flags_all,)
        _lib.check(_lib.load().urhgpu_shard_bits_finish_dev(self.ctx.handle, C.c_void_p(flags_all.data_ptr())))
        if self._hslot is not None:
            self._res._host = (self, self._hslot, self._queue_host_copy(self._hslot), self._slot_pass[self._hslot])
        res, self._res = self._res, None
        res._keep = self._keep
        self._keep = ()
        return res
```

Before: 471,400.

## Move sharded host-result staging into C with early row shipping and packed head

```diff
diff --git a/include/urhgpu.h b/include/urhgpu.h
--- a/include/urhgpu.h
+++ b/include/urhgpu.h
@@ -379,6 +379,13 @@
                                  const urhgpu_outputs *out, int64_t message_length_divisor, const int64_t *first, const void *d_window,
                                  int64_t window_len, void *d_rec, int64_t cap_msg, void *h_rec);
 
+typedef struct urhgpu_shard_host urhgpu_shard_host;
+int urhgpu_shard_host_create(urhgpu_ctx *ctx, void *copy_stream, urhgpu_shard_host **out);
+int urhgpu_shard_host_destroy(urhgpu_shard_host *h);
+int urhgpu_shard_host_begin(urhgpu_shard_host *h, const urhgpu_params *p, int64_t n_local, int64_t n_total, urhgpu_outputs *out, int64_t *ticket);
+int urhgpu_shard_host_result(urhgpu_shard_host *h, int64_t ticket, const void **blob, int64_t *held);
+int urhgpu_shard_host_stats(urhgpu_shard_host *h, int64_t *out4);
+
 #ifdef __cplusplus
 }
 #endif
diff --git a/urh_amd/_lib.py b/urh_amd/_lib.py
--- a/urh_amd/_lib.py
+++ b/urh_amd/_lib.py
@@ -217,6 +217,11 @@
     "urhgpu_shard_dc_resolve_dev": (_i, [_vp, _vp, _i64, C.POINTER(C.c_uint32), _vp]),
     "urhgpu_shard_dc_apply_dev": (_i, [_vp, _vp, _i64, _i, _vp, _vp]),
     "urhgpu_shard_dc_stats": (_i, [_vp, C.POINTER(_i64)]),
+    "urhgpu_shard_host_create": (_i, [_vp, _vp, C.POINTER(_vp)]),
+    "urhgpu_shard_host_destroy": (_i, [_vp]),
+    "urhgpu_shard_host_begin": (_i, [_vp, C.POINTER(Params), _i64, _i64, C.POINTER(Outputs), C.POINTER(_i64)]),
+    "urhgpu_shard_host_result": (_i, [_vp, _i64, C.POINTER(_vp), C.POINTER(_i64)]),
+    "urhgpu_shard_host_stats": (_i, [_vp, C.POINTER(_i64)]),
 }
 
 _lib = None
diff --git a/urh_amd/csrc/common.hpp b/urh_amd/csrc/common.hpp
--- a/urh_amd/csrc/common.hpp
+++ b/urh_amd/csrc/common.hpp
@@ -111,6 +111,7 @@
     bool prof_on = false;
     bool prof_bracket = false;
     void *shard = nullptr;
+    void *shard_host = nullptr;
     bool pipelined = false;
     int hot_lds_pad_sharded = 33 * 1024;
     int tune_hot_cus_removed = 4;
diff --git a/urh_amd/csrc/compact.hip b/urh_amd/csrc/compact.hip
--- a/urh_amd/csrc/compact.hip
+++ b/urh_amd/csrc/compact.hip
@@ -81,6 +81,87 @@
 #endif
     if (hipMemsetAsync((char *)o->blob + 15 * 8, 0, 8, s) != hipSuccess) return URHGPU_ERR_HIP;
     hipLaunchKernelGGL(k_pack_blob, dim3(URH_PACK_BLOCKS), dim3(256), 0, s, a);
+    return URHGPU_OK;
+}
+
+struct HeadArgs {
+    const uint8_t *bits; const int64_t *msg_off, *pauses, *pos_off, *pos; const int64_t *counts;
+    int64_t cap_rows, cap_bits, cap_msg, cap_pos;
+    int has_pos;
+    char *head, *stage;
+    int64_t off_row_state, off_row_len, off_pos32;
+    const int64_t *esc; int64_t esc_cap;
+};
+
+__global__ __launch_bounds__(256) void k_pack_head(const HeadArgs a) {
+    URH_TAIL_PRIO();
+    const int64_t gtid = blockIdx.x * 256ll + threadIdx.x, stride = (int64_t)gridDim.x * 256;
+    const int64_t c5[5] = {0, a.counts[1], a.counts[2], 0, 0};
+    const BlobLayout L = blob_layout(c5, a.cap_rows, a.cap_bits, a.cap_msg, a.cap_pos, 0);
+    const int64_t nbits = L.n_bits, n_msg = L.n_msg;
+    int64_t n_rows = a.counts[0] < a.cap_rows ? a.counts[0] : a.cap_rows;
+    if (n_rows < 0) n_rows = 0;
+    int64_t n_pos = a.has_pos ? (a.counts[3] < a.cap_pos ? a.counts[3] : a.cap_pos) : 0;
+    if (n_pos < 0) n_pos = 0;
+    {
+        uint8_t *out = (uint8_t *)(a.head + L.off_bits);
+        const unsigned long long *in8 = (const unsigned long long *)a.bits;
+        const int64_t nb = (nbits + 7) / 8, nw = nbits / 64;
+        for (int64_t k = gtid; k < nw; k += stride) {
+            unsigned long long r = 0;
+#pragma unroll
+            for (int b = 0; b < 8; ++b) r |= (((in8[8 * k + b] & 0x0101010101010101ull) * 0x8040201008040201ull) >> 56) << (8 * b);
+            *(unsigned long long *)(out + 8 * k) = r;
+        }
+        for (int64_t j = 8 * nw + gtid; j < nb; j += stride) {
+            unsigned long long w;
+            if (8 * j + 8 <= nbits) w = in8[j];
+            else { w = 0; for (int k = 0; k < 8 && 8 * j + k < nbits; ++k) w |= (unsigned long long)a.bits[8 * j + k] << (8 * k); }
+            out[j] = (uint8_t)(((w & 0x0101010101010101ull) * 0x8040201008040201ull) >> 56);
+        }
+    }
+    if (a.has_pos) {
+        uint32_t *p32 = (uint32_t *)(a.stage + a.off_pos32);
+        for (int64_t i = gtid; i < n_pos; i += stride) p32[i] = (uint32_t)a.pos[i];
+    }
+    {
+        int64_t *pa = (int64_t *)(a.head + L.off_pauses), *mo = (int64_t *)(a.head + L.off_msg_off), *po = (int64_t *)(a.head + L.off_pos_off);
+        for (int64_t i = gtid; i <= n_msg; i += stride) {
+            if (i < n_msg) pa[i] = a.pauses[i];
+            mo[i] = a.msg_off[i]; po[i] = a.pos_off[i];
+        }
+    }
+    int64_t n_esc = 0;
+    bool esc_over = false;
+    if (a.esc) {
+        n_esc = a.esc[0];
+        esc_over = n_esc > a.esc_cap;
+        if (esc_over) n_esc = a.esc_cap;
+        int64_t *dst = (int64_t *)(a.head + ((L.off_bits + (nbits + 7) / 8 + 15) & ~int64_t(15)));
+        if (gtid == 0) dst[0] = esc_over ? -n_esc : n_esc;
+        for (int64_t i = gtid; i < n_esc; i += stride) dst[1 + i] = a.esc[1 + i];
+    }
+    if (gtid == 0) {
+        int64_t *hdr = (int64_t *)a.head;
+        const int64_t *c = a.counts;
+        hdr[1] = n_rows; hdr[2] = n_msg; hdr[3] = nbits; hdr[4] = n_pos; hdr[5] = c[4];
+        hdr[6] = URHGPU_BLOB_HEADER_BYTES + n_rows * (a.esc ? 3 : 5) + (a.esc ? 8 + n_esc * 8 : 0) + (nbits + 7) / 8 + n_pos * 4 + n_msg * 24 + 16;
+        hdr[7] = a.has_pos | (a.esc ? URHGPU_BLOB_LEN16 : 0);
+        hdr[8] = L.off_pauses; hdr[9] = L.off_msg_off; hdr[10] = L.off_pos_off; hdr[11] = a.off_row_state; hdr[12] = L.off_bits;
+        hdr[13] = a.off_row_len; hdr[14] = a.off_pos32;
+        hdr[15] = ((c[1] > a.cap_msg || c[2] > a.cap_bits || (a.has_pos && c[3] > a.cap_pos) || c[4] > a.cap_rows) ? 1 : 0) | (esc_over ? 4 : 0);
+        hdr[0] = URHGPU_BLOB_MAGIC;
+    }
+}
+
+int launch_pack_head(const urhgpu_outputs *o, int write_pos, void *head, void *stage, const int64_t *off3, const int64_t *esc, int64_t esc_cap,
+                     hipStream_t s) {
+    if (!o || !head || !stage || !off3 || !o->bits || !o->msg_off || !o->pauses || !o->pos_off || !o->counts) return URHGPU_ERR_ARG;
+    if (((uintptr_t)o->bits & 7) || ((uintptr_t)head & 15) || ((uintptr_t)stage & 15)) return URHGPU_ERR_ARG;
+    const int has_pos = (write_pos && o->pos) ? 1 : 0;
+    HeadArgs a{o->bits, o->msg_off, o->pauses, o->pos_off, o->pos, o->counts, o->cap_rows, o->cap_bits, o->cap_msg, o->cap_pos, has_pos,
+               (char *)head, (char *)stage, off3[0], off3[1], off3[2], esc, esc_cap};
+    hipLaunchKernelGGL(k_pack_head, dim3(has_pos ? 256 : 32), dim3(256), 0, s, a);
     return URHGPU_OK;
 }
 
diff --git a/urh_amd/csrc/compact.hpp b/urh_amd/csrc/compact.hpp
--- a/urh_amd/csrc/compact.hpp
+++ b/urh_amd/csrc/compact.hpp
@@ -35,11 +35,12 @@
 }
 
 struct StagedLayout { int64_t head_cap, off_row_state, off_row_len, off_pos32, total; };
-__host__ __device__ inline StagedLayout staged_layout(int64_t cap_rows, int64_t cap_bits, int64_t cap_msg, int64_t cap_pos, int has_pos) {
+__host__ __device__ inline StagedLayout staged_layout(int64_t cap_rows, int64_t cap_bits, int64_t cap_msg, int64_t cap_pos, int has_pos,
+                                                      int64_t head_extra = 0) {
     const int64_t c[5] = {0, cap_msg, cap_bits, 0, 0};
     auto up = [](int64_t x) { return (x + 15) & ~int64_t(15); };
     StagedLayout S;
-    S.head_cap = blob_layout(c, cap_rows, cap_bits, cap_msg, cap_pos, 0).total;
+    S.head_cap = blob_layout(c, cap_rows, cap_bits, cap_msg, cap_pos, 0).total + up(head_extra);
     S.off_row_state = S.head_cap;
     S.off_row_len = up(S.off_row_state + cap_rows);
     S.off_pos32 = up(S.off_row_len + 4 * cap_rows);
diff --git a/urh_amd/csrc/launchers.hpp b/urh_amd/csrc/launchers.hpp
--- a/urh_amd/csrc/launchers.hpp
+++ b/urh_amd/csrc/launchers.hpp
@@ -264,7 +264,8 @@
 size_t tile_rdesc_bytes(int64_t n_chunks);
 size_t tile_tail_bytes(int64_t n_chunks);
 int64_t tile_desc_cap(int64_t cap_rows, int64_t n_chunks);
-int launch_tile_rows(const ResolveArgs &r, const EmitArgs &e, const TileTailMem &m, const BitsParams *bp, hipStream_t s);
+struct ShipRows { int8_t *state; int32_t *len; int len16; int64_t *esc; int64_t esc_cap; };
+int launch_tile_rows(const ResolveArgs &r, const EmitArgs &e, const TileTailMem &m, const BitsParams *bp, hipStream_t s, const ShipRows *ship = nullptr);
 int launch_tile_bits(const TileTailMem &m, const int64_t *rows, const int64_t *d_n_rows, int64_t cap_rows, const BitsParams &bp,
                      const BitsOut &o, void *scratch, const ScanState &ss, hipStream_t s);
 int launch_tile_bits_prepare(const TileTailMem &m, const int64_t *rows, const int64_t *d_n_rows, int64_t cap_rows, const BitsParams &bp,
@@ -321,6 +322,8 @@
 size_t seg_ctl_bytes();
 void seg_ctl_read(const void *host_copy, int64_t *n_seg, int64_t *n_msgs, int *ambiguous);
 int launch_pack_blob(const urhgpu_outputs *o, int write_pos, hipStream_t s);
+int launch_pack_head(const urhgpu_outputs *o, int write_pos, void *head, void *stage, const int64_t *off3, const int64_t *esc, int64_t esc_cap,
+                     hipStream_t s);
 void launch_copy_shape(const float *in, float *out, int64_t n_samples, int shape, hipStream_t s);
 int launch_msg_records(const void *d_iq, int64_t n, const urhgpu_params *p, const urhgpu_outputs *out, int64_t divisor, void *d_rec, int64_t cap_rec,
                        void *h_rec, hipStream_t s);
diff --git a/urh_amd/csrc/pulse_table.hip b/urh_amd/csrc/pulse_table.hip
--- a/urh_amd/csrc/pulse_table.hip
+++ b/urh_amd/csrc/pulse_table.hip
@@ -1633,11 +1633,12 @@
            64 + (size_t)kTileHugeCap * sizeof(HugeRef) + 10 * 256;
 }
 
-int launch_tile_rows(const ResolveArgs &r, const EmitArgs &e, const TileTailMem &m, const BitsParams *bp, hipStream_t s) {
+int launch_tile_rows(const ResolveArgs &r, const EmitArgs &e, const TileTailMem &m, const BitsParams *bp, hipStream_t s, const ShipRows *ship) {
     if (r.n_chunks <= 0 || r.local_pass || r.chunk_first != e.chunk_first || r.chunk_first < 0 || r.chunk_first + r.n_local > r.n_chunks ||
         m.n_chunks != r.n_chunks || e.is_ask)
         return URHGPU_ERR_ARG;
     if ((r.n_local != r.n_chunks) != (m.d_row_base != nullptr)) return URHGPU_ERR_ARG;
+    if (ship && (!ship->state || !ship->len || (ship->len16 != 0 && ship->len16 != 1) || (ship->len16 && (!ship->esc || ship->esc_cap < 1)))) return URHGPU_ERR_ARG;
     TileCarve tc = carve_tile(m);
     EmitTileArgs g;
     g.e = e; g.r = r; g.ft = tc.ft; g.huge = tc.huge; g.huge_cap = kTileHugeCap;
@@ -1645,6 +1646,10 @@
     if (bp) { g.bp = *bp; g.ft.want_bits = 1; }
     const unsigned gb = (unsigned)resolve_blocks(r.n_chunks);
     g.w0 = 0; g.w_end = tail_waves(r.n_chunks); g.final_seg = 1; g.seg = nullptr; g.seg_k = 0; g.h_state = nullptr; g.h_len = nullptr; g.len16 = 0; g.esc = nullptr; g.esc_cap = 0; g.ft.esc = nullptr;
+    if (ship) {
+        g.h_state = ship->state; g.h_len = ship->len; g.len16 = ship->len16;
+        if (ship->len16) { g.esc = ship->esc; g.esc_cap = ship->esc_cap; g.ft.esc = ship->esc; }
+    }
     SegGate no_gate;
     memset(&no_gate, 0, sizeof(no_gate));
     if (!(g_tail_skip & 1)) hipLaunchKernelGGL(k_resolve_one, dim3(gb), dim3(kResolveBlock), 0, s, r, g.ft, (int64_t)0, no_gate);
diff --git a/urh_amd/csrc/shard.hip b/urh_amd/csrc/shard.hip
--- a/urh_amd/csrc/shard.hip
+++ b/urh_amd/csrc/shard.hip
@@ -1,6 +1,29 @@
 #include "pass.hpp"
 
 using namespace urh;
+
+struct urhgpu_shard_host {
+    urhgpu_ctx *ctx = nullptr;
+    hipStream_t copy_stream = nullptr;
+    int64_t cap_bytes = 0;
+    struct Slot {
+        char *dev = nullptr;
+        char *h_blob2[2] = {nullptr, nullptr};
+        char *h_blob = nullptr;
+        hipEvent_t ev_rows = nullptr, ev_head = nullptr, ev_shipped = nullptr;
+        int64_t pass = -1;
+        int state = 0;
+        bool staged = false, len16 = false;
+        int has_pos = 0;
+        StagedLayout SL;
+        int64_t cap_rows = 0, cap_pos = 0, esc_cap = 0;
+        int64_t copied = 0, copied_rows = 0, copied_pos = 0;
+    } slot[3];
+    Slot *armed = nullptr;
+    int64_t passes = 0;
+    int64_t predicted_bytes = 0, predicted_rows = 0, predicted_pos = 0;
+    int64_t short_copies = 0, staged_passes = 0;
+};
 
 namespace {
 
@@ -29,7 +52,76 @@
     const void *demod_iq = nullptr; float *demod_qad = nullptr; int64_t demod_n = 0;
     int demod_mod = 0, demod_dtype = 0; float demod_noise = 0.f;
     float *d_seam = nullptr;
+    urhgpu_shard_host::Slot *ship = nullptr;
 };
+
+void predict_from_arrived(urhgpu_shard_host *h, const urhgpu_shard_host::Slot *self) {
+    for (auto &s : h->slot) {
+        if (&s == self || s.state != 2 || hipEventQuery(s.ev_head) != hipSuccess || hipEventQuery(s.ev_shipped) != hipSuccess) continue;
+        const int64_t *hdr = (const int64_t *)s.h_blob;
+        if (hdr[0] != URHGPU_BLOB_MAGIC) continue;
+        const int64_t total = hdr[6] < 0 ? -hdr[6] : hdr[6];
+        h->predicted_bytes = std::max(h->predicted_bytes, total + total / 8 + 65536);
+        h->predicted_rows = std::max(h->predicted_rows, hdr[1] + hdr[1] / 8 + 4096);
+        h->predicted_pos = std::max(h->predicted_pos, hdr[4] + hdr[4] / 8 + 4096);
+    }
+    (void)hipGetLastError();
+}
+
+int ship_rows(urhgpu_shard_host *h, urhgpu_shard_host::Slot &k, hipStream_t s) {
+    URH_HIP(hipEventRecord(k.ev_rows, s));
+    if (h->predicted_rows <= 0) predict_from_arrived(h, &k);
+    const int64_t rows = std::min<int64_t>(h->predicted_rows, k.cap_rows);
+    k.copied_rows = 0;
+    if (rows > 0) {
+        URH_HIP(hipStreamWaitEvent(h->copy_stream, k.ev_rows, 0));
+        URH_HIP(hipMemcpyAsync(k.h_blob + k.SL.off_row_state, k.dev + k.SL.off_row_state, (size_t)rows, hipMemcpyDeviceToHost, h->copy_stream));
+        URH_HIP(hipMemcpyAsync(k.h_blob + k.SL.off_row_len, k.dev + k.SL.off_row_len, (size_t)rows * (k.len16 ? 2 : 4), hipMemcpyDeviceToHost, h->copy_stream));
+        k.copied_rows = rows;
+    }
+    return URHGPU_OK;
+}
+
+int ship_end(urhgpu_shard_host *h, urhgpu_shard_host::Slot &k, const urhgpu_outputs &o, int write_pos, hipStream_t s) {
+    if (k.staged) {
+        const int64_t off3[3] = {k.SL.off_row_state, k.SL.off_row_len, k.SL.off_pos32};
+        int64_t *esc = k.len16 ? (int64_t *)(k.dev + URHGPU_BLOB_HEADER_BYTES) : nullptr;
+        URH_TRY(launch_pack_head(&o, write_pos, k.h_blob, k.dev, off3, esc, k.esc_cap, s));
+        URH_HIP(hipGetLastError());
+        URH_HIP(hipEventRecord(k.ev_head, s));
+        k.copied_pos = 0;
+        const int64_t npos = k.has_pos ? std::min<int64_t>(h->predicted_pos, k.cap_pos) : 0;
+        if (npos > 0) {
+            URH_HIP(hipStreamWaitEvent(h->copy_stream, k.ev_head, 0));
+            URH_HIP(hipMemcpyAsync(k.h_blob + k.SL.off_pos32, k.dev + k.SL.off_pos32, (size_t)npos * 4, hipMemcpyDeviceToHost, h->copy_stream));
+            k.copied_pos = npos;
+        }
+        URH_HIP(hipEventRecord(k.ev_shipped, h->copy_stream));
+        h->staged_passes += 1;
+    } else {
+        URH_TRY(launch_pack_blob(&o, write_pos, s));
+        URH_HIP(hipGetLastError());
+        URH_HIP(hipEventRecord(k.ev_head, s));
+        if (h->predicted_bytes <= 0) predict_from_arrived(h, &k);
+        const int64_t n = h->predicted_bytes > 0 ? std::min<int64_t>(h->predicted_bytes, o.cap_blob) : o.cap_blob;
+        URH_HIP(hipStreamWaitEvent(h->copy_stream, k.ev_head, 0));
+        URH_HIP(hipMemcpyAsync(k.h_blob, k.dev, (size_t)n, hipMemcpyDeviceToHost, h->copy_stream));
+        URH_HIP(hipEventRecord(k.ev_shipped, h->copy_stream));
+        k.copied = n;
+    }
+    k.state = 2;
+    return URHGPU_OK;
+}
+
+void free_host_slots(urhgpu_shard_host *h) {
+    for (auto &s : h->slot) {
+        if (s.dev) (void)hipFree(s.dev);
+        for (char *&p : s.h_blob2) { if (p) (void)hipHostFree(p); p = nullptr; }
+        s.dev = nullptr; s.h_blob = nullptr; s.pass = -1; s.state = 0;
+    }
+    h->cap_bytes = 0;
+    h->armed = nullptr;
+}
 
 ShardSession *session(urhgpu_ctx *ctx) {
     if (!ctx->shard) ctx->shard = new (std::nothrow) ShardSession();
@@ -43,6 +135,8 @@
     if (ss && ss->d_seam) (void)hipFree(ss->d_seam);
     delete ss;
     ctx->shard = nullptr;
+    if (ctx->shard_host) ((urhgpu_shard_host *)ctx->shard_host)->ctx = nullptr;
+    ctx->shard_host = nullptr;
 }
 
 extern "C" {
@@ -75,6 +169,14 @@
     if (ss->piped && ss->use_tile) URH_TRY(hot_stream_begin(ctx, &s));
     ss->phase = 0; ss->rank = rank; ss->world = world; ss->n_local = n_local; ss->pos_base = pos_base; ss->n_total = n_total;
     ss->p = *p; ss->out = *out;
+    ss->ship = nullptr;
+    if (urhgpu_shard_host *h = (urhgpu_shard_host *)ctx->shard_host) {
+        if (h->armed && out->blob && out->blob == h->armed->dev) {
+            ss->ship = h->armed;
+            if (!(ss->use_tile && out->bits && n_total <= INT32_MAX)) ss->ship->staged = false;
+        }
+        h->armed = nullptr;
+    }
     const Plan pl = make_plan(ctx, n_local, p->tolerance);
     ss->pl = pl;
     URH_TRY(ctx->arena.reserve(digitize_scratch_bytes(pl, out->cap_rows, ask, true)));
@@ -247,7 +349,16 @@
     if (ss->use_tile) {
         BitsParams bp = bits_params(&ss->p);
         bp.d_row_base = ss->tile.d_row_base;
-        URH_TRY(launch_tile_rows(r, e, ss->tile, &bp, s));
+        if (ss->ship && ss->ship->staged && ctx->shard_host) {
+            urhgpu_shard_host::Slot &k = *ss->ship;
+            const ShipRows ship{(int8_t *)(k.dev + k.SL.off_row_state), (int32_t *)(k.dev + k.SL.off_row_len), k.len16 ? 1 : 0,
+                                k.len16 ? (int64_t *)(k.dev + URHGPU_BLOB_HEADER_BYTES) : nullptr, k.esc_cap};
+            URH_TRY(launch_tile_rows(r, e, ss->tile, &bp, s, &ship));
+            URH_HIP(hipGetLastError());
+            URH_TRY(ship_rows((urhgpu_shard_host *)ctx->shard_host, k, s));
+        } else {
+            URH_TRY(launch_tile_rows(r, e, ss->tile, &bp, s));
+        }
         ss->d_row_base = ss->tile.d_row_base;
     } else {
         URH_TRY(launch_resolve(r, ctx->d_tickets, s));
@@ -317,7 +428,10 @@
         URH_TRY(scan_state(ctx, cap, &sst));
         URH_TRY(launch_bits_finish(o.rows, ss->d_small + 3, cap, bp, bo, ss->bits_scratch, sst, s));
     }
-    if (o.blob) {
+    if (ss->ship && ctx->shard_host) {
+        URH_TRY(ship_end((urhgpu_shard_host *)ctx->shard_host, *ss->ship, o, ss->p.write_bit_sample_pos, s));
+        ss->ship = nullptr;
+    } else if (o.blob) {
         URH_TRY(launch_pack_blob(&o, ss->p.write_bit_sample_pos, s));
     }
     URH_HIP(hipGetLastError());
@@ -376,4 +490,131 @@
     return URHGPU_OK;
 }
 
-}
+int urhgpu_shard_host_create(urhgpu_ctx *ctx, void *copy_stream, urhgpu_shard_host **out) {
+    if (!ctx || !out || ctx->shard_host) return URHGPU_ERR_ARG;
+    URH_HIP(hipSetDevice(ctx->device));
+    urhgpu_shard_host *h = new (std::nothrow) urhgpu_shard_host();
+    if (!h) return URHGPU_ERR_ARG;
+    h->ctx = ctx; h->copy_stream = (hipStream_t)copy_stream;
+    for (auto &s : h->slot) {
+        if (hipEventCreateWithFlags(&s.ev_rows, hipEventDisableTiming) != hipSuccess || hipEventCreateWithFlags(&s.ev_head, hipEventDisableTiming) != hipSuccess ||
+            hipEventCreateWithFlags(&s.ev_shipped, hipEventDisableTiming) != hipSuccess) {
+            urhgpu_shard_host_destroy(h);
+            return URHGPU_ERR_HIP;
+        }
+    }
+    ctx->shard_host = h;
+    *out = h;
+    return URHGPU_OK;
+}
+
+int urhgpu_shard_host_destroy(urhgpu_shard_host *h) {
+    if (!h) return URHGPU_OK;
+    if (h->ctx) {
+        (void)hipSetDevice(h->ctx->device);
+        (void)urhgpu_ctx_sync(h->ctx);
+        if (h->ctx->shard) ((ShardSession *)h->ctx->shard)->ship = nullptr;
+        if (h->ctx->shard_host == h) h->ctx->shard_host = nullptr;
+    }
+    (void)hipStreamSynchronize(h->copy_stream);
+    free_host_slots(h);
+    for (auto &s : h->slot) {
+        if (s.ev_rows) (void)hipEventDestroy(s.ev_rows);
+        if (s.ev_head) (void)hipEventDestroy(s.ev_head);
+        if (s.ev_shipped) (void)hipEventDestroy(s.ev_shipped);
+    }
+    delete h;
+    return URHGPU_OK;
+}
+
+int urhgpu_shard_host_begin(urhgpu_shard_host *h, const urhgpu_params *p, int64_t n_local, int64_t n_total, urhgpu_outputs *out, int64_t *ticket) {
+    if (!h || !h->ctx || !p || !out || !ticket || n_local < 2 || n_total < n_local) return URHGPU_ERR_ARG;
+    if (out->cap_rows < 1 || out->cap_bits < 0 || out->cap_msg < 0) return URHGPU_ERR_ARG;
+    urhgpu_ctx *ctx = h->ctx;
+    URH_HIP(hipSetDevice(ctx->device));
+    const int has_pos = (p->write_bit_sample_pos && out->pos) ? 1 : 0;
+    const int64_t cap_pos = has_pos ? out->cap_pos : 0;
+    const bool staged = p->mod != URHGPU_MOD_ASK && g_tile_tail && out->bits && n_total <= INT32_MAX;
+    const int64_t esc_cap = n_local / 65535 + 3;
+    const StagedLayout SL = staged_layout(out->cap_rows, out->cap_bits, out->cap_msg, cap_pos, has_pos, 8 + esc_cap * 8 + 16);
+    const int64_t need = std::max<int64_t>(blob_capacity(out->cap_rows, out->cap_bits, out->cap_msg, cap_pos, has_pos), SL.total);
+    if (need > h->cap_bytes) {
+        URH_TRY(urhgpu_ctx_sync(ctx));
+        URH_HIP(hipStreamSynchronize(h->copy_stream));
+        free_host_slots(h);
+        const size_t bytes = ((size_t)need + 255) & ~size_t(255);
+        for (auto &s : h->slot) {
+            if (hipMalloc((void **)&s.dev, bytes) != hipSuccess || hipHostMalloc((void **)&s.h_blob2[0], bytes) != hipSuccess ||
+                hipHostMalloc((void **)&s.h_blob2[1], bytes) != hipSuccess) {
+                (void)hipGetLastError();
+                free_host_slots(h);
+                return URHGPU_ERR_HIP;
+            }
+        }
+        h->cap_bytes = (int64_t)bytes;
+        h->predicted_bytes = h->predicted_rows = h->predicted_pos = 0;
+    }
+    const int64_t i = h->passes;
+    urhgpu_shard_host::Slot &k = h->slot[i % 3];
+    if (k.state == 2) URH_HIP(hipStreamWaitEvent(ctx->pipelined && ctx->tail_stream ? ctx->tail_stream : ctx->stream, k.ev_shipped, 0));
+    k.h_blob = k.h_blob2[(i / 3) & 1];
+    k.pass = i; k.state = 1; k.staged = staged; k.len16 = staged; k.has_pos = has_pos; k.SL = SL;
+    k.cap_rows = out->cap_rows; k.cap_pos = cap_pos; k.esc_cap = esc_cap;
+    k.copied = k.copied_rows = k.copied_pos = 0;
+    out->blob = k.dev; out->cap_blob = h->cap_bytes;
+    h->armed = &k;
+    h->passes = i + 1;
+    *ticket = i;
+    return URHGPU_OK;
+}
+
+int urhgpu_shard_host_result(urhgpu_shard_host *h, int64_t ticket, const void **blob, int64_t *held) {
+    if (!h || !blob || !held || ticket < 0) return URHGPU_ERR_ARG;
+    *blob = nullptr;
+    urhgpu_shard_host::Slot &k = h->slot[ticket % 3];
+    *held = k.pass;
+    if (k.pass != ticket) return URHGPU_OK;
+    if (k.state != 2) return URHGPU_ERR_ARG;
+    if (h->ctx) URH_HIP(hipSetDevice(h->ctx->device));
+    URH_HIP(hipEventSynchronize(k.ev_head));
+    URH_HIP(hipEventSynchronize(k.ev_shipped));
+    const int64_t *hdr = (const int64_t *)k.h_blob;
+    bool more = false;
+    auto fetch = [&](int64_t off, int64_t bytes) -> int {
+        URH_HIP(hipMemcpyAsync(k.h_blob + off, k.dev + off, (size_t)bytes, hipMemcpyDeviceToHost, h->copy_stream));
+        more = true;
+        return URHGPU_OK;
+    };
+    if (k.staged) {
+        const int64_t n_rows = hdr[1], n_pos = (hdr[7] & 1) ? hdr[4] : 0;
+        const int64_t len_bytes = (hdr[7] & URHGPU_BLOB_LEN16) ? 2 : 4;
+        if (hdr[0] != URHGPU_BLOB_MAGIC || n_rows < 0 || n_rows > k.cap_rows || n_pos < 0 || n_pos > k.cap_pos) return URHGPU_ERR_ARG;
+        if (n_rows > k.copied_rows) {
+            URH_TRY(fetch(k.SL.off_row_state + k.copied_rows, n_rows - k.copied_rows));
+            URH_TRY(fetch(k.SL.off_row_len + len_bytes * k.copied_rows, len_bytes * (n_rows - k.copied_rows)));
+            k.copied_rows = n_rows;
+        }
+        if (n_pos > k.copied_pos) { URH_TRY(fetch(k.SL.off_pos32 + 4 * k.copied_pos, 4 * (n_pos - k.copied_pos))); k.copied_pos = n_pos; }
+        h->predicted_rows = n_rows + n_rows / 8 + 4096;
+        h->predicted_pos = n_pos + n_pos / 8 + 4096;
+    } else {
+        const int64_t total = hdr[6] < 0 ? -hdr[6] : hdr[6];
+        if (hdr[0] != URHGPU_BLOB_MAGIC || total > h->cap_bytes) return URHGPU_ERR_ARG;
+        if (total > k.copied) { URH_TRY(fetch(k.copied, total - k.copied)); k.copied = total; }
+        h->predicted_bytes = total + total / 8 + 65536;
+    }
+    if (more) {
+        URH_HIP(hipStreamSynchronize(h->copy_stream));
+        h->short_copies += 1;
+    }
+    *blob = k.h_blob;
+    return URHGPU_OK;
+}
+
+int urhgpu_shard_host_stats(urhgpu_shard_host *h, int64_t *out4) {
+    if (!h || !out4) return URHGPU_ERR_ARG;
+    out4[0] = h->passes; out4[1] = h->short_copies; out4[2] = h->staged_passes; out4[3] = h->cap_bytes;
+    return URHGPU_OK;
+}
+
+}
diff --git a/urh_amd/shard_engine.py b/urh_amd/shard_engine.py
--- a/urh_amd/shard_engine.py
+++ b/urh_amd/shard_engine.py
@@ -48,8 +48,8 @@
         if self._host is None:
             raise ValueError("the engine was not asked for host results (host_results=True)")
         if not isinstance(self._host, HostBits):
-            eng, slot, copied, pass_no = self._host
-            self._host = eng._finish_host_copy(slot, copied, self.params, self.qad, pass_no)
+            eng, ticket = self._host
+            self._host = eng._host_result(ticket, self.params, self.qad)
         return self._host
 
     def __getitem__(self, k):
@@ -65,68 +65,51 @@
         super().__init__(device, pipelined=pipelined, tuning=tuning, tail_stream_priority=tail_stream_priority)
         self.worst_case_rows = bool(worst_case_rows)
         self.host_results = bool(host_results)
-        self._pass = 0
-        self._hslots = None
+        self._hhost = None
         self._copy_stream = None
-        self._predicted = 0
-        self._hqueued = [False, False, False]
-        self._slot_pass = [-1, -1, -1]
-
-    def _host_slot(self, cap_rows, cap_bits, cap_msg, cap_pos, has_pos):
-        torch = self.torch
-        cap = int(_lib.load().urhgpu_blob_capacity(cap_rows, cap_bits, cap_msg, cap_pos, 1 if has_pos else 0))
-        if self._hslots is None or self._hslots[0][0].numel() < cap:
-            self._hslots = [(torch.empty(cap, dtype=torch.uint8, device=self.device), torch.empty(cap, dtype=torch.uint8).pin_memory(),
-                             torch.cuda.Event()) for _ in range(3)]
-            self._hevents = [torch.cuda.Event() for _ in range(3)]
-            self._copy_stream = torch.cuda.Stream(self.device)
-            self._predicted = 0
-            self._hqueued = [False, False, False]
-            self._slot_pass = [-1, -1, -1]
-        k = self._pass % 3
-        self._slot_pass[k] = self._pass
-        self._pass += 1
-        return k, cap
-
-    def _queue_host_copy(self, k):
-        torch = self.torch
-        dblob, hblob, done = self._hslots[k]
-        if self._predicted <= 0:
-            for j in range(3):
-                if j != k and self._hqueued[j] and self._hslots[j][2].query():
-                    hdr = self._hslots[j][1][:128].numpy().view(np.int64)
-                    if int(hdr[0]) == _lib.BLOB_MAGIC:
-                        self._predicted = max(self._predicted, abs(int(hdr[6])) + abs(int(hdr[6])) // 8 + 65536)
-        n = dblob.numel() if self._predicted <= 0 else min(dblob.numel(), self._predicted)
-        self._hqueued[k] = True
-        ev = self._hevents[k]
-        ev.record(torch.cuda.current_stream(self.device))
-        self._copy_stream.wait_event(ev)
-        with torch.cuda.stream(self._copy_stream):
-            hblob[:n].copy_(dblob[:n], non_blocking=True)
-            done.record(self._copy_stream)
-        return n
-
-    def _finish_host_copy(self, k, copied, params, qad, pass_no):
+
+    def _host_begin(self, cp, n, n_total, o):
+        lib = _lib.load()
+        if self._hhost is None:
+            self._copy_stream = self.torch.cuda.Stream(self.device)
+            h = C.c_void_p()
+            _lib.check(lib.urhgpu_shard_host_create(self.ctx.handle, C.c_void_p(self._copy_stream.cuda_stream), C.byref(h)))
+            self._hhost = h
+        ticket = C.c_int64(-1)
+        _lib.check(lib.urhgpu_shard_host_begin(self._hhost, C.byref(cp), int(n), int(max(n_total, n)), C.byref(o), C.byref(ticket)))
+        return int(ticket.value)
+
+    def _host_result(self, ticket, params, qad):
         from .pipeline import HostBits
-        if self._slot_pass[k] != pass_no:
-            raise RuntimeError(f"ShardResult.host(): the blob slot of pass {pass_no} has been reused by pass {self._slot_pass[k]} (three blob slots "
+        blob, held = C.c_void_p(), C.c_int64(-1)
+        _lib.check(_lib.load().urhgpu_shard_host_result(self._hhost, int(ticket), C.byref(blob), C.byref(held)))
+        if not blob.value:
+            raise RuntimeError(f"ShardResult.host(): the blob slot of pass {ticket} has been reused by pass {held.value} (three blob slots "
                                f"rotate: look at a result before three later passes have been issued) or the slots were reallocated")
-        dblob, hblob, done = self._hslots[k]
-        done.synchronize()
-        hdr = hblob[:128].numpy().view(np.int64)
-        total = abs(int(hdr[6]))
-        if total > copied:
-            with self.torch.cuda.stream(self._copy_stream):
-                hblob[copied:total].copy_(dblob[copied:total], non_blocking=False)
-        self._predicted = total + total // 8 + 65536
-        h = self._host_bits(HostBits, hblob, params, qad)
+        h = self._host_bits(HostBits, blob.value, params, qad)
         h.sharded_piece = True
         return h
 
+    def host_stats(self):
+        st = (C.c_int64 * 4)()
+        if self._hhost is not None:
+            _lib.check(_lib.load().urhgpu_shard_host_stats(self._hhost, st))
+        return {"passes": int(st[0]), "short_copies": int(st[1]), "staged_passes": int(st[2]), "blob_bytes": int(st[3])}
+
+    def close_host(self):
+        if self._hhost is not None:
+            h, self._hhost = self._hhost, None
+            _lib.load().urhgpu_shard_host_destroy(h)
+
+    def __del__(self):
+        try:
+            self.close_host()
+        except Exception:
+            pass
+
     @staticmethod
-    def _host_bits(HostBits, hblob, params, qad):
-        return HostBits.from_blob(hblob.data_ptr(), params, n_samples=int(qad.shape[0]) if qad is not None else 0,
+    def _host_bits(HostBits, host_ptr, params, qad):
+        return HostBits.from_blob(host_ptr, params, n_samples=int(qad.shape[0]) if qad is not None else 0,
                                   d_qad=qad.data_ptr() if qad is not None else 0)
 
     def tail(self, iq_local, p):
@@ -196,17 +179,11 @@
         o.cap_pos = cap_pos if pos is not None else 0
         o.pos_off = pos_off.data_ptr()
         o.counts = counts.data_ptr()
-        self._hslot = None
-        if self.host_results:
-            k, cap = self._host_slot(cap_rows, cap_bits, cap_msg, cap_pos if pos is not None else 0, pos is not None)
-            dblob, _, done = self._hslots[k]
-            (self.tail_stream if self.tail_stream is not None else torch.cuda.current_stream(self.device)).wait_event(done)
-            o.blob = dblob.data_ptr(); o.cap_blob = cap
-            self._hslot = k
         self._res = ShardResult(qad, rows, bits, msg_off, pauses, pos, pos_off, counts, p, self.ctx)
         self._ask = p.modulation_type == "ASK"
         self._keep = (iq,)
         self.ctx.set_stream(torch.cuda.current_stream(self.device).cuda_stream)
+        self._hticket = self._host_begin(cp, n, n_total, o) if self.host_results else None
         return iq, n, cp, o
 
     def runs_begin(self, iq, pos_base, n_total, rank, world, p, want_qad):
@@ -543,8 +520,8 @@
     def bits_finish(self, flags_all):
         self._keep += (flags_all,)
         _lib.check(_lib.load().urhgpu_shard_bits_finish_dev(self.ctx.handle, C.c_void_p(flags_all.data_ptr())))
-        if self._hslot is not None:
-            self._res._host = (self, self._hslot, self._queue_host_copy(self._hslot), self._slot_pass[self._hslot])
+        if self._hticket is not None:
+            self._res._host = (self, self._hticket)
         res, self._res = self._res, None
         res._keep = self._keep
         self._keep = ()
```

Result: no change. 470,200 (-0.3%).
